# Hi-PACE/hipace

Hardware: AMD Instinct MI355X
Metric: transverse slices/s at 1024^2 x 4ppc (explicit solver) (higher is better)
Workload: dtype f64

## Files before the change

hipace_amd/_lib.py:

```python
import ctypes as C
import os
import subprocess


def hip_already_started():
    import sys
    if _LIB is not None:
        return True
    t = sys.modules.get("torch")
    try:
        return bool(t is not None and t.cuda.is_initialized())
    except Exception:
        return False


_LIB = None
_HWQ_PRESET = "GPU_MAX_HW_QUEUES" in os.environ
_HIP_STARTED_AT_IMPORT = hip_already_started()
_HERE = os.path.dirname(os.path.abspath(__file__))
CSRC = os.path.join(_HERE, "csrc")
SO = os.environ.get("HPS_LIB") or os.path.join(CSRC, "libhpslice.so")


class Slab(C.Structure):
    _fields_ = [("p", C.c_void_p), ("nx", C.c_int), ("ny", C.c_int), ("ng", C.c_int), ("ncomp", C.c_int),
                ("jstride", C.c_long), ("nstride", C.c_long)]


PL_REAL = ["x", "y", "w", "ux", "uy", "psi", "x_prev", "y_prev", "ux_half", "uy_half", "psi_half"]


class Plasma(C.Structure):
    _fields_ = [(k, C.c_void_p) for k in PL_REAL] + [("idcpu", C.c_void_p), ("ion_lev", C.c_void_p), ("n", C.c_long)]


class BeamSlice(C.Structure):
    _fields_ = [(k, C.c_void_p) for k in ("x", "y", "z", "ux", "uy", "uz", "w")] + [("nsub", C.c_void_p), ("n", C.c_long)]


class Geom(C.Structure):
    _fields_ = [(k, C.c_double) for k in ("dx", "dy", "dz", "xoff", "yoff", "c", "ep0", "mu0", "q_e", "m_e")] + \
               [("plo", C.c_double * 2), ("phi", C.c_double * 2), ("bc", C.c_int), ("normalized", C.c_int)]


class Deck(C.Structure):
    _fields_ = [("nx", C.c_int), ("ny", C.c_int), ("nz", C.c_int),
                ("lo", C.c_double * 3), ("hi", C.c_double * 3),
                ("order", C.c_int), ("deriv_type", C.c_int),
                ("plasma_ppc", C.c_int * 2), ("plasma_density", C.c_double), ("plasma_radius", C.c_double),
                ("plasma_charge", C.c_double), ("plasma_mass", C.c_double), ("max_qsa", C.c_double),
                ("n_subcycles", C.c_int),
                ("beam_profile", C.c_int), ("beam_zmin", C.c_double), ("beam_zmax", C.c_double),
                ("beam_radius", C.c_double), ("beam_density", C.c_double),
                ("beam_umean", C.c_double * 3), ("beam_pos_mean", C.c_double * 3),
                ("beam_pos_std", C.c_double * 3), ("beam_ppc", C.c_int * 3), ("beam_charge", C.c_double),
                ("bc", C.c_int), ("mg_tol_rel", C.c_double), ("mg_tol_abs", C.c_double),
                ("deposit_rho", C.c_int), ("n_steps", C.c_int),
                ("dt", C.c_double), ("beam_n_subcycles", C.c_int), ("beam_mass", C.c_double), ("ext_E_slope", C.c_double * 2),
                ("bxby_solver", C.c_int), ("predcorr_tol", C.c_double), ("predcorr_max_iter", C.c_int),
                ("predcorr_mix", C.c_double), ("field_bc", C.c_int),
                ("laser_on", C.c_int), ("laser_a0", C.c_double), ("laser_w0", C.c_double), ("laser_L0", C.c_double),
                ("laser_lambda0", C.c_double), ("laser_pos", C.c_double * 3),
                ("laser_zfoc", C.c_double), ("laser_solver", C.c_int), ("laser_use_phase", C.c_int), ("si_units", C.c_int),
                ("grid_current_on", C.c_int), ("grid_current_peak", C.c_double), ("grid_current_mean", C.c_double * 3),
                ("grid_current_std", C.c_double * 3), ("laser_mg_tol_rel", C.c_double), ("laser_mg_tol_abs", C.c_double),
                ("beam_radiation_reaction", C.c_int), ("background_density_SI", C.c_double), ("beam_no_z_push", C.c_int),
                ("plasma_no_neutralize", C.c_int), ("ion_on", C.c_int), ("ion_ppc", C.c_int * 2), ("ion_density", C.c_double),
                ("ion_mass", C.c_double), ("ion_charge", C.c_double), ("ion_init_level", C.c_int), ("ion_Z", C.c_int),
                ("ion_energies", C.c_double * 56), ("ion_seed", C.c_ulonglong),
                ("beam_spin_tracking", C.c_int), ("beam_initial_spin", C.c_double * 3), ("beam_spin_anom", C.c_double),
                ("dt_adaptive", C.c_int), ("nt_per_betatron", C.c_double), ("dt_max", C.c_double),
                ("adaptive_threshold_uz", C.c_double), ("adaptive_phase_tolerance", C.c_double),
                ("adaptive_no_predict_step", C.c_int), ("adaptive_no_phase_control", C.c_int), ("adaptive_phase_substeps", C.c_int),
                ("adaptive_density", C.c_double), ("max_time", C.c_double), ("beam_uz_std", C.c_double),
                ("ext_Ez_slope", C.c_double),
                ("beam_do_salame", C.c_int), ("salame_n_iter", C.c_int), ("salame_relative_tolerance", C.c_double),
                ("salame_no_advance", C.c_int), ("salame_Ez_target_slope", C.c_double)]


COMPS = ["N_jx_beam", "N_jy_beam", "chi", "Sy", "Sx", "ExmBy", "EypBx", "Ez", "Bx", "By", "Bz",
         "Psi", "jx_beam", "jy_beam", "jz_beam", "jx", "jy", "rhomjz", "P_jx_beam", "P_jy_beam",
         "Ion_rhomjz", "rho"]
CIDX = {n: i for i, n in enumerate(COMPS)}
COMPS_PC = ["N_jx", "N_jy", "ExmBy", "EypBx", "Ez", "Bx", "By", "Bz", "Psi", "jx", "jy", "jz", "rhomjz",
            "P_Bx", "P_By", "P_jx", "P_jy", "Ion_rhomjz", "It_Bx", "It_By", "PIt_Bx", "PIt_By", "rho"]
CIDX_PC = {n: i for i, n in enumerate(COMPS_PC)}
COMPS_SALAME = ["Ez_target", "Ez_no_salame", "Ez", "jx", "jy", "jz_beam", "Bx", "By", "Sy", "Sx", "Sy_back", "Sx_back"]
ID_VALID = 1 << 63

_SIGS = {
    "hps_last_error": (C.c_char_p, []),
    "hps_version": (C.c_char_p, []),
    "hps_deposit_current": (C.c_int, [Slab, Plasma, Geom, C.c_void_p, C.c_double, C.c_double, C.c_int, C.c_double,
                                      C.c_int, C.c_void_p, C.c_void_p]),
    "hps_explicit_deposit": (C.c_int, [Slab, Plasma, Geom, C.c_void_p, C.c_void_p, C.c_double, C.c_double, C.c_int,
                                       C.c_int, C.c_int, C.c_void_p]),
    "hps_advance_plasma": (C.c_int, [Slab, Plasma, Geom, C.c_void_p, C.c_double, C.c_double, C.c_int, C.c_int,
                                     C.c_int, C.c_int, C.c_void_p]),
    "hps_tiling_create": (C.c_int, [C.c_int, C.c_int, C.c_int, C.c_long, C.POINTER(C.c_void_p)]),
    "hps_reorder_particles": (C.c_int, [C.c_void_p, Plasma, Plasma, Geom, C.c_void_p]),
    "hps_tiling_info": (C.c_int, [C.c_void_p, C.POINTER(C.c_int), C.POINTER(C.c_void_p), C.POINTER(C.c_void_p)]),
    "hps_tiling_destroy": (C.c_int, [C.c_void_p]),
    "hps_deposit_current_tiled": (C.c_int, [Slab, Plasma, Geom, C.c_void_p, C.c_double, C.c_double, C.c_int, C.c_double,
                                            C.c_int, C.c_void_p, C.c_void_p, C.c_void_p, C.c_void_p]),
    "hps_explicit_deposit_tiled": (C.c_int, [Slab, Plasma, Geom, C.c_void_p, C.c_void_p, C.c_double, C.c_double, C.c_int,
                                             C.c_int, C.c_int, C.c_void_p, C.c_void_p, C.c_void_p]),
    "hps_advance_plasma_tiled": (C.c_int, [Slab, Plasma, Geom, C.c_void_p, C.c_double, C.c_double, C.c_int, C.c_int,
                                           C.c_int, C.c_int, C.c_void_p, C.c_void_p, C.c_void_p]),
    "hps_deposit_current_tiled_laser": (C.c_int, [Slab, Plasma, Geom, C.c_void_p, C.c_int, C.c_double, C.c_double, C.c_int,
                                                  C.c_double, C.c_int, C.c_void_p, C.c_void_p, C.c_void_p, C.c_void_p]),
    "hps_explicit_deposit_tiled_laser": (C.c_int, [Slab, Plasma, Geom, C.c_void_p, C.c_int, C.c_void_p, C.c_double, C.c_double,
                                                   C.c_int, C.c_int, C.c_int, C.c_void_p, C.c_void_p, C.c_void_p]),
    "hps_advance_plasma_tiled_laser": (C.c_int, [Slab, Plasma, Geom, C.c_void_p, C.c_int, C.c_double, C.c_double, C.c_int,
                                                 C.c_int, C.c_int, C.c_int, C.c_void_p, C.c_void_p, C.c_void_p]),
    "hps_tiling_set_validity": (C.c_int, [C.c_void_p, C.c_int, C.c_int]),
    "hps_particles_record": (C.c_int, [C.c_int]),
    "hps_particles_recorded": (C.c_int, [C.c_char_p, C.c_long, C.POINTER(C.c_long)]),
    "hps_poisson_create": (C.c_int, [C.c_int, C.c_int, C.c_double, C.c_double, C.POINTER(C.c_void_p)]),
    "hps_poisson_solve": (C.c_int, [C.c_void_p, C.c_void_p, Slab, C.c_int, C.c_void_p]),
    "hps_poisson_solve_batch": (C.c_int, [C.c_void_p, C.c_int, C.c_void_p, Slab, C.c_void_p, C.c_void_p]),
    "hps_poisson_info": (C.c_int, [C.c_void_p, C.POINTER(C.c_int), C.POINTER(C.c_int), C.POINTER(C.c_int)]),
    "hps_poisson_destroy": (C.c_int, [C.c_void_p]),
    "hps_mg_create": (C.c_int, [C.c_int, C.c_int, C.c_double, C.c_double, C.POINTER(C.c_void_p)]),
    "hps_mg_solve1": (C.c_int, [C.c_void_p, Slab, C.c_int, C.c_int, C.c_int, C.c_double, C.c_double, C.c_int,
                                C.POINTER(C.c_int), C.POINTER(C.c_double), C.c_void_p]),
    "hps_mg_solve1_fabs": (C.c_int, [C.c_void_p, Slab, Slab, Slab, C.c_double, C.c_double, C.c_int,
                                     C.POINTER(C.c_int), C.POINTER(C.c_double), C.c_void_p]),
    "hps_mg_info": (C.c_int, [C.c_void_p, C.POINTER(C.c_int), C.POINTER(C.c_int), C.POINTER(C.c_int), C.POINTER(C.c_int),
                              C.POINTER(C.c_long), C.POINTER(C.c_int), C.POINTER(C.c_int), C.POINTER(C.c_int), C.POINTER(C.c_int)]),
    "hps_mg_destroy": (C.c_int, [C.c_void_p]),
    "hps_mg2_create": (C.c_int, [C.c_int, C.c_int, C.c_double, C.c_double, C.POINTER(C.c_void_p)]),
    "hps_mg2_solve2": (C.c_int, [C.c_void_p, C.c_void_p, C.c_void_p, C.c_void_p, C.c_void_p, C.c_double, C.c_double, C.c_int,
                                 C.POINTER(C.c_int), C.POINTER(C.c_double), C.c_void_p]),
    "hps_mg2_info": (C.c_int, [C.c_void_p, C.POINTER(C.c_int), C.POINTER(C.c_int), C.POINTER(C.c_int), C.POINTER(C.c_int)]),
    "hps_mg2_destroy": (C.c_int, [C.c_void_p]),
    "hps_engine_laser_vcycles": (C.c_int, [C.c_void_p, C.POINTER(C.c_long)]),
    "hps_engine_create": (C.c_int, [C.POINTER(Deck), C.c_int, C.POINTER(C.c_void_p)]),
    "hps_engine_destroy": (C.c_int, [C.c_void_p]),
    "hps_engine_begin_step": (C.c_int, [C.c_void_p]),
    "hps_engine_solve_slice": (C.c_int, [C.c_void_p, C.c_int]),
    "hps_engine_solve_slice_begin": (C.c_int, [C.c_void_p, C.c_int]),
    "hps_engine_solve_slice_finish": (C.c_int, [C.c_void_p, C.c_int]),
    "hps_engine_slice_ready": (C.c_int, [C.c_void_p]),
    "hps_engine_run_step": (C.c_int, [C.c_void_p]),
    "hps_engine_sync": (C.c_int, [C.c_void_p]),
    "hps_engine_info": (C.c_int, [C.c_void_p, C.POINTER(C.c_int), C.POINTER(C.c_int), C.POINTER(C.c_long)]),
    "hps_engine_slab": (Slab, [C.c_void_p]),
    "hps_engine_plasma": (Plasma, [C.c_void_p]),
    "hps_engine_stream": (C.c_void_p, [C.c_void_p]),
    "hps_engine_ions": (Plasma, [C.c_void_p]),
    "hps_engine_ion_stats": (C.c_int, [C.c_void_p, C.POINTER(C.c_long), C.POINTER(C.c_long)]),
    "hps_engine_checksums": (C.c_int, [C.c_void_p, C.c_void_p]),
    "hps_beam_sort_by_box": (C.c_int, [C.c_void_p, C.c_long, C.c_double, C.c_double, C.c_int, C.c_void_p, C.c_void_p,
                                       C.c_void_p, C.c_void_p]),
    "hps_engine_stats": (C.c_int, [C.c_void_p, C.POINTER(C.c_long), C.POINTER(C.c_long)]),
    "hps_engine_set_insitu_plasma": (C.c_int, [C.c_void_p, C.c_double]),
    "hps_engine_set_insitu_beam": (C.c_int, [C.c_void_p, C.c_double]),
    "hps_engine_insitu_beam": (C.c_int, [C.c_void_p, C.c_void_p]),
    "hps_engine_insitu_plasma": (C.c_int, [C.c_void_p, C.c_void_p]),
    "hps_engine_set_insitu_fields": (C.c_int, [C.c_void_p, C.c_int]),
    "hps_engine_insitu_fields": (C.c_int, [C.c_void_p, C.c_void_p]),
    "hps_engine_set_field_diagnostic": (C.c_int, [C.c_void_p, C.c_int, C.c_void_p, C.c_void_p]),
    "hps_engine_field_diagnostic": (C.c_int, [C.c_void_p, C.c_void_p]),
    "hps_engine_set_field_diagnostic_box": (C.c_int, [C.c_void_p, C.c_int, C.c_void_p, C.c_void_p, C.c_int, C.c_void_p, C.c_void_p]),
    "hps_engine_field_diagnostic_geometry": (C.c_int, [C.c_void_p, C.c_void_p, C.c_void_p, C.c_void_p]),
    "hps_engine_record_event": (C.c_int, [C.c_void_p, C.c_int, C.POINTER(C.c_void_p)]),
    "hps_engine_wait_event": (C.c_int, [C.c_void_p, C.c_void_p]),
    "hps_stream_pool_shared_pairs": (C.c_int, [C.c_int]),
    "hps_engine_copy_async": (C.c_int, [C.c_void_p, C.c_void_p, C.c_void_p, C.c_long]),
    "hps_engine_set_profiling_stride": (C.c_int, [C.c_void_p, C.c_int]),
    "hps_engine_set_laser_import": (C.c_int, [C.c_void_p, C.c_int, C.c_int]),
    "hps_engine_set_step": (C.c_int, [C.c_void_p, C.c_int]),
    "hps_engine_set_time": (C.c_int, [C.c_void_p, C.c_double, C.c_double]),
    "hps_engine_beam_moments": (C.c_int, [C.c_void_p, C.c_void_p]),
    "hps_adaptive_create": (C.c_int, [C.c_void_p, C.POINTER(C.c_void_p)]),
    "hps_adaptive_set_density_profile": (C.c_int, [C.c_void_p, C.c_int, C.c_void_p, C.c_void_p, C.c_int, C.c_void_p, C.c_void_p]),
    "hps_adaptive_initial_dt": (C.c_int, [C.c_void_p, C.c_double, C.c_double, C.c_int, C.POINTER(C.c_double)]),
    "hps_adaptive_before_step": (C.c_int, [C.c_void_p, C.c_double, C.POINTER(C.c_double)]),
    "hps_adaptive_next_time": (C.c_int, [C.c_void_p, C.POINTER(C.c_double)]),
    "hps_adaptive_after_step": (C.c_int, [C.c_void_p, C.c_void_p, C.c_double, C.c_int, C.POINTER(C.c_double)]),
    "hps_adaptive_destroy": (C.c_int, [C.c_void_p]),
    "hps_engine_export_laser_slice": (C.c_int, [C.c_void_p, C.c_int, C.c_void_p]),
    "hps_engine_import_laser_slice": (C.c_int, [C.c_void_p, C.c_int, C.c_void_p]),
    "hps_engine_import_laser_from": (C.c_int, [C.c_void_p, C.c_int, C.c_void_p]),
    "hps_engine_laser_envelope": (C.c_int, [C.c_void_p, C.c_void_p]),
    "hps_engine_laser_info": (C.c_int, [C.c_void_p, C.POINTER(C.c_int), C.POINTER(C.c_double)]),
    "hps_deposit_current_laser": (C.c_int, [Slab, Plasma, Geom, C.c_void_p, C.c_int, C.c_double, C.c_double, C.c_int, C.c_double,
                                            C.c_int, C.c_void_p, C.c_void_p]),
    "hps_explicit_deposit_laser": (C.c_int, [Slab, Plasma, Geom, C.c_void_p, C.c_int, C.c_void_p, C.c_double, C.c_double, C.c_int,
                                             C.c_int, C.c_int, C.c_void_p]),
    "hps_advance_plasma_laser": (C.c_int, [Slab, Plasma, Geom, C.c_void_p, C.c_int, C.c_double, C.c_double, C.c_int, C.c_int,
                                           C.c_int, C.c_int, C.c_void_p]),
    "hps_engine_pc_stats": (C.c_int, [C.c_void_p, C.POINTER(C.c_long), C.POINTER(C.c_double)]),
    "hps_engine_pc_zero_b_slices": (C.c_int, [C.c_void_p, C.POINTER(C.c_long)]),
    "hps_engine_set_diagnostics": (C.c_int, [C.c_void_p, C.c_int]),
    "hps_engine_set_tiling": (C.c_int, [C.c_void_p, C.c_int, C.c_int]),
    "hps_engine_fallbacks": (C.c_int, [C.c_void_p, C.POINTER(C.c_long)]),
    "hps_engine_set_fusion": (C.c_int, [C.c_void_p, C.c_int]),
    "hps_engine_set_density_profile": (C.c_int, [C.c_void_p, C.c_int, C.c_void_p, C.c_void_p, C.c_int, C.c_void_p, C.c_void_p]),
    "hps_engine_sorts": (C.c_int, [C.c_void_p, C.POINTER(C.c_long)]),
    "hps_engine_assume_initial_beam_support": (C.c_int, [C.c_void_p]),
    "hps_engine_beam_state": (C.c_int, [C.c_void_p, C.c_void_p, C.c_void_p]),
    "hps_engine_beam_capacity": (C.c_int, [C.c_void_p, C.POINTER(C.c_long)]),
    "hps_engine_set_beam_capacity": (C.c_int, [C.c_void_p, C.c_long]),
    "hps_engine_beam_message_rows": (C.c_int, [C.c_void_p, C.POINTER(C.c_int)]),
    "hps_engine_beam_spin": (C.c_int, [C.c_void_p, C.c_void_p]),
    "hps_engine_set_beam_import": (C.c_int, [C.c_void_p, C.c_int]),
    "hps_engine_export_beam_slice": (C.c_int, [C.c_void_p, C.c_int, C.c_void_p]),
    "hps_engine_import_beam_slice": (C.c_int, [C.c_void_p, C.c_int, C.c_void_p]),
    "hps_engine_set_profiling": (C.c_int, [C.c_void_p, C.c_int]),
    "hps_engine_phase_times": (C.c_int, [C.c_void_p, C.c_void_p, C.c_void_p]),
    "hps_engine_beam_info": (C.c_int, [C.c_void_p, C.POINTER(C.c_long), C.c_void_p]),
    "hps_engine_set_beam_particles": (C.c_int, [C.c_void_p, C.c_long, C.c_void_p, C.POINTER(C.c_long)]),
    "hps_engine_set_beam_storage": (C.c_int, [C.c_void_p, C.c_void_p]),
    "hps_engine_initial_beam": (C.c_int, [C.c_void_p, C.c_void_p]),
    "hps_ring_unique_id": (C.c_int, [C.c_char_p]),
    "hps_ring_init": (C.c_int, [C.c_int, C.c_int, C.c_int, C.c_char_p, C.c_char_p, C.POINTER(C.c_void_p)]),
    "hps_ring_send_slice": (C.c_int, [C.c_void_p, C.c_void_p, C.c_long, C.c_void_p, C.c_int, C.POINTER(C.c_void_p)]),
    "hps_ring_recv_slice": (C.c_int, [C.c_void_p, C.c_void_p, C.c_long, C.c_void_p, C.c_int, C.POINTER(C.c_void_p)]),
    "hps_ring_sendrecv_self": (C.c_int, [C.c_void_p, C.c_void_p, C.c_void_p, C.c_long, C.c_void_p, C.c_int, C.POINTER(C.c_void_p)]),
    "hps_ring_stream_wait": (C.c_int, [C.c_void_p, C.c_int, C.c_void_p]),
    "hps_ring_sync_sends": (C.c_int, [C.c_void_p]),
    "hps_ring_sync": (C.c_int, [C.c_void_p]),
    "hps_ring_sync_timeout": (C.c_int, [C.c_void_p, C.c_double]),
    "hps_ring_stats": (C.c_int, [C.c_void_p, C.POINTER(C.c_long), C.POINTER(C.c_long), C.POINTER(C.c_longlong), C.POINTER(C.c_longlong)]),
    "hps_engine_tiling": (C.c_int, [C.c_void_p, C.POINTER(C.c_void_p)]),
    "hps_ring_info": (C.c_int, [C.c_void_p] + [C.POINTER(C.c_int)] * 5),
    "hps_ring_destroy": (C.c_int, [C.c_void_p]),
    "hps_ring_edge_kind": (C.c_int, [C.c_void_p]),
    "hps_ring_can_send": (C.c_int, [C.c_void_p]),
    "hps_ring_recv_landed": (C.c_int, [C.c_void_p, C.c_void_p]),
    "hps_ring_engine_wait": (C.c_int, [C.c_void_p, C.c_void_p, C.c_void_p]),
    "hps_engine_salame_stats": (C.c_int, [C.c_void_p, C.c_void_p]),
    "hps_salame_only_advance": (C.c_int, [Slab, Plasma, Geom, C.c_int, C.c_int, C.c_double, C.c_double, C.c_int, C.c_int, C.c_void_p]),
    "hps_salame_jxjy_from_bxby": (C.c_int, [Slab, Geom, C.c_int, C.c_int, C.c_int, C.c_int, C.c_int, C.c_void_p]),
    "hps_salame_sxsy_from_jz": (C.c_int, [Slab, Geom, C.c_int, C.c_int, C.c_int, C.c_void_p]),
    "hps_salame_get_w": (C.c_int, [Slab, C.c_int, C.c_int, C.c_int, C.c_int, C.c_void_p, C.c_void_p, C.c_void_p]),
    "hps_salame_scale_beam_slice": (C.c_int, [C.c_void_p, C.c_long, C.c_double, C.c_void_p]),
    "hps_collide_plasma": (C.c_int, [Plasma, C.c_void_p, Plasma, C.c_void_p, Geom, C.c_int, C.c_int, C.c_double, C.c_double, C.c_int,
                                     C.c_double, C.c_double, C.c_int, C.c_double, C.c_double, C.c_ulonglong, C.c_int, C.c_int, C.c_int,
                                     C.POINTER(C.c_long), C.POINTER(C.c_long), C.c_void_p]),
    "hps_engine_add_collision": (C.c_int, [C.c_void_p, C.c_int, C.c_int, C.c_double, C.c_ulonglong]),
    "hps_engine_collision_stats": (C.c_int, [C.c_void_p, C.POINTER(C.c_long), C.POINTER(C.c_long)]),
    "hps_collide_beam_plasma": (C.c_int, [BeamSlice, Plasma, Geom, C.c_int, C.c_int, C.c_double, C.c_double, C.c_double, C.c_double,
                                          C.c_int, C.c_double, C.c_double, C.c_ulonglong, C.c_int, C.c_int, C.c_int, C.c_double,
                                          C.POINTER(C.c_long), C.POINTER(C.c_long), C.c_void_p]),
    "hps_engine_add_beam_collision": (C.c_int, [C.c_void_p, C.c_int, C.c_double, C.c_ulonglong]),
    "hps_memcpy_d2h": (C.c_int, [C.c_void_p, C.c_void_p, C.c_long]),
    "hps_memcpy_h2d": (C.c_int, [C.c_void_p, C.c_void_p, C.c_long]),
    "hps_device_count": (C.c_int, [C.POINTER(C.c_int)]),
}


def build(force=False):
    args = ["make", "-C", CSRC, "-j8"]
    if force:
        args.append("-B")
    subprocess.check_call(args + ["libhpslice.so"], stdout=subprocess.DEVNULL)
    return SO


def lib():
    global _LIB
    if _LIB is None:
        if not os.path.exists(SO):
            raise RuntimeError(
                f"{SO} is missing: the HIP extension was not built (run __graft_entry__.build()); "
                "hipace_amd has no CPU fallback")
        L = C.CDLL(SO)
        for name, (res, args) in _SIGS.items():
            fn = getattr(L, name)
            fn.restype = res
            fn.argtypes = args
        _LIB = L
    return _LIB


class HpsError(RuntimeError):
    pass


def check(status):
    if status != 0:
        raise HpsError(f"hpslice status {status}: {lib().hps_last_error().decode()}")


def fill_struct(st, d):
    for name, typ in st._fields_:
        if name not in d:
            continue
        v = d[name]
        if hasattr(typ, "_length_"):
            setattr(st, name, typ(*v))
        else:
            setattr(st, name, v)
    return st
```

hipace_amd/api.py:

```python
import ctypes as C

import numpy as np
import torch

from . import _lib
from ._lib import CIDX, COMPS, ID_VALID, PL_REAL, check


def _stream():
    return C.c_void_p(torch.cuda.current_stream().cuda_stream)


def _iarr(vals):
    return (C.c_int * len(vals))(*[int(v) for v in vals])


class Geometry:

    def __init__(self, nx, ny, lo, hi, dz, bc=1, normalized=True, consts=(1., 1., 1., 1., 1.), ng=None):
        self.nx, self.ny = nx, ny
        g = _lib.Geom()
        g.dx = (hi[0] - lo[0]) / nx
        g.dy = (hi[1] - lo[1]) / ny
        g.dz = dz
        g.xoff = 0.5 * (lo[0] + hi[0] - g.dx * (nx - 1))
        g.yoff = 0.5 * (lo[1] + hi[1] - g.dy * (ny - 1))
        g.c, g.ep0, g.mu0, g.q_e, g.m_e = consts
        g.plo = (C.c_double * 2)(lo[0], lo[1])
        g.phi = (C.c_double * 2)(hi[0], hi[1])
        g.bc = bc
        g.normalized = int(normalized)
        self.c = g


class Fields:

    def __init__(self, nx, ny, ng, ncomp, device="cuda", data=None):
        self.nx, self.ny, self.ng, self.ncomp = nx, ny, ng, ncomp
        shape = (ncomp, ny + 2 * ng, nx + 2 * ng)
        if data is None:
            self.t = torch.zeros(shape, dtype=torch.float64, device=device)
        else:
            self.t = torch.as_tensor(np.ascontiguousarray(data), dtype=torch.float64).reshape(shape).to(device).contiguous()

    def struct(self):
        s = _lib.Slab()
        s.p = self.t.data_ptr()
        s.nx, s.ny, s.ng, s.ncomp = self.nx, self.ny, self.ng, self.ncomp
        s.jstride = self.nx + 2 * self.ng
        s.nstride = s.jstride * (self.ny + 2 * self.ng)
        return s

    def numpy(self):
        return self.t.cpu().numpy()


class PlasmaSheet:

    def __init__(self, real, valid=None, ion_lev=None, device="cuda", key=None):
        real = np.ascontiguousarray(real, dtype=np.float64)
        assert real.shape[0] == 11
        self.n = real.shape[1]
        self.real = torch.as_tensor(real).to(device).contiguous()
        if valid is None:
            valid = np.ones(self.n, dtype=np.int32)
        idcpu = np.where(np.asarray(valid) != 0, np.uint64(ID_VALID | (1 << 24)), np.uint64(1 << 24)).astype(np.uint64)
        if key is not None:
            ids = (np.asarray(key, dtype=np.uint64) + np.uint64(1)) << np.uint64(24)
            idcpu = (idcpu & np.uint64(ID_VALID)) | ids
        self.idcpu = torch.as_tensor(idcpu.view(np.int64)).to(device).contiguous()
        if ion_lev is None:
            ion_lev = np.zeros(self.n, dtype=np.int32)
        self.ion_lev = torch.as_tensor(np.asarray(ion_lev, dtype=np.int32)).to(device).contiguous()

    def struct(self):
        p = _lib.Plasma()
        base = self.real.data_ptr()
        for k, name in enumerate(PL_REAL):
            setattr(p, name, base + 8 * k * self.n)
        p.idcpu = self.idcpu.data_ptr()
        p.ion_lev = self.ion_lev.data_ptr()
        p.n = self.n
        return p

    def numpy(self):
        idc = self.idcpu.cpu().numpy().view(np.uint64)
        return self.real.cpu().numpy(), ((idc >> np.uint64(63)) & np.uint64(1)).astype(np.int32)


class BoxSorter:

    def sortParticlesByBox(self, z, plo_z, dz, num_boxes):
        z = z.contiguous()
        n = z.numel()
        counts = torch.zeros(num_boxes + 1, dtype=torch.int64, device=z.device)
        offsets = torch.zeros(num_boxes + 1, dtype=torch.int64, device=z.device)
        perm = torch.zeros(max(n, 1), dtype=torch.int64, device=z.device)
        check(_lib.lib().hps_beam_sort_by_box(C.c_void_p(z.data_ptr() if n else 0), n, float(plo_z), float(dz), num_boxes,
                                              C.c_void_p(counts.data_ptr()), C.c_void_p(offsets.data_ptr()),
                                              C.c_void_p(perm.data_ptr()), _stream()))
        torch.cuda.synchronize()
        self.boxCounts = counts.cpu().numpy().astype(np.uint64)
        self.boxOffsets = offsets.cpu().numpy().astype(np.uint64)
        self.boxPermutations = perm[:n].cpu().numpy().astype(np.uint64)
        return self


class Tiling:

    def __init__(self, nx, ny, tile_size, max_particles):
        self._h = C.c_void_p()
        check(_lib.lib().hps_tiling_create(nx, ny, tile_size, max_particles, C.byref(self._h)))
        self.fallback = torch.zeros(1, dtype=torch.int32, device="cuda")

    def reorder(self, plasma, geom):
        out = PlasmaSheet.__new__(PlasmaSheet)
        out.n = plasma.n
        out.real = torch.empty_like(plasma.real)
        out.idcpu = torch.empty_like(plasma.idcpu)
        out.ion_lev = torch.empty_like(plasma.ion_lev)
        check(_lib.lib().hps_reorder_particles(self._h, plasma.struct(), out.struct(), geom.c, _stream()))
        return out

    def set_validity(self, by_weight=False, by_psi_half=False):
        check(_lib.lib().hps_tiling_set_validity(self._h, int(by_weight), int(by_psi_half)))

    def info(self):
        nt, off, perm = C.c_int(), C.c_void_p(), C.c_void_p()
        check(_lib.lib().hps_tiling_info(self._h, C.byref(nt), C.byref(off), C.byref(perm)))
        return nt.value, off.value, perm.value

    def offsets_and_perm(self, n):
        torch.cuda.synchronize()
        nt, off, perm = self.info()
        o = np.empty(nt + 2, dtype=np.int32)
        p = np.empty(n, dtype=np.uint32)
        check(_lib.lib().hps_memcpy_d2h(o.ctypes.data_as(C.c_void_p), C.c_void_p(off), o.nbytes))
        if n:
            check(_lib.lib().hps_memcpy_d2h(p.ctypes.data_as(C.c_void_p), C.c_void_p(perm), p.nbytes))
        return o, p

    def __del__(self):
        if getattr(self, "_h", None) and _lib is not None:
            _lib.lib().hps_tiling_destroy(self._h)
            self._h = None


def DepositCurrent(plasma, fields, geom, charge, mass, depos_order, jx=-1, jy=-1, jz=-1, rho=-1, chi=-1,
                   rhomjz=-1, max_qsa_weighting_factor=35.0, can_ionize=False, n_qsa=None, tiling=None, aabs=-1):
    comp = _iarr([jx, jy, jz, rho, chi, rhomjz])
    nq = C.c_void_p(n_qsa.data_ptr()) if n_qsa is not None else None
    if tiling is None:
        check(_lib.lib().hps_deposit_current_laser(fields.struct(), plasma.struct(), geom.c, comp, aabs, charge, mass,
                                                   depos_order, max_qsa_weighting_factor, int(can_ionize), nq, _stream()))
    else:
        check(_lib.lib().hps_deposit_current_tiled_laser(fields.struct(), plasma.struct(), geom.c, comp, aabs, charge, mass,
                                                         depos_order, max_qsa_weighting_factor, int(can_ionize), nq,
                                                         tiling._h, C.c_void_p(tiling.fallback.data_ptr()), _stream()))


def ExplicitDeposition(plasma, fields, geom, charge, mass, depos_order, Bz, Ez, ExmBy, EypBx, Sy, Sx,
                       derivative_type=2, can_ionize=False, tiling=None, aabs=-1):
    if tiling is None:
        check(_lib.lib().hps_explicit_deposit_laser(fields.struct(), plasma.struct(), geom.c, _iarr([Bz, Ez, ExmBy, EypBx]),
                                                    aabs, _iarr([Sy, Sx]), charge, mass, depos_order, derivative_type,
                                                    int(can_ionize), _stream()))
    else:
        check(_lib.lib().hps_explicit_deposit_tiled_laser(fields.struct(), plasma.struct(), geom.c,
                                                          _iarr([Bz, Ez, ExmBy, EypBx]), aabs, _iarr([Sy, Sx]), charge, mass,
                                                          depos_order, derivative_type, int(can_ionize), tiling._h,
                                                          C.c_void_p(tiling.fallback.data_ptr()), _stream()))


def AdvancePlasmaParticles(plasma, fields, geom, charge, mass, depos_order, Psi, Ez, Bx, By, Bz,
                           temp_slice=False, n_subcycles=1, can_ionize=False, tiling=None, aabs=-1):
    if tiling is None:
        check(_lib.lib().hps_advance_plasma_laser(fields.struct(), plasma.struct(), geom.c, _iarr([Psi, Ez, Bx, By, Bz]),
                                                  aabs, charge, mass, depos_order, int(temp_slice), n_subcycles,
                                                  int(can_ionize), _stream()))
    else:
        check(_lib.lib().hps_advance_plasma_tiled_laser(fields.struct(), plasma.struct(), geom.c,
                                                        _iarr([Psi, Ez, Bx, By, Bz]), aabs, charge, mass, depos_order,
                                                        int(temp_slice), n_subcycles, int(can_ionize), tiling._h,
                                                        C.c_void_p(tiling.fallback.data_ptr()), _stream()))


def CoulombCollision(plasma_a, plasma_b, geom, charge_a, mass_a, charge_b=None, mass_b=None, can_ionize_a=False,
                     can_ionize_b=False, coulomb_log=-1.0, background_density_SI=0.0, seed=0, collision=0, step=0, islice=0,
                     tiling_a=None, tiling_b=None):
    if plasma_b is plasma_a or charge_b is None:
        charge_b, mass_b, can_ionize_b = charge_a, mass_a, can_ionize_a
    pairs, over = C.c_long(), C.c_long()
    check(_lib.lib().hps_collide_plasma(plasma_a.struct(), tiling_a._h if tiling_a is not None else None,
                                        plasma_b.struct(), tiling_b._h if tiling_b is not None else None, geom.c, geom.nx, geom.ny,
                                        charge_a, mass_a, int(can_ionize_a), charge_b, mass_b, int(can_ionize_b), coulomb_log,
                                        background_density_SI, seed, collision, step, islice, C.byref(pairs), C.byref(over),
                                        _stream()))
    return pairs.value, over.value


class BeamSlice:

    def __init__(self, soa, nsub=None, device="cuda"):
        soa = np.ascontiguousarray(soa, dtype=np.float64)
        assert soa.ndim == 2 and soa.shape[0] == 7
        self.n = soa.shape[1]
        self.soa = torch.as_tensor(soa).to(device).contiguous()
        self.nsub = None if nsub is None else torch.as_tensor(np.ascontiguousarray(nsub, dtype=np.int32)).to(device).contiguous()
        assert self.nsub is None or self.nsub.numel() == self.n

    def struct(self):
        b = _lib.BeamSlice()
        base = self.soa.data_ptr()
        for k, name in enumerate(("x", "y", "z", "ux", "uy", "uz", "w")):
            setattr(b, name, base + 8 * k * self.n)
        b.nsub = self.nsub.data_ptr() if self.nsub is not None else None
        b.n = self.n
        return b

    def numpy(self):
        return self.soa.cpu().numpy()


def BeamPlasmaCollision(beam, plasma, geom, charge_beam, mass_beam, charge_plasma, mass_plasma, dt, can_ionize_plasma=False,
                        coulomb_log=-1.0, background_density_SI=0.0, seed=0, collision=0, step=0, islice=0):
    pairs, over = C.c_long(), C.c_long()
    check(_lib.lib().hps_collide_beam_plasma(beam.struct(), plasma.struct(), geom.c, geom.nx, geom.ny, charge_beam, mass_beam,
                                             charge_plasma, mass_plasma, int(can_ionize_plasma), coulomb_log, background_density_SI,
                                             seed, collision, step, islice, dt, C.byref(pairs), C.byref(over), _stream()))
    return pairs.value, over.value


def record_particle_dispatch(on=True):
    check(_lib.lib().hps_particles_record(int(on)))


def recorded_particle_dispatch():
    n = C.c_long()
    check(_lib.lib().hps_particles_recorded(None, 0, C.byref(n)))
    buf = C.create_string_buffer(n.value + 1)
    check(_lib.lib().hps_particles_recorded(buf, n.value + 1, C.byref(n)))
    return set(buf.value.decode().split())


class FFTPoissonSolver:

    def __init__(self, nx, ny, dx, dy, device="cuda"):
        self.nx, self.ny = nx, ny
        self._h = C.c_void_p()
        check(_lib.lib().hps_poisson_create(nx, ny, dx, dy, C.byref(self._h)))
        self.staging = torch.zeros((ny, nx), dtype=torch.float64, device=device)

    def StagingArea(self):
        return self.staging

    BACKENDS = ("own-sym", "own-pow2", "dense", "rocfft")

    def info(self):
        b, n, m = C.c_int(), C.c_int(), C.c_int()
        check(_lib.lib().hps_poisson_info(self._h, C.byref(b), C.byref(n), C.byref(m)))
        return self.BACKENDS[b.value], n.value, m.value

    def SolvePoissonEquation(self, lhs_fields, comp):
        check(_lib.lib().hps_poisson_solve(self._h, C.c_void_p(self.staging.data_ptr()), lhs_fields.struct(), comp,
                                           _stream()))

    def __del__(self):
        if getattr(self, "_h", None) and _lib is not None:
            _lib.lib().hps_poisson_destroy(self._h)
            self._h = None


class MultiGrid2:

    def __init__(self, nx, ny, dx, dy):
        self._h = C.c_void_p()
        check(_lib.lib().hps_mg2_create(nx, ny, dx, dy, C.byref(self._h)))

    def solve2(self, sol2, rhs2, acoef_real, acoef_imag, tol_rel=1e-4, tol_abs=0.0, nummaxiter=200):
        it = C.c_int()
        rn = C.c_double()
        for t in (sol2, rhs2, acoef_real, acoef_imag):
            assert t.is_cuda and t.is_contiguous() and t.dtype == torch.float64
        check(_lib.lib().hps_mg2_solve2(self._h, sol2.data_ptr(), rhs2.data_ptr(), acoef_real.data_ptr(), acoef_imag.data_ptr(),
                                        tol_rel, tol_abs, nummaxiter, C.byref(it), C.byref(rn), _stream()))
        return it.value, rn.value

    BOTTOMS = ("lower-v", "single-block", "per-sweep")
    TILES = ("single-block", "32x16", "64x32")

    def info(self):
        nl, top, b, t = C.c_int(), C.c_int(), C.c_int(), (C.c_int * 31)()
        check(_lib.lib().hps_mg2_info(self._h, C.byref(nl), C.byref(top), C.byref(b), t))
        return {"nlev": nl.value, "low_top": top.value, "bottom": self.BOTTOMS[b.value],
                "tiles": tuple(self.TILES[v] for v in t if v >= 0)}

    def __del__(self):
        if getattr(self, "_h", None) and _lib is not None:
            _lib.lib().hps_mg2_destroy(self._h)
            self._h = None


class MultiGrid:

    def __init__(self, nx, ny, dx, dy):
        self._h = C.c_void_p()
        check(_lib.lib().hps_mg_create(nx, ny, dx, dy, C.byref(self._h)))

    LOWV = ("v3", "v-cc", "v-nodal", "bottom")
    TILES = ("TileSmall", "TileBig", "TileSmall-pull", "TileMid-pull")

    def info(self):
        cc, nl, lb, kind, npyr, nres, pull1 = (C.c_int() for _ in range(7))
        lds, t = C.c_long(), (C.c_int * 31)()
        check(_lib.lib().hps_mg_info(self._h, C.byref(cc), C.byref(nl), C.byref(lb), C.byref(kind), C.byref(lds), t,
                                     C.byref(pull1), C.byref(npyr), C.byref(nres)))
        return {"cc": bool(cc.value), "nlev": nl.value, "lowv_begin": lb.value, "lowv": self.LOWV[kind.value],
                "lowv_lds": lds.value, "tiles": tuple(self.TILES[v] for v in t if v >= 0), "nodal_pull1": bool(pull1.value),
                "pyramid": npyr.value, "restricts": nres.value}

    def solve1(self, fields, sol_comp, rhs_comp, acoef_comp, tol_rel=1e-4, tol_abs=2.2250738585072014e-308,
               nummaxiter=200):
        it = C.c_int()
        rn = C.c_double()
        check(_lib.lib().hps_mg_solve1(self._h, fields.struct(), sol_comp, rhs_comp, acoef_comp, tol_rel, tol_abs,
                                       nummaxiter, C.byref(it), C.byref(rn), _stream()))
        return it.value, rn.value

    def solve1_fabs(self, sol, rhs, acoef, tol_rel=1e-4, tol_abs=2.2250738585072014e-308, nummaxiter=200):
        it = C.c_int()
        rn = C.c_double()
        check(_lib.lib().hps_mg_solve1_fabs(self._h, sol.struct(), rhs.struct(), acoef.struct(), tol_rel, tol_abs, nummaxiter,
                                            C.byref(it), C.byref(rn), _stream()))
        return it.value, rn.value

    def __del__(self):
        if getattr(self, "_h", None) and _lib is not None:
            _lib.lib().hps_mg_destroy(self._h)
            self._h = None


class AdaptiveTimeStep:

    def __init__(self, deck, density_profile=None):
        self.deck = dict(deck)
        self._dk = _lib.fill_struct(_lib.Deck(), deck)
        self._h = C.c_void_p()
        check(_lib.lib().hps_adaptive_create(C.byref(self._dk), C.byref(self._h)))
        if density_profile is not None:
            self.set_density_profile(*density_profile)

    @classmethod
    def for_engine(cls, engine):
        return cls(engine.deck, getattr(engine, "density_profile", None))

    def __del__(self):
        if getattr(self, "_h", None) and _lib is not None:
            _lib.lib().hps_adaptive_destroy(self._h)
            self._h = None

    def set_density_profile(self, r=(), fr=(), ct=(), ft=()):
        a = [np.ascontiguousarray(v, dtype=np.float64) for v in (r, fr, ct, ft)]
        assert len(a[0]) == len(a[1]) and len(a[2]) == len(a[3])
        p = [x.ctypes.data_as(C.c_void_p) if len(x) else None for x in a]
        check(_lib.lib().hps_adaptive_set_density_profile(self._h, len(a[0]), p[0], p[1], len(a[2]), p[2], p[3]))

    def initial_dt(self, uz_mean=None, uz_std=None, nstages=1):
        um = self.deck["beam_umean"][2] if uz_mean is None else uz_mean
        us = self.deck.get("beam_uz_std", 0.0) if uz_std is None else uz_std
        dt = C.c_double()
        check(_lib.lib().hps_adaptive_initial_dt(self._h, float(um), float(us), int(nstages), C.byref(dt)))
        return dt.value

    def CalculateFromDensity(self, t):
        dt = C.c_double()
        check(_lib.lib().hps_adaptive_before_step(self._h, float(t), C.byref(dt)))
        return dt.value

    def next_time(self):
        t = C.c_double()
        check(_lib.lib().hps_adaptive_next_time(self._h, C.byref(t)))
        return t.value

    def CalculateFromMinUz(self, moments, t, nstages=1):
        m = np.ascontiguousarray(moments, dtype=np.float64)
        assert m.shape == (4,)
        dt = C.c_double()
        check(_lib.lib().hps_adaptive_after_step(self._h, m.ctypes.data_as(C.c_void_p), float(t), int(nstages), C.byref(dt)))
        return dt.value


class SliceEngine:

    def __init__(self, deck, device=0, tile_size=None, sort_period=None):
        self.deck = dict(deck)
        self.step_times = []
        self._dk = _lib.fill_struct(_lib.Deck(), deck)
        self._h = C.c_void_p()
        check(_lib.lib().hps_engine_create(C.byref(self._dk), device, C.byref(self._h)))
        if tile_size is not None:
            check(_lib.lib().hps_engine_set_tiling(self._h, tile_size, sort_period or 128))
        for a, b, coulomb_log, seed in deck.get("collisions", ()):
            if a == "beam":
                self.add_beam_collision(b, coulomb_log, seed)
            else:
                self.add_collision(a, b, coulomb_log, seed)
        nc, ng, npart = C.c_int(), C.c_int(), C.c_long()
        check(_lib.lib().hps_engine_info(self._h, C.byref(nc), C.byref(ng), C.byref(npart)))
        self.ncomp, self.ng, self.nparticles = nc.value, ng.value, npart.value

    def __del__(self):
        if getattr(self, "_h", None) and _lib is not None:
            _lib.lib().hps_engine_destroy(self._h)
            self._h = None

    def begin_step(self):
        check(_lib.lib().hps_engine_begin_step(self._h))

    def solve_slice(self, islice):
        check(_lib.lib().hps_engine_solve_slice(self._h, islice))

    def solve_slice_begin(self, islice):
        check(_lib.lib().hps_engine_solve_slice_begin(self._h, islice))

    def solve_slice_finish(self, islice):
        check(_lib.lib().hps_engine_solve_slice_finish(self._h, islice))

    def slice_ready(self):
        return bool(_lib.lib().hps_engine_slice_ready(self._h))

    def run_step(self):
        check(_lib.lib().hps_engine_run_step(self._h))

    def sync(self):
        check(_lib.lib().hps_engine_sync(self._h))

    def set_tiling(self, tile_size=16, sort_period=128):
        check(_lib.lib().hps_engine_set_tiling(self._h, tile_size, sort_period))

    def add_collision(self, species_a=0, species_b=0, coulomb_log=-1.0, seed=0):
        check(_lib.lib().hps_engine_add_collision(self._h, species_a, species_b, coulomb_log, seed))

    def add_beam_collision(self, plasma_species=0, coulomb_log=-1.0, seed=0):
        check(_lib.lib().hps_engine_add_beam_collision(self._h, plasma_species, coulomb_log, seed))

    def collision_stats(self):
        a, b = C.c_long(), C.c_long()
        check(_lib.lib().hps_engine_collision_stats(self._h, C.byref(a), C.byref(b)))
        return dict(pairs_collided=a.value, overfull_cells=b.value)

    @property
    def moving(self):
        return float(self.deck.get("dt", 0.0)) != 0.0 or self.adaptive

    @property
    def adaptive(self):
        return bool(self.deck.get("dt_adaptive", 0))

    def set_time(self, t, dt):
        check(_lib.lib().hps_engine_set_time(self._h, float(t), float(dt)))

    def beam_moments(self):
        out = np.zeros(4, dtype=np.float64)
        check(_lib.lib().hps_engine_beam_moments(self._h, out.ctypes.data_as(C.c_void_p)))
        return out

    def run_adaptive(self, n_steps=None, controller=None, on_step_end=None):
        assert self.adaptive, "run_adaptive needs a deck with dt_adaptive"
        n = self.deck["n_steps"] if n_steps is None else int(n_steps)
        ats = controller or AdaptiveTimeStep.for_engine(self)
        ats.initial_dt(nstages=1)
        t, log = 0.0, []
        for step in range(n):
            if t == float("inf"):
                break
            dt = ats.CalculateFromDensity(t)
            log.append((step, t, dt))
            self.set_time(t, dt)
            self.run_step()
            ats.CalculateFromMinUz(self.beam_moments(), t, 1)
            if on_step_end is not None:
                on_step_end(step, t, dt)
            t = ats.next_time()
        return log

    def beam_capacity(self):
        n = C.c_long()
        check(_lib.lib().hps_engine_beam_capacity(self._h, C.byref(n)))
        return n.value

    def set_beam_capacity(self, cap):
        check(_lib.lib().hps_engine_set_beam_capacity(self._h, int(cap)))

    def beam_message_doubles(self):
        r = C.c_int()
        check(_lib.lib().hps_engine_beam_message_rows(self._h, C.byref(r)))
        return 1 + r.value * self.beam_capacity()

    def beam_spin(self):
        nbeam, _ = self.beam_layout()
        out = np.zeros((3, max(nbeam, 1)), dtype=np.float64)
        check(_lib.lib().hps_engine_beam_spin(self._h, out.ctypes.data_as(C.c_void_p) if nbeam else None))
        return out[:, :nbeam]

    def set_beam_import(self, on):
        check(_lib.lib().hps_engine_set_beam_import(self._h, int(on)))

    def export_beam_slice(self, islice, msg):
        check(_lib.lib().hps_engine_export_beam_slice(self._h, islice, C.c_void_p(msg.data_ptr())))

    def import_beam_slice(self, islice, msg):
        check(_lib.lib().hps_engine_import_beam_slice(self._h, islice, C.c_void_p(msg.data_ptr())))

    def beam_state(self):
        nbeam, _ = self.beam_layout()
        nz = self.deck["nz"]
        bnd = np.zeros(nz + 1, dtype=np.int64)
        soa = np.zeros((7, max(nbeam, 1)), dtype=np.float64)
        check(_lib.lib().hps_engine_beam_state(self._h, bnd.ctypes.data_as(C.c_void_p), soa.ctypes.data_as(C.c_void_p) if nbeam else None))
        return bnd, soa[:, :nbeam].reshape(7, nbeam) if nbeam else soa[:, :0]

    def set_density_profile(self, r=(), fr=(), ct=(), ft=()):
        self.density_profile = (r, fr, ct, ft)
        a = [np.ascontiguousarray(v, dtype=np.float64) for v in (r, fr, ct, ft)]
        assert len(a[0]) == len(a[1]) and len(a[2]) == len(a[3])
        p = [x.ctypes.data_as(C.c_void_p) if len(x) else None for x in a]
        check(_lib.lib().hps_engine_set_density_profile(self._h, len(a[0]), p[0], p[1], len(a[2]), p[2], p[3]))

    def set_fusion(self, on=True):
        check(_lib.lib().hps_engine_set_fusion(self._h, int(on)))

    def fallbacks(self):
        n = C.c_long()
        check(_lib.lib().hps_engine_fallbacks(self._h, C.byref(n)))
        return n.value

    def sorts(self):
        n = C.c_long()
        check(_lib.lib().hps_engine_sorts(self._h, C.byref(n)))
        return n.value

    def set_diagnostics(self, on=True):
        check(_lib.lib().hps_engine_set_diagnostics(self._h, int(on)))

    def set_profiling(self, on=True, stride=1, light=False):
        check(_lib.lib().hps_engine_set_profiling_stride(self._h, int(stride)))
        check(_lib.lib().hps_engine_set_profiling(self._h, (2 if light else 1) if on else 0))

    def beam_layout(self):
        nb = C.c_long()
        off = (C.c_long * (self.deck["nz"] + 1))()
        check(_lib.lib().hps_engine_beam_info(self._h, C.byref(nb), off))
        return nb.value, np.array(off[:], dtype=np.int64)

    def set_beam_particles(self, soa, allow_outside=False):
        soa = np.ascontiguousarray(soa, dtype=np.float64)
        assert soa.ndim == 2 and soa.shape[0] == 7
        out = C.c_long(0)
        check(_lib.lib().hps_engine_set_beam_particles(self._h, soa.shape[1], soa.ctypes.data_as(C.c_void_p),
                                                       C.byref(out) if allow_outside else None))
        return out.value

    def set_beam_storage(self, tensor, injected_beam_support=False):
        check(_lib.lib().hps_engine_set_beam_storage(self._h, C.c_void_p(tensor.data_ptr()) if tensor is not None else None))
        if tensor is not None and injected_beam_support:
            check(_lib.lib().hps_engine_assume_initial_beam_support(self._h))

    def initial_beam_into(self, tensor):
        check(_lib.lib().hps_engine_initial_beam(self._h, C.c_void_p(tensor.data_ptr())))

    def set_field_diagnostic(self, names, coarsening=(1, 1, 1), diag_type="xyz", patch_lo=None, patch_hi=None):
        idx = _lib.CIDX_PC if self.deck.get("bxby_solver", 0) else _lib.CIDX
        cn = self.comp_names()
        comps = (C.c_int * len(names))(*[idx[n] if n in idx else cn.index(n) for n in names])
        co = (C.c_int * 3)(*coarsening)
        sd = {"xyz": -1, "yz": 0, "xz": 1, "xy": 2}[diag_type]
        plo = (C.c_double * 3)(*patch_lo) if patch_lo is not None else None
        phi = (C.c_double * 3)(*patch_hi) if patch_hi is not None else None
        check(_lib.lib().hps_engine_set_field_diagnostic_box(self._h, len(names), comps, co, sd, plo, phi))
        self._fd = (list(names), tuple(coarsening))

    def field_diagnostic_geometry(self):
        n, lo, hi = (C.c_int * 3)(), (C.c_double * 3)(), (C.c_double * 3)()
        check(_lib.lib().hps_engine_field_diagnostic_geometry(self._h, n, lo, hi))
        return tuple(n), tuple(lo), tuple(hi)

    def field_diagnostic(self):
        names, _ = self._fd
        n, _, _ = self.field_diagnostic_geometry()
        out = np.empty((len(names), n[2], n[1], n[0]))
        check(_lib.lib().hps_engine_field_diagnostic(self._h, out.ctypes.data_as(C.c_void_p)))
        return {k: out[i] for i, k in enumerate(names)}

    INSITU_FIELDS = ["[Ex^2]", "[Ey^2]", "[Ez^2]", "[Bx^2]", "[By^2]", "[Bz^2]", "[ExmBy^2]", "[EypBx^2]", "[jz_beam]",
                     "[Ez*jz_beam]"]

    INSITU_PLASMA = ["sum(w)", "[x]", "[x^2]", "[y]", "[y^2]", "[ux]", "[ux^2]", "[uy]", "[uy^2]", "[uz]", "[uz^2]", "[ga]",
                     "[ga^2]", "[(ga-1)*(1-vz)]", "Np"]

    INSITU_BEAM = ["sum(w)", "[x]", "[x^2]", "[y]", "[y^2]", "[z]", "[z^2]", "[ux]", "[ux^2]", "[uy]", "[uy^2]", "[uz]", "[uz^2]",
                   "[x*ux]", "[y*uy]", "[z*uz]", "[x*uy]", "[y*ux]", "[ux/uz]", "[uy/uz]", "[ga]", "[ga^2]", "Np"]

    def laser_vcycles(self):
        n = C.c_long()
        check(_lib.lib().hps_engine_laser_vcycles(self._h, C.byref(n)))
        return n.value

    def set_insitu_beam(self, radius=float("inf")):
        check(_lib.lib().hps_engine_set_insitu_beam(self._h, min(float(radius), 1.0e300)))

    def insitu_beam(self):
        out = np.empty((23, self.deck["nz"]))
        check(_lib.lib().hps_engine_insitu_beam(self._h, out.ctypes.data_as(C.c_void_p)))
        return {n: out[i] for i, n in enumerate(self.INSITU_BEAM)}

    def set_insitu_plasma(self, radius=float("inf")):
        check(_lib.lib().hps_engine_set_insitu_plasma(self._h, min(float(radius), 1.0e300)))

    def insitu_plasma(self):
        out = np.empty((15, self.deck["nz"]))
        check(_lib.lib().hps_engine_insitu_plasma(self._h, out.ctypes.data_as(C.c_void_p)))
        return {n: out[i] for i, n in enumerate(self.INSITU_PLASMA)}
# ... 142 lines not shown
```

hipace_amd/csrc/multigrid.hip:

```cpp
#include "common.h"
#include <type_traits>
#include "mg_gate.h"
#include "slab_ops.h"

#include <vector>
#include <algorithm>
#include <cmath>
#include <cstring>

namespace hps {

struct FView {
    double* p; long js, ns; int oi, oj;
    __device__ __forceinline__ double& operator() (int i, int j, int n) const {
        const unsigned o = (unsigned)((i + oi) + (j + oj)*(int)js + n*(int)ns)*8u;
        return *reinterpret_cast<double*>(reinterpret_cast<char*>(p) + o);
    }
};

struct LevBox { int lox, loy, hix, hiy;
                int vlx, vly, vhx, vhy; };

enum { SRC_ZERO = 0, SRC_DIRECT = 1, SRC_PROLONG = 2 };

#define HPS_KEEP(x) asm volatile("" :: "v"(x))

#ifdef HPS_STAMPS
__device__ long long* g_mg_dbg = nullptr;
#define MG_STAMP(i) do { if (g_mg_dbg && blockIdx.x == 0 && threadIdx.x == 0) g_mg_dbg[i] = __builtin_amdgcn_s_memtime(); } while (0)
#else
#define MG_STAMP(i) do { } while (0)
#endif

template <int TX_, int TY_, int NT_>
struct TileShape {
    static constexpr int TX = TX_, TY = TY_, NT = NT_;
    static constexpr int AX = TX + 2, AY = TY + 2;
    static constexpr int PR = TX/2;
    static constexpr int GPAIRS = TX*TY/2/NT;
    static_assert(TX*TY/2 % NT == 0 && NT % 64 == 0 && (PR == 16 || PR == 32), "tile shape");
};
using TileBig = TileShape<64, 32, 512>;
using TileMid = TileShape<32, 32, 256>;
using TileHuge = TileShape<64, 48, 512>;
using TileHugeNodal = TileShape<64, 32, 512>;
template <bool CC> struct HugeTileOf { using type = TileHuge; };
template <> struct HugeTileOf<false> { using type = TileHugeNodal; };
using TileSmall = TileShape<32, 16, 256>;

template <bool CC>
__device__ __forceinline__ double diag_c0 (int i, int j, const LevBox& b, double acf, double facx, double facy)
{
    double c0 = -(acf + 2.0*(facx + facy));
    if (CC && (i == b.lox || i == b.hix)) c0 -= 2.0*facx;
    if (CC && (j == b.loy || j == b.hiy)) c0 -= 2.0*facy;
    return c0;
}

template <bool CC, bool INTERIOR = false, class P>
__device__ __forceinline__ double offdiag (P c, int sy, int i, int j, const LevBox& b, double facx, double facy)
{
    const double w = c[-1], e = c[1], s = c[-sy], n = c[sy];
    double lx = facx*(w + e), ly = facy*(s + n);
    if (CC && !INTERIOR) {
        const double fx43 = facx*(4./3.), fy43 = facy*(4./3.);
        lx = (i == b.lox) ? fx43*e : ((i == b.hix) ? fx43*w : lx);
        ly = (j == b.loy) ? fy43*n : ((j == b.hiy) ? fy43*s : ly);
    }
    return lx + ly;
}

template <class P>
__device__ __forceinline__ double offdiag_m (P c, int sy, double fxm, double fym)
{
    return fxm*(c[-1] + c[1]) + fym*(c[-sy] + c[sy]);
}
template <bool CC>
__device__ __forceinline__ double wall_mult (int i, int lo, int hi, double fac)
{
    return (CC && (i == lo || i == hi)) ? fac*(4./3.) : fac;
}

template <bool INTERIOR = false>
__device__ __forceinline__ double residual_v (double p0, double w, double e, double s, double n, int i, int j, const LevBox& b,
                                              double rhs, double acf, double facx, double facy);

template <bool INTERIOR = false, class P>
__device__ __forceinline__ double residual_at (P c, int sy, int i, int j, const LevBox& b,
                                               double rhs, double acf, double facx, double facy)
{
    return residual_v<INTERIOR>(c[0], c[-1], c[1], c[-sy], c[sy], i, j, b, rhs, acf, facx, facy);
}

template <bool INTERIOR>
__device__ __forceinline__ double residual_v (double p0, double w, double e, double s, double n, int i, int j, const LevBox& b,
                                              double rhs, double acf, double facx, double facy)
{
    double lap = -2.0*(facx + facy)*p0;
    double tx = facx*(w + e), ty = facy*(s + n);
    if (!INTERIOR) {
        tx = (i == b.lox) ? facx*((4./3.)*e - 2.0*p0) : ((i == b.hix) ? facx*((4./3.)*w - 2.0*p0) : tx);
        ty = (j == b.loy) ? facy*((4./3.)*n - 2.0*p0) : ((j == b.hiy) ? facy*((4./3.)*s - 2.0*p0) : ty);
    }
    lap += tx;
    lap += ty;
    return rhs + acf*p0 - lap;
}

template <bool CC>
__device__ __forceinline__ double prolong_at (const FView& crse, int i, int j, int n)
{
    const int ic = i >> 1, jc = j >> 1;
    if (CC) return crse(ic, jc, n);
    const bool io = (i & 1), jo = (j & 1);
    if (io && jo)  return (crse(ic, jc, n) + crse(ic+1, jc, n) + crse(ic, jc+1, n) + crse(ic+1, jc+1, n))*0.25;
    if (io)        return (crse(ic, jc, n) + crse(ic+1, jc, n))*0.5;
    if (jo)        return (crse(ic, jc, n) + crse(ic, jc+1, n))*0.5;
    return crse(ic, jc, n);
}

constexpr int MG_MAX_VCYCLES = 1024;
template <int NT>
__device__ __forceinline__ void block_max_to (unsigned long long* slot, double v, double* s_red)
{
    for (int o = 32; o > 0; o >>= 1) v = fmax(v, __shfl_xor(v, o));
    if ((threadIdx.x & 63) == 0) s_red[threadIdx.x >> 6] = v;
    __syncthreads();
    if (threadIdx.x == 0) {
        double m = 0.0;
        for (int w = 0; w < NT/64; ++w) m = fmax(m, s_red[w]);
        if (m > 0.0) atomicMax(slot + (blockIdx.x & (MG_NSUB - 1)), (unsigned long long)__double_as_longlong(m));
    }
    __syncthreads();
}

#define MG_ROWPK(m) const int jj = BR ? (tid / PR)*GPAIRS + (m) : (tid + MG_NT*(m)) / PR, pk = BR ? (tid & (PR - 1)) : (tid + MG_NT*(m)) - jj*PR
template <bool CC> __device__ __forceinline__ double restrict_at (const FView& fine, int i, int j, int n);
template <class TS, bool CC, int SRC, bool DO_RES, bool FUSE_R, bool INTERIOR, int NSW, bool GATE_IN = (NSW == 4), bool RPULL = false>
__device__ __forceinline__ void smooth_tile (double (&s_phi)[2][TS::AY*TS::AX], double* s_red, double* s_crs, const LevBox& b, const FView& phi_out,
                                             const FView& phi_out2, const FView& rhs, const FView& acf, const FView& phi_in, const FView& crse,
                                             const FView& res_out, const FView& cres_out, double facx, double facy,
                                             int gi0, int gj0, unsigned long long* resnorm, unsigned long long* rhsnorm, const StopRule& sr)
{
    constexpr int E = DO_RES ? NSW : NSW - 1;
    constexpr int GT_X = TS::TX, GT_Y = TS::TY, GA_X = TS::AX, GA_Y = TS::AY, MG_NT = TS::NT, GPAIRS = TS::GPAIRS, PR = TS::PR;
    constexpr int AXH = GA_X/2, CH = GA_Y*AXH;
    constexpr bool BR = GPAIRS <= 2 || INTERIOR;
    const int tid = threadIdx.x;
    const int cpar = (gi0 + gj0) & 1;
    MG_STAMP(0);
    double r0[GPAIRS][2], r1[GPAIRS][2], ac[GPAIRS][2], ci[GPAIRS][2];
    bool in[GPAIRS][2];
    int hx[GPAIRS];
    double fxm[GPAIRS][2], fym[GPAIRS];
    double rmax = 0.0;
#pragma unroll
    for (int m = 0; m < GPAIRS; ++m) {
        MG_ROWPK(m);
        const int j = gj0 + jj;
        hx[m] = (gi0 + 2*pk + j) & 1;
        fym[m] = INTERIOR ? facy : wall_mult<CC>(j, b.loy, b.hiy, facy);
#pragma unroll
        for (int p = 0; p < 2; ++p) {
            const int i = gi0 + 2*pk + (hx[m] ^ p);
            fxm[m][p] = INTERIOR ? facx : wall_mult<CC>(i, b.lox, b.hix, facx);
            const int ic = INTERIOR ? i : min(max(i, b.vlx), b.vhx), jc = INTERIOR ? j : min(max(j, b.vly), b.vhy);
            const bool ok = INTERIOR || (ic == i && jc == j);
            in[m][p] = ok;
            double a0, a1;
            if constexpr (RPULL) { a0 = restrict_at<CC>(crse, ic, jc, 0); a1 = restrict_at<CC>(crse, ic, jc, 1); }
            else { a0 = rhs(ic, jc, 0); a1 = rhs(ic, jc, 1); }
            const double a2 = acf(ic, jc, 0);
            r0[m][p] = ok ? a0 : 0.0;
            r1[m][p] = ok ? a1 : 0.0;
            ac[m][p] = ok ? a2 : 0.0;
            ci[m][p] = 1.0/diag_c0<CC>(i, j, b, ac[m][p], facx, facy);
            if (rhsnorm) rmax = fmax(rmax, fmax(fabs(r0[m][p]), fabs(r1[m][p])));
        }
    }
    MG_STAMP(1);
    {
        constexpr int NF = (GA_X*GA_Y + MG_NT - 1)/MG_NT;
        double v0[NF], v1[NF];
        constexpr bool PLDS = !CC && SRC == SRC_PROLONG;
        constexpr int CXN = GA_X/2 + 2, CYN = GA_Y/2 + 2;
        const int cx0 = (INTERIOR ? gi0 - 1 : min(max(gi0 - 1, b.vlx), b.vhx)) >> 1, cy0 = (INTERIOR ? gj0 - 1 : min(max(gj0 - 1, b.vly), b.vhy)) >> 1;
        if constexpr (PLDS) {
            const int cxl = b.vlx >> 1, cxh = (b.vhx >> 1) + 1, cyl = b.vly >> 1, cyh = (b.vhy >> 1) + 1;
            constexpr int NC = (CXN*CYN + MG_NT - 1)/MG_NT;
            double c0[NC], c1[NC];
#pragma unroll
            for (int m = 0; m < NC; ++m) {
                const int q = min(tid + MG_NT*m, CXN*CYN - 1);
                const int ly = q / CXN, lx = q - ly*CXN;
                const int X = min(max(cx0 + lx, cxl), cxh), Y = min(max(cy0 + ly, cyl), cyh);
                c0[m] = crse(X, Y, 0); c1[m] = crse(X, Y, 1);
            }
#pragma unroll
            for (int m = 0; m < NC; ++m) {
                const int q = tid + MG_NT*m;
                if (q < CXN*CYN) { s_crs[q] = c0[m]; s_crs[CXN*CYN + q] = c1[m]; }
            }
        }
#pragma unroll
        for (int m = 0; m < NF; ++m) {
            const int s = min(tid + MG_NT*m, GA_X*GA_Y - 1);
            const int lj = s / GA_X, li = s - lj*GA_X;
            const int i = gi0 - 1 + li, j = gj0 - 1 + lj;
            v0[m] = 0.0; v1[m] = 0.0;
            if (SRC != SRC_ZERO) {
                const int ic = INTERIOR ? i : min(max(i, b.vlx), b.vhx), jc = INTERIOR ? j : min(max(j, b.vly), b.vhy);
                double a0 = phi_in(ic, jc, 0), a1 = phi_in(ic, jc, 1);
                if (SRC == SRC_PROLONG && !PLDS) { a0 += prolong_at<CC>(crse, ic, jc, 0); a1 += prolong_at<CC>(crse, ic, jc, 1); }
                const bool inside = INTERIOR || (ic == i && jc == j);
                v0[m] = inside ? a0 : 0.0; v1[m] = inside ? a1 : 0.0;
            }
        }
        if constexpr (PLDS) {
            __syncthreads();
#pragma unroll
            for (int m = 0; m < NF; ++m) {
                const int s = min(tid + MG_NT*m, GA_X*GA_Y - 1);
                const int lj = s / GA_X, li = s - lj*GA_X;
                const int i = gi0 - 1 + li, j = gj0 - 1 + lj;
                const int ic = INTERIOR ? i : min(max(i, b.vlx), b.vhx), jc = INTERIOR ? j : min(max(j, b.vly), b.vhy);
                const bool inside = INTERIOR || (ic == i && jc == j);
                const int o = ((jc >> 1) - cy0)*CXN + (ic >> 1) - cx0;
                const bool io = (ic & 1), jo = (jc & 1);
                double p0, p1;
                const double* q0 = s_crs + o; const double* q1 = s_crs + CXN*CYN + o;
                if (io && jo)  { p0 = (q0[0] + q0[1] + q0[CXN] + q0[CXN + 1])*0.25; p1 = (q1[0] + q1[1] + q1[CXN] + q1[CXN + 1])*0.25; }
                else if (io)   { p0 = (q0[0] + q0[1])*0.5; p1 = (q1[0] + q1[1])*0.5; }
                else if (jo)   { p0 = (q0[0] + q0[CXN])*0.5; p1 = (q1[0] + q1[CXN])*0.5; }
                else           { p0 = q0[0]; p1 = q1[0]; }
                if (inside) { v0[m] += p0; v1[m] += p1; }
            }
        }
        {
            if (GATE_IN) {
                const bool active = vcycle_active(sr);
#pragma unroll
                for (int m = 0; m < GPAIRS; ++m) { HPS_KEEP(r0[m][0]); HPS_KEEP(r0[m][1]); HPS_KEEP(r1[m][0]); HPS_KEEP(r1[m][1]); HPS_KEEP(ac[m][0]); HPS_KEEP(ac[m][1]); }
#pragma unroll
                for (int m = 0; m < NF; ++m) { HPS_KEEP(v0[m]); HPS_KEEP(v1[m]); }
                if (!active) return;
            }
        }
#pragma unroll
        for (int m = 0; m < NF; ++m) {
            const int s = tid + MG_NT*m;
            if (s < GA_X*GA_Y) {
                const int lj = s / GA_X, li = s - lj*GA_X;
                const int o = ((cpar + li + lj) & 1)*CH + lj*AXH + (li >> 1);
                s_phi[0][o] = v0[m]; s_phi[1][o] = v1[m];
            }
        }
    }
    __syncthreads();
    MG_STAMP(2);

    double l0[GPAIRS][2], l1[GPAIRS][2];
    if constexpr (BR) {
#pragma unroll
        for (int m = 0; m < GPAIRS; ++m) {
            MG_ROWPK(m);
            const int row = (jj + 1)*AXH + pk;
#pragma unroll
            for (int p = 0; p < 2; ++p) { const int h = hx[m] ^ p; l0[m][p] = s_phi[0][p*CH + row + h]; l1[m][p] = s_phi[1][p*CH + row + h]; }
        }
#pragma unroll
        for (int icolor = 0; icolor < NSW; ++icolor) {
            const int p = icolor & 1;
#pragma unroll
            for (int m = 0; m < GPAIRS; ++m) {
                MG_ROWPK(m);
                const int h = hx[m] ^ p;
                const int row = (jj + 1)*AXH + pk;
                const double* nb0 = &s_phi[0][(1 - p)*CH + row];
                const double* nb1 = &s_phi[1][(1 - p)*CH + row];
                const double we0 = nb0[h] + l0[m][1 - p], we1 = nb1[h] + l1[m][1 - p];
                const double s0 = (m > 0) ? l0[m > 0 ? m - 1 : 0][1 - p] : nb0[h - AXH], s1 = (m > 0) ? l1[m > 0 ? m - 1 : 0][1 - p] : nb1[h - AXH];
                const double t0 = (m + 1 < GPAIRS) ? l0[m + 1 < GPAIRS ? m + 1 : m][1 - p] : nb0[h + AXH], t1 = (m + 1 < GPAIRS) ? l1[m + 1 < GPAIRS ? m + 1 : m][1 - p] : nb1[h + AXH];
                const double n0 = (r0[m][p] - (fxm[m][p]*we0 + fym[m]*(s0 + t0)))*ci[m][p];
                const double n1 = (r1[m][p] - (fxm[m][p]*we1 + fym[m]*(s1 + t1)))*ci[m][p];
                if (INTERIOR || in[m][p]) { s_phi[0][p*CH + row + h] = n0; s_phi[1][p*CH + row + h] = n1; l0[m][p] = n0; l1[m][p] = n1; }
            }
            __syncthreads();
        }
    } else {
#pragma unroll
        for (int icolor = 0; icolor < NSW; ++icolor) {
            constexpr int dummy = 0; (void)dummy;
            const int p = icolor & 1;
#pragma unroll
            for (int m = 0; m < GPAIRS; ++m) {
                MG_ROWPK(m);
                const int h = hx[m] ^ p;
                const int row = (jj + 1)*AXH + pk;
                const double* nb0 = &s_phi[0][(1 - p)*CH + row];
                const double* nb1 = &s_phi[1][(1 - p)*CH + row];
                const double n0 = (r0[m][p] - (fxm[m][p]*(nb0[0] + nb0[1]) + fym[m]*(nb0[h - AXH] + nb0[h + AXH])))*ci[m][p];
                const double n1 = (r1[m][p] - (fxm[m][p]*(nb1[0] + nb1[1]) + fym[m]*(nb1[h - AXH] + nb1[h + AXH])))*ci[m][p];
                if (INTERIOR || in[m][p]) { s_phi[0][p*CH + row + h] = n0; s_phi[1][p*CH + row + h] = n1; }
            }
            __syncthreads();
        }
    }
    MG_STAMP(3);

    double resmax = 0.0;
    if constexpr (BR) {
        double la0[GPAIRS], ra0[GPAIRS], la1[GPAIRS], ra1[GPAIRS];
        bool finr[GPAIRS];
#pragma unroll
        for (int m = 0; m < GPAIRS; ++m) {
            MG_ROWPK(m);
            const int j = gj0 + jj;
            const bool rowok = (jj >= E && jj < GT_Y - E);
            double q0[2], q1[2];
            bool fin[2];
#pragma unroll
            for (int p = 0; p < 2; ++p) {
                const int h = hx[m] ^ p;
                const int ii = 2*pk + h;
                fin[p] = rowok && ii >= E && ii < GT_X - E && in[m][p];
                const int i = gi0 + ii;
                const int row = (jj + 1)*AXH + pk;
                const double f0 = l0[m][p], f1 = l1[m][p];
                q0[p] = 0.0; q1[p] = 0.0;
                if (DO_RES) {
                    const double* nb0 = &s_phi[0][(1 - p)*CH + row];
                    const double* nb1 = &s_phi[1][(1 - p)*CH + row];
                    const double o0 = nb0[h], o1 = nb1[h];
                    const double w0 = h ? l0[m][1 - p] : o0, e0 = h ? o0 : l0[m][1 - p];
                    const double w1 = h ? l1[m][1 - p] : o1, e1 = h ? o1 : l1[m][1 - p];
                    const double s0 = (m > 0) ? l0[m > 0 ? m - 1 : 0][1 - p] : nb0[h - AXH], s1 = (m > 0) ? l1[m > 0 ? m - 1 : 0][1 - p] : nb1[h - AXH];
                    const double n0 = (m + 1 < GPAIRS) ? l0[m + 1 < GPAIRS ? m + 1 : m][1 - p] : nb0[h + AXH], n1 = (m + 1 < GPAIRS) ? l1[m + 1 < GPAIRS ? m + 1 : m][1 - p] : nb1[h + AXH];
                    const double t0 = residual_v<INTERIOR>(f0, w0, e0, s0, n0, i, j, b, r0[m][p], ac[m][p], facx, facy);
                    const double t1 = residual_v<INTERIOR>(f1, w1, e1, s1, n1, i, j, b, r1[m][p], ac[m][p], facx, facy);
                    q0[p] = fin[p] ? t0 : 0.0; q1[p] = fin[p] ? t1 : 0.0;
                    resmax = fmax(resmax, fmax(fabs(q0[p]), fabs(q1[p])));
                }
                if (fin[p]) {
                    if constexpr (RPULL) { rhs(i, j, 0) = r0[m][p]; rhs(i, j, 1) = r1[m][p]; }
                    if (DO_RES && !FUSE_R) { res_out(i, j, 0) = q0[p]; res_out(i, j, 1) = q1[p]; }
                    phi_out(i, j, 0) = f0;
                    phi_out(i, j, 1) = f1;
                    if (phi_out2.p) { phi_out2(i, j, 0) = f0; phi_out2(i, j, 1) = f1; }
                }
            }
            const bool sw = (hx[m] != 0);
            la0[m] = sw ? q0[1] : q0[0]; ra0[m] = sw ? q0[0] : q0[1];
            la1[m] = sw ? q1[1] : q1[0]; ra1[m] = sw ? q1[0] : q1[1];
            finr[m] = fin[0];
        }
        if (FUSE_R) {
            const double c0 = __shfl_down(la0[0], PR), d0 = __shfl_down(ra0[0], PR);
            const double c1 = __shfl_down(la1[0], PR), d1 = __shfl_down(ra1[0], PR);
#pragma unroll
            for (int m = 0; m < GPAIRS; ++m) {
                MG_ROWPK(m);
                if (finr[m] && ((jj & 1) == 0)) {
                    const bool own = (m + 1 < GPAIRS);
                    const int mu = own ? m + 1 : m;
                    const double ua0 = own ? la0[mu] : c0, ub0 = own ? ra0[mu] : d0, ua1 = own ? la1[mu] : c1, ub1 = own ? ra1[mu] : d1;
                    const int ic = (gi0 + 2*pk) >> 1, jc = (gj0 + jj) >> 1;
                    cres_out(ic, jc, 0) = 0.25*(la0[m] + ra0[m] + ua0 + ub0);
                    cres_out(ic, jc, 1) = 0.25*(la1[m] + ra1[m] + ua1 + ub1);
                }
            }
        }
    } else {
#pragma unroll
        for (int m = 0; m < GPAIRS; ++m) {
            MG_ROWPK(m);
            const int j = gj0 + jj;
            const bool rowok = (jj >= E && jj < GT_Y - E);
            double q0[2], q1[2];
            bool fin[2];
#pragma unroll
            for (int p = 0; p < 2; ++p) {
                const int h = hx[m] ^ p;
                const int ii = 2*pk + h;
                fin[p] = rowok && ii >= E && ii < GT_X - E && in[m][p];
                const int i = gi0 + ii;
                const int row = (jj + 1)*AXH + pk;
                const double f0 = s_phi[0][p*CH + row + h], f1 = s_phi[1][p*CH + row + h];
                q0[p] = 0.0; q1[p] = 0.0;
                if (DO_RES) {
                    const double* nb0 = &s_phi[0][(1 - p)*CH + row];
                    const double* nb1 = &s_phi[1][(1 - p)*CH + row];
                    const double t0 = residual_v<INTERIOR>(f0, nb0[0], nb0[1], nb0[h - AXH], nb0[h + AXH], i, j, b, r0[m][p], ac[m][p], facx, facy);
                    const double t1 = residual_v<INTERIOR>(f1, nb1[0], nb1[1], nb1[h - AXH], nb1[h + AXH], i, j, b, r1[m][p], ac[m][p], facx, facy);
                    q0[p] = fin[p] ? t0 : 0.0; q1[p] = fin[p] ? t1 : 0.0;
                    resmax = fmax(resmax, fmax(fabs(q0[p]), fabs(q1[p])));
                }
                if (fin[p]) {
                    if constexpr (RPULL) { rhs(i, j, 0) = r0[m][p]; rhs(i, j, 1) = r1[m][p]; }
                    if (DO_RES && !FUSE_R) { res_out(i, j, 0) = q0[p]; res_out(i, j, 1) = q1[p]; }
                    phi_out(i, j, 0) = f0;
                    phi_out(i, j, 1) = f1;
                    if (phi_out2.p) { phi_out2(i, j, 0) = f0; phi_out2(i, j, 1) = f1; }
                }
            }
            if (FUSE_R) {
                const bool sw = (hx[m] != 0);
                const double la0 = sw ? q0[1] : q0[0], ra0 = sw ? q0[0] : q0[1];
                const double la1 = sw ? q1[1] : q1[0], ra1 = sw ? q1[0] : q1[1];
                const double c0 = __shfl_down(la0, PR), d0 = __shfl_down(ra0, PR);
                const double c1 = __shfl_down(la1, PR), d1 = __shfl_down(ra1, PR);
                if (fin[0] && ((tid & PR) == 0)) {
                    const int ic = (gi0 + 2*pk) >> 1, jc = j >> 1;
                    cres_out(ic, jc, 0) = 0.25*(la0 + ra0 + c0 + d0);
                    cres_out(ic, jc, 1) = 0.25*(la1 + ra1 + c1 + d1);
                }
            }
        }
    }
    MG_STAMP(4);
    if (DO_RES && resnorm) block_max_to<MG_NT>(resnorm, resmax, s_red);
    if (rhsnorm) block_max_to<MG_NT>(rhsnorm, rmax, s_red);
    MG_STAMP(5);
}

template <class TS, bool CC, int SRC, bool DO_RES, bool FUSE_R, int NSW = 4, bool RPULL = false>
__global__ __launch_bounds__(TS::NT, (RPULL && TS::GPAIRS > 1) ? 2 : 4)
void k_smooth (LevBox b, FView phi_out, FView phi_out2, FView rhs, FView acf, FView phi_in, FView crse, FView res_out,
               FView cres_out, double facx, double facy, int ntx, unsigned long long* resnorm,
               unsigned long long* rhsnorm, StopRule sr)
{
    static_assert(!FUSE_R || (CC && DO_RES), "fused restriction is cell-centred only");
    if (NSW != 4 && !vcycle_active(sr)) return;
    constexpr int GT_X = TS::TX, GT_Y = TS::TY;
    __shared__ double s_phi[2][TS::AY*TS::AX];
    __shared__ double s_red[TS::NT/64];
    constexpr bool PLDS = !CC && SRC == SRC_PROLONG;
    __shared__ double s_crs[PLDS ? 2*(TS::AX/2 + 2)*(TS::AY/2 + 2) : 1];
    constexpr int E = DO_RES ? NSW : NSW - 1;
    constexpr int FX = GT_X - 2*E, FY = GT_Y - 2*E;
    const int nb = gridDim.x, q8 = nb >> 3, r8 = nb & 7, xcd = blockIdx.x & 7;
    const int tile = xcd*q8 + min(xcd, r8) + (blockIdx.x >> 3);
    const int bx = tile % ntx, by = tile / ntx;
    const int gi0 = b.vlx + bx*FX - E;
    const int gj0 = b.vly + by*FY - E;
    const bool interior = (gi0 - 1 >= b.vlx) && (gi0 + GT_X <= b.vhx) && (gj0 - 1 >= b.vly) && (gj0 + GT_Y <= b.vhy)
                       && (gi0 > b.lox) && (gi0 + GT_X - 1 < b.hix) && (gj0 > b.loy) && (gj0 + GT_Y - 1 < b.hiy);
    constexpr bool GATE_IN = (NSW == 4);
    if (interior) smooth_tile<TS, CC, SRC, DO_RES, FUSE_R, true, NSW, GATE_IN, RPULL>(s_phi, s_red, s_crs, b, phi_out, phi_out2, rhs, acf, phi_in, crse, res_out, cres_out,
                                                             facx, facy, gi0, gj0, resnorm, rhsnorm, sr);
    else          smooth_tile<TS, CC, SRC, DO_RES, FUSE_R, false, NSW, GATE_IN, RPULL>(s_phi, s_red, s_crs, b, phi_out, phi_out2, rhs, acf, phi_in, crse, res_out, cres_out,
                                                              facx, facy, gi0, gj0, resnorm, rhsnorm, sr);
}

template <bool CC>
__device__ __forceinline__ double restrict_at (const FView& fine, int i, int j, int n)
{
    if (CC) return 0.25*(fine(2*i, 2*j, n) + fine(2*i+1, 2*j, n) + fine(2*i, 2*j+1, n) + fine(2*i+1, 2*j+1, n));
    return (1./16.)*(fine(2*i-1, 2*j-1, n) + 2.*fine(2*i, 2*j-1, n) + fine(2*i+1, 2*j-1, n)
                   + 2.*fine(2*i-1, 2*j, n) + 4.*fine(2*i, 2*j, n) + 2.*fine(2*i+1, 2*j, n)
                   + fine(2*i-1, 2*j+1, n) + 2.*fine(2*i, 2*j+1, n) + fine(2*i+1, 2*j+1, n));
}

template <bool CC>
__global__ __launch_bounds__(256)
void k_restrict (LevBox cb, FView crse, FView fine, int ncomp, StopRule sr)
{
    if (!vcycle_active(sr)) return;
    const int i = cb.vlx + blockIdx.x*blockDim.x + threadIdx.x;
    const int j = cb.vly + blockIdx.y;
    if (i > cb.vhx || j > cb.vhy) return;
    for (int n = 0; n < ncomp; ++n) crse(i, j, n) = restrict_at<CC>(fine, i, j, n);
}

typedef __attribute__((address_space(3))) double lds_double;

struct LowLev { LevBox b; int nxb; int cells; int off; };

struct LView {
    lds_double* p; int nxb; int lox, loy;
    __device__ __forceinline__ lds_double& operator() (int i, int j) const { return p[(i - lox) + (j - loy)*nxb]; }
};
__device__ __forceinline__ LView lplane (lds_double* base, const LowLev& l, int plane)
{
    return LView{base + l.off + plane*l.cells, l.nxb, l.b.lox, l.b.loy};
}

template <bool CC>
__device__ __forceinline__ double lrestrict (const LView& f, int i, int j)
{
    if (CC) return 0.25*(f(2*i, 2*j) + f(2*i+1, 2*j) + f(2*i, 2*j+1) + f(2*i+1, 2*j+1));
    return (1./16.)*(f(2*i-1, 2*j-1) + 2.*f(2*i, 2*j-1) + f(2*i+1, 2*j-1)
                   + 2.*f(2*i-1, 2*j) + 4.*f(2*i, 2*j) + 2.*f(2*i+1, 2*j)
                   + f(2*i-1, 2*j+1) + 2.*f(2*i, 2*j+1) + f(2*i+1, 2*j+1));
}

template <bool CC>
__device__ __forceinline__ double lprolong (const LView& c, int i, int j)
{
    const int ic = i >> 1, jc = j >> 1;
    if (CC) return c(ic, jc);
    const bool io = (i & 1), jo = (j & 1);
    if (io && jo)  return (c(ic, jc) + c(ic+1, jc) + c(ic, jc+1) + c(ic+1, jc+1))*0.25;
    if (io)        return (c(ic, jc) + c(ic+1, jc))*0.5;
    if (jo)        return (c(ic, jc) + c(ic, jc+1))*0.5;
    return c(ic, jc);
}

#define HPS_LOW_FOR_VALID(l, i, j)                                                          \
    for (int j = (l).b.vly + (int)(threadIdx.x >> 5); j <= (l).b.vhy; j += (int)(blockDim.x >> 5))   \
        for (int i = (l).b.vlx + (int)(threadIdx.x & 31); i <= (l).b.vhx; i += 32)

__device__ __forceinline__ double low_fac (double f0, int l) { for (int k = 0; k < l; ++k) f0 *= 0.25; return f0; }

template <bool CC>
__device__ void low_sweeps (lds_double* base, const LowLev& l, double facx, double facy, int nsweeps, int n0 = 0, int n1 = 2)
{
    const int ti = (int)(threadIdx.x & 15), tj = (int)(threadIdx.x >> 4);
    const int si = 16, sj = (int)(blockDim.x >> 4);
    const LView cinv = lplane(base, l, 7);
    if (!CC && l.b.vhy - l.b.vly < sj && l.b.vhx - l.b.vlx < 2*si) {
        const int j = l.b.vly + tj;
        const bool rowok = j <= l.b.vhy;
        const int jc = rowok ? j : l.b.vly;
        int off[2]; bool ok[2]; double ci[2], r0[2], r1[2];
        const bool two = (n1 - n0) == 2;
        lds_double* ph0 = base + l.off + (3 + n0)*l.cells;
        lds_double* ph1 = base + l.off + (2 + n1)*l.cells;
#pragma unroll
        for (int par = 0; par < 2; ++par) {
            const int i = l.b.vlx + ((l.b.vlx + jc + par) & 1) + 2*ti;
            ok[par] = rowok && i <= l.b.vhx;
            const int ic = ok[par] ? i : l.b.vlx;
            off[par] = (ic - l.b.lox) + (jc - l.b.loy)*l.nxb;
            ci[par] = cinv(ic, jc);
            r0[par] = base[l.off + (1 + n0)*l.cells + off[par]];
            r1[par] = base[l.off + n1*l.cells + off[par]];
        }
        const int sy = l.nxb;
        for (int is = 0; is < nsweeps; ++is) {
            const int par = is & 1;
            const int o = par ? off[1] : off[0];
            const bool k = par ? ok[1] : ok[0];
            const double c = par ? ci[1] : ci[0], ra = par ? r0[1] : r0[0], rb = par ? r1[1] : r1[0];
            if (k) {
                {   const lds_double* q = ph0 + o;
                    const double w = q[-1], e = q[1], so = q[-sy], no = q[sy];
                    ph0[o] = (ra - (facx*(w + e) + facy*(so + no)))*c; }
                if (two) {
                    const lds_double* q = ph1 + o;
                    const double w = q[-1], e = q[1], so = q[-sy], no = q[sy];
                    ph1[o] = (rb - (facx*(w + e) + facy*(so + no)))*c; }
            }
            __syncthreads();
        }
        return;
    }
    for (int is = 0; is < nsweeps; ++is) {
        for (int j = l.b.vly + tj; j <= l.b.vhy; j += sj) {
            for (int i = l.b.vlx + ((l.b.vlx + j + is) & 1) + 2*ti; i <= l.b.vhx; i += 2*si) {
                const double ci = cinv(i, j);
                for (int n = n0; n < n1; ++n) {
                    const LView rhs = lplane(base, l, 1 + n), phi = lplane(base, l, 3 + n);
                    phi(i, j) = (rhs(i, j) - offdiag<CC, false>((const lds_double*)&phi(i, j), l.nxb, i, j, l.b, facx, facy))*ci;
                }
            }
        }
        __syncthreads();
    }
}

template <bool CC>
__device__ void low_hier_level (lds_double* base, const LowLev& f, const LowLev& c)
{
    const LView fine = lplane(base, f, 0), crse = lplane(base, c, 0);
    HPS_LOW_FOR_VALID(c, i, j) crse(i, j) = lrestrict<CC>(fine, i, j);
    __syncthreads();
}
template <bool CC>
__device__ void low_cinv_level (lds_double* base, const LowLev& l, double fx, double fy)
{
    const LView acf = lplane(base, l, 0), cinv = lplane(base, l, 7);
    HPS_LOW_FOR_VALID(l, i, j) cinv(i, j) = 1.0/diag_c0<CC>(i, j, l.b, acf(i, j), fx, fy);
}

template <bool CC>
__device__ void low_down_level (lds_double* base, const LowLev& l, const LowLev& c, double facx, double facy, int n0, int n1)
{
    low_sweeps<CC>(base, l, facx, facy, 4, n0, n1);
    {
        const LView acf = lplane(base, l, 0);
        HPS_LOW_FOR_VALID(l, i, j) {
            const double a = acf(i, j);
            for (int n = n0; n < n1; ++n) {
                const LView rhs = lplane(base, l, 1 + n), phi = lplane(base, l, 3 + n), rc = lplane(base, l, 5 + n);
                rc(i, j) = residual_at<false>((const lds_double*)&phi(i, j), l.nxb, i, j, l.b, rhs(i, j), a, facx, facy);
            }
        }
        __syncthreads();
    }
    {
        HPS_LOW_FOR_VALID(c, i, j) {
            for (int n = n0; n < n1; ++n) lplane(base, c, 1 + n)(i, j) = lrestrict<CC>(lplane(base, l, 5 + n), i, j);
        }
        __syncthreads();
    }
}
template <bool CC>
__device__ void low_up_level (lds_double* base, const LowLev& l, const LowLev& c, double facx, double facy, int n0, int n1)
{
    HPS_LOW_FOR_VALID(l, i, j) {
        for (int n = n0; n < n1; ++n) {
            const LView fine = lplane(base, l, 3 + n);
            fine(i, j) = fine(i, j) + lprolong<CC>(lplane(base, c, 3 + n), i, j);
        }
    }
    __syncthreads();
    low_sweeps<CC>(base, l, facx, facy, 4, n0, n1);
}

template <bool CC, int P0>
__device__ __forceinline__ void low_bottom_regs_p (lds_double* base, const LowLev& l, double facx, double facy, int nsweeps, int n0, int n1)
{
    const int nvx = l.b.vhx - l.b.vlx + 1, nvy = l.b.vhy - l.b.vly + 1;
    for (int n = n0 + (int)threadIdx.x; n < n1; n += (int)blockDim.x) {
        const LView rhs = lplane(base, l, 1 + n), phi = lplane(base, l, 3 + n), cinv = lplane(base, l, 7);
        double p[5][5], r[3][3], c[3][3];
        bool ok[3][3];
#pragma unroll
        for (int a = 0; a < 5; ++a)
#pragma unroll
            for (int b = 0; b < 5; ++b) p[a][b] = 0.0;
#pragma unroll
        for (int a = 0; a < 3; ++a)
#pragma unroll
            for (int b = 0; b < 3; ++b) {
                ok[a][b] = a < nvy && b < nvx;
                r[a][b] = ok[a][b] ? rhs(l.b.vlx + b, l.b.vly + a) : 0.0;
                c[a][b] = ok[a][b] ? cinv(l.b.vlx + b, l.b.vly + a) : 0.0;
            }
        auto half = [&] (auto colc) {
            constexpr int col = decltype(colc)::value;
#pragma unroll
            for (int a = 0; a < 3; ++a)
#pragma unroll
                for (int b = 0; b < 3; ++b) {
                    if (((a + b + P0 + col) & 1) != 0) continue;
                    const int i = l.b.vlx + b, j = l.b.vly + a;
                    const double w = p[a + 1][b], e = p[a + 1][b + 2], so = p[a][b + 1], no = p[a + 2][b + 1];
                    double lx = facx*(w + e), ly = facy*(so + no);
                    if (CC) {
                        const double fx43 = facx*(4./3.), fy43 = facy*(4./3.);
                        lx = (i == l.b.lox) ? fx43*e : ((i == l.b.hix) ? fx43*w : lx);
                        ly = (j == l.b.loy) ? fy43*no : ((j == l.b.hiy) ? fy43*so : ly);
                    }
                    const double v = (r[a][b] - (lx + ly))*c[a][b];
                    p[a + 1][b + 1] = ok[a][b] ? v : p[a + 1][b + 1];
                }
        };
        int is = 0;
        for (; is + 1 < nsweeps; is += 2) { half(std::integral_constant<int, 0>{}); half(std::integral_constant<int, 1>{}); }
        if (is < nsweeps) half(std::integral_constant<int, 0>{});
#pragma unroll
        for (int a = 0; a < 3; ++a)
#pragma unroll
            for (int b = 0; b < 3; ++b)
                if (ok[a][b]) phi(l.b.vlx + b, l.b.vly + a) = p[a + 1][b + 1];
    }
}
template <bool CC>
__device__ void low_bottom_lane (lds_double* base, const LowLev& l, double facx, double facy, int nsweeps, int n0, int n1)
{
    if (((l.b.vlx + l.b.vly) & 1) == 0) low_bottom_regs_p<CC, 0>(base, l, facx, facy, nsweeps, n0, n1);
    else low_bottom_regs_p<CC, 1>(base, l, facx, facy, nsweeps, n0, n1);
    __syncthreads();
}

template <bool CC>
__global__ __launch_bounds__(1024)
void k_lower_v (const LowLev* __restrict__ lv, int nl, const double* __restrict__ acf_g, const double* __restrict__ res_g,
                double* __restrict__ cor_g, double facx0, double facy0, int nsweeps_bottom, StopRule sr, FView fine_res = FView{})
{
    if (!vcycle_active(sr)) return;
    extern __shared__ __attribute__((aligned(16))) double lds_raw[];
    lds_double* base = (lds_double*)lds_raw;
    const int n0 = gridDim.x == 2 ? (int)blockIdx.x : 0, n1 = gridDim.x == 2 ? n0 + 1 : 2;
    MG_STAMP(8);
    {
        const LowLev last = lv[nl - 1];
        const int total = last.off + 8*last.cells;
        for (int s = threadIdx.x; s < total; s += blockDim.x) base[s] = 0.0;
        __syncthreads();
    }
    {
        const LowLev l = lv[0];
        if (fine_res.p) {
            for (int s = threadIdx.x; s < l.cells; s += blockDim.x) base[l.off + s] = acf_g[s];
            HPS_LOW_FOR_VALID(l, i, j) {
                for (int n = n0; n < n1; ++n) lplane(base, l, 1 + n)(i, j) = restrict_at<CC>(fine_res, i, j, n);
            }
        } else
        for (int s = threadIdx.x; s < l.cells; s += blockDim.x) {
            base[l.off + s] = acf_g[s];
            base[l.off + l.cells + s] = res_g[s];
            base[l.off + 2*l.cells + s] = res_g[l.cells + s];
        }
        __syncthreads();
    }
    for (int il = 1; il < nl; ++il) { const LowLev f = lv[il - 1], c = lv[il]; low_hier_level<CC>(base, f, c); }
    MG_STAMP(9);
    for (int il = 0; il < nl; ++il) { const LowLev l = lv[il]; low_cinv_level<CC>(base, l, low_fac(facx0, il), low_fac(facy0, il)); }
    __syncthreads();
    MG_STAMP(10);
    for (int il = 0; il < nl - 1; ++il) { const LowLev l = lv[il], c = lv[il + 1]; low_down_level<CC>(base, l, c, low_fac(facx0, il), low_fac(facy0, il), n0, n1); }
    MG_STAMP(11);
    {
        const LowLev l = lv[nl - 1];
        if (l.b.vhx - l.b.vlx < 3 && l.b.vhy - l.b.vly < 3)
            low_bottom_lane<CC>(base, l, low_fac(facx0, nl - 1), low_fac(facy0, nl - 1), nsweeps_bottom, n0, n1);
        else
        low_sweeps<CC>(base, l, low_fac(facx0, nl - 1), low_fac(facy0, nl - 1), nsweeps_bottom, n0, n1);
    }
    MG_STAMP(12);
    for (int il = nl - 2; il >= 0; --il) { const LowLev l = lv[il], c = lv[il + 1]; low_up_level<CC>(base, l, c, low_fac(facx0, il), low_fac(facy0, il), n0, n1); }
    MG_STAMP(13);
    {
        const LowLev l = lv[0];
        for (int s = n0*l.cells + threadIdx.x; s < n1*l.cells; s += blockDim.x) cor_g[s] = base[l.off + 3*l.cells + s];
    }
    MG_STAMP(14);
}

constexpr int LOW2_MAXLEV = 8;
struct Low2 { int nl; int total; int nx[LOW2_MAXLEV], ny[LOW2_MAXLEV], off[LOW2_MAXLEV];
              int coff[LOW2_MAXLEV], cbase, ctot; };

__device__ __forceinline__ LevBox cc_box (int nx, int ny) { return LevBox{0, 0, nx - 1, ny - 1, 0, 0, nx - 1, ny - 1}; }

template <bool WAVE>
__device__ __forceinline__ void lvl_sync ()
{
    if (WAVE) asm volatile("" ::: "memory");
    else __syncthreads();
}

struct Blk {
    lds_double* c0;
    int pitch;
    bool act;
    bool ok[4];
    double fxm[2], fym[2];
    double v0[4];
    double r0[4], ci[4];
};
// ... 234 lines not shown
#pragma unroll
        for (int m = 0; m < NIMG; ++m) if (t + 1024*m < ctot) base[d.cbase + t + 1024*m] = img[m];
        for (int q = t + 1024*NIMG; q < ctot; q += 1024) base[d.cbase + q] = coef_g[q];
    }
    __syncthreads();
    if (derive) {
        if (nl > 1 && A.act) {
            const int p1 = d.nx[1] + 2;
            base[d.coff[1] + ((jA >> 1) + 1)*p1 + (iA >> 1) + 1] = 0.25*(aA[0] + aA[1] + aA[2] + aA[3]);
        }
        __syncthreads();
        for (int l = 1; l < nl; ++l) {
            const double fx = lvl_fac(facx0, l), fy = lvl_fac(facy0, l);
            const int nx = d.nx[l], ny = d.ny[l];
            Blk B; int i, j;
            blk_geometry(B, base + d.coff[l], nx, ny, t, fx, fy, i, j);
            const int ps = B.pitch*(ny + 2);
            lds_double* acf = B.c0;
            const int ok[4] = {0, 1, B.pitch, B.pitch + 1};
            if (B.act) {
                double a[4];
#pragma unroll
                for (int k = 0; k < 4; ++k) a[k] = B.ok[k] ? acf[ok[k]] : 0.0;
                if (l + 1 < nl) {
                    const int pn = d.nx[l+1] + 2;
                    base[d.coff[l+1] + ((j >> 1) + 1)*pn + (i >> 1) + 1] = 0.25*(a[0] + a[1] + a[2] + a[3]);
                }
#pragma unroll
                for (int k = 0; k < 4; ++k)
                    if (B.ok[k]) acf[ps + ok[k]] = 1.0/diag_c0<true>(i + (k & 1), j + (k >> 1), cc_box(nx, ny), a[k], fx, fy);
            }
            __syncthreads();
        }
        if (blockIdx.x == 0) for (int q = t; q < ctot; q += 1024) coef_g[q] = base[d.cbase + q];
    }
    MG_STAMP(9);
    const bool bottomA = (nl == 1);
    blk_down_sweeps<false>(A, bottomA ? nsweeps_bottom : 4);
    if (!bottomA) {
        double q0[4];
        blk_residual(A, iA, jA, bA, aA, facx0, facy0, q0);
        if (A.act) {
            const int p1 = d.nx[1] + 2, ps1 = p1*(d.ny[1] + 2);
            base[d.off[1] + ps1 + ((jA >> 1) + 1)*p1 + (iA >> 1) + 1] = 0.25*(q0[0] + q0[1] + q0[2] + q0[3]);
        }
        __syncthreads();
    }
    MG_STAMP(10);
    if (!bottomA) {
        int lw = 1;
        for (; lw < nl; ++lw) {
            const int nbx = (d.nx[lw] + 1) >> 1, nby = (d.ny[lw] + 1) >> 1;
            int lg = 0; while ((1 << lg) < nbx) ++lg;
            if ((nby << lg) <= 64) break;
        }
        for (int l = 1; l < lw; ++l)
            low_down_s<false>(base, d, l, t, lvl_fac(facx0, l), lvl_fac(facy0, l), (l == nl - 1) ? nsweeps_bottom : 4, l == nl - 1);
        MG_STAMP(11);
        if (lw < nl) {
            if (t < 64) {
                for (int l = lw; l < nl; ++l) {
                    MG_STAMP(16 + l);
                    const bool tiny = (d.nx[l] <= 8 && d.ny[l] <= 8 && l < nl - 1);
                    if (tiny) tiny_down_s(base, d, l, t, lvl_fac(facx0, l), lvl_fac(facy0, l));
                    else low_down_s<true>(base, d, l, t, lvl_fac(facx0, l), lvl_fac(facy0, l), (l == nl - 1) ? nsweeps_bottom : 4, l == nl - 1);
                }
                for (int l = nl - 2; l >= lw; --l) {
                    MG_STAMP(32 + l);
                    if (d.nx[l] <= 8 && d.ny[l] <= 8) tiny_up_s(base, d, l, t, lvl_fac(facx0, l), lvl_fac(facy0, l));
                    else low_up_s<true>(base, d, l, t, lvl_fac(facx0, l), lvl_fac(facy0, l));
                }
            }
            __syncthreads();
        }
        MG_STAMP(12);
        for (int l = min(lw - 1, nl - 2); l >= 1; --l)
            low_up_s<false>(base, d, l, t, lvl_fac(facx0, l), lvl_fac(facy0, l));
        const int p1 = d.nx[1] + 2;
        const lds_double* kc = base + d.off[1] + ((jA >> 1) + 1)*p1 + (iA >> 1) + 1;
        const double k0 = A.act ? kc[0] : 0.0;
        const int ok[4] = {0, 1, A.pitch, A.pitch + 1};
#pragma unroll
        for (int k = 0; k < 4; ++k) {
            const int o = A.ok[k] ? ok[k] : 0;
            const double c0 = A.c0[o];
            A.v0[k] = A.ok[k] ? c0 + k0 : 0.0;
            if (A.ok[k]) A.c0[o] = A.v0[k];
            A.r0[k] = rA[k];
        }
        __syncthreads();
        blk_sweep<0, false>(A); blk_sweep<1, false>(A); blk_sweep<0, false>(A); blk_sweep<1, false>(A);
    }
    MG_STAMP(13);
#pragma unroll
    for (int k = 0; k < 4; ++k) {
        const int g = min(iA + (k & 1), nxA - 1) + min(jA + (k >> 1), nyA - 1)*nxA;
        if (A.ok[k]) cor_g[g] = A.v0[k];
    }
    MG_STAMP(14);
}

struct PyrOut { double* p[5]; int nx[5], ny[5];
                double* cinv; int cinv_l; double cfx, cfy; };

__device__ __forceinline__ void acf_pyramid_block (const FView& acf0, int nx0, int ny0, const PyrOut& out, int nlev_out, unsigned long long* zero, int nzero,
                                                   int bx, int by)
{
    if (bx == 0 && by == 0) for (int q = threadIdx.x; q < nzero; q += 256) zero[q] = 0ULL;
    __shared__ double s_a[2][16*16];
    const int t = threadIdx.x;
    const int bi = bx*32, bj = by*32;
    int li = t & 15, lj = t >> 4;
    double v = 0.0;
    {
        const int i = bi + 2*li, j = bj + 2*lj;
        if (i + 1 < nx0 && j + 1 < ny0) v = 0.25*(acf0(i, j, 0) + acf0(i+1, j, 0) + acf0(i, j+1, 0) + acf0(i+1, j+1, 0));
        const int ic = (bi >> 1) + li, jc = (bj >> 1) + lj;
        if (ic < out.nx[0] && jc < out.ny[0]) {
            out.p[0][ic + (long)jc*out.nx[0]] = v;
            if (out.cinv && out.cinv_l == 0) out.cinv[ic + (long)jc*out.nx[0]] = 1.0/diag_c0<true>(ic, jc, cc_box(out.nx[0], out.ny[0]), v, out.cfx, out.cfy);
        }
        s_a[0][t] = v;
    }
    int n = 16, cur = 0;
    for (int l = 1; l < nlev_out; ++l) {
        __syncthreads();
        n >>= 1;
        if (t < n*n) {
            li = t % n; lj = t / n;
            const double* f = s_a[cur];
            const int w = 2*n;
            v = 0.25*(f[2*li + 2*lj*w] + f[2*li + 1 + 2*lj*w] + f[2*li + (2*lj + 1)*w] + f[2*li + 1 + (2*lj + 1)*w]);
            const int ic = (bi >> (l + 1)) + li, jc = (bj >> (l + 1)) + lj;
            if (ic < out.nx[l] && jc < out.ny[l]) {
                out.p[l][ic + (long)jc*out.nx[l]] = v;
                if (out.cinv && out.cinv_l == l) out.cinv[ic + (long)jc*out.nx[l]] = 1.0/diag_c0<true>(ic, jc, cc_box(out.nx[l], out.ny[l]), v, out.cfx, out.cfy);
            }
            s_a[cur ^ 1][t] = v;
        }
        cur ^= 1;
    }
}

__global__ __launch_bounds__(256)
void k_acf_pyramid (FView acf0, int nx0, int ny0, PyrOut out, int nlev_out, unsigned long long* zero, int nzero)
{
    acf_pyramid_block(acf0, nx0, ny0, out, nlev_out, zero, nzero, (int)blockIdx.x, (int)blockIdx.y);
}

__global__ __launch_bounds__(256)
void k_hierarchy_gradpsi (FView acf0, int nx0, int ny0, PyrOut out, int nlev_out, unsigned long long* zero, int nzero, int gx, int gy,
                          SlabView f, GradPsiSxSy ga, int nbx)
{
    const int b = (int)blockIdx.x;
    if (b < gx*gy) { acf_pyramid_block(acf0, nx0, ny0, out, nlev_out, zero, nzero, b % gx, b / gx); return; }
    const int q = b - gx*gy;
    const int row = q / nbx, bxs = q - row*nbx;
    gradpsi_sxsy_cell(f, ga, bxs*256 + (int)threadIdx.x - f.ng, row - f.ng);
}

constexpr int NPYR_MAX = 5, NPYR_NB = 2;
struct NodalPyr { FView lev[NPYR_MAX]; int vhx[NPYR_MAX + 1], vhy[NPYR_MAX + 1]; int np; };

template <int NP>
__global__ __launch_bounds__(256)
void k_nodal_acf_pyramid (FView f0, NodalPyr o, unsigned long long* zero, int nzero)
{
    extern __shared__ double npyr_lds[];
    constexpr int np = NP;
    const int tid = threadIdx.x;
    if (blockIdx.x == 0 && blockIdx.y == 0) for (int w = tid; w < nzero; w += 256) zero[w] = 0ULL;
    const int T0x = blockIdx.x*NPYR_NB, T0y = blockIdx.y*NPYR_NB;
    int w = NPYR_NB*(1 << np) + (1 << np) - 1;
    int lox = T0x*(1 << np) - ((1 << np) - 1), loy = T0y*(1 << np) - ((1 << np) - 1);
    double* cur = npyr_lds;
    for (int e0 = tid; e0 < w*w; e0 += 8*256) {
        double v[8];
#pragma unroll
        for (int u = 0; u < 8; ++u) {
            const int e = min(e0 + 256*u, w*w - 1);
            const int lj = e / w, li = e - lj*w;
            const int i = lox + li, j = loy + lj;
            const bool in = (i >= 1 && i <= o.vhx[0] && j >= 1 && j <= o.vhy[0]);
            const double x = f0(min(max(i, 1), o.vhx[0]), min(max(j, 1), o.vhy[0]), 0);
            v[u] = in ? x : 0.0;
        }
#pragma unroll
        for (int u = 0; u < 8; ++u) { const int e = e0 + 256*u; if (e < w*w) cur[e] = v[u]; }
    }
    __syncthreads();
#pragma unroll
    for (int l = 1; l <= np; ++l) {
        const int s = np - l;
        const int wl = NPYR_NB*(1 << s) + (1 << s) - 1;
        const int lxl = T0x*(1 << s) - ((1 << s) - 1), lyl = T0y*(1 << s) - ((1 << s) - 1);
        const int ox = T0x*(1 << s), oy = T0y*(1 << s);
        double* nxt = cur + w*w;
        const FView& out = o.lev[l - 1];
        for (int e = tid; e < wl*wl; e += 256) {
            const int lj = e / wl, li = e - lj*wl;
            const int i = lxl + li, j = lyl + lj;
            double v = 0.0;
            if (i >= 1 && i <= o.vhx[l] && j >= 1 && j <= o.vhy[l]) {
                const double* f = cur + (2*lj)*w + 2*li;
                v = (1./16.)*(f[0] + 2.*f[1] + f[2]
                            + 2.*f[w] + 4.*f[w + 1] + 2.*f[w + 2]
                            + f[2*w] + 2.*f[2*w + 1] + f[2*w + 2]);
                if (i >= ox && j >= oy) out(i, j, 0) = v;
            }
            if (l < np) nxt[e] = v;
        }
        __syncthreads();
        cur = nxt; w = wl;
    }
}
static size_t nodal_pyramid_lds (int np)
{
    size_t n = 0;
    for (int l = 0; l < np; ++l) { const int s = np - l; const size_t w = (size_t)NPYR_NB*(1 << s) + (1 << s) - 1; n += w*w; }
    return n*sizeof(double);
}

__global__ void k_level_cinv (const double* __restrict__ acf, double* __restrict__ cinv, int nx, int ny, double fx, double fy)
{
    const int i = blockIdx.x*blockDim.x + threadIdx.x, j = blockIdx.y;
    if (i < nx && j < ny) cinv[i + (long)j*nx] = 1.0/diag_c0<true>(i, j, cc_box(nx, ny), acf[i + (long)j*nx], fx, fy);
}

__global__ void k_copy2 (LevBox b, FView dst, FView src)
{
    const int i = b.vlx + blockIdx.x*blockDim.x + threadIdx.x;
    const int j = b.vly + blockIdx.y;
    if (i > b.vhx || j > b.vhy) return;
    dst(i, j, 0) = src(i, j, 0); dst(i, j, 1) = src(i, j, 1);
}

template <bool CC>
__global__ __launch_bounds__(256)
void k_bottom_sweep (LevBox b, FView cor, FView rhs, FView acf, double facx, double facy, int is, StopRule sr)
{
    if (!vcycle_active(sr)) return;
    const int i = b.vlx + blockIdx.x*blockDim.x + threadIdx.x;
    const int j = b.vly + blockIdx.y;
    if (i > b.vhx || j > b.vhy) return;
    if (is < 0) { cor(i, j, 0) = 0.0; cor(i, j, 1) = 0.0; return; }
    if ((i + j + is) & 1) return;
    const double ci = 1.0/diag_c0<CC>(i, j, b, acf(i, j, 0), facx, facy);
    for (int n = 0; n < 2; ++n) {
        const double w = (i > b.lox) ? cor(i-1, j, n) : 0.0, e = (i < b.hix) ? cor(i+1, j, n) : 0.0;
        const double s = (j > b.loy) ? cor(i, j-1, n) : 0.0, no = (j < b.hiy) ? cor(i, j+1, n) : 0.0;
        double lx = facx*(w + e), ly = facy*(s + no);
        if (CC) {
            lx = (i == b.lox) ? facx*(4./3.)*e : ((i == b.hix) ? facx*(4./3.)*w : lx);
            ly = (j == b.loy) ? facy*(4./3.)*no : ((j == b.hiy) ? facy*(4./3.)*s : ly);
        }
        cor(i, j, n) = (rhs(i, j, n) - (lx + ly))*ci;
    }
}

struct MGLevelDev { LevBox b; long cells; double *acf, *res, *cor, *rescor; };

constexpr long LOWV_MAX_CELLS = 34*34;
constexpr long SMALL_TILE_CELLS = 300L*300L;

constexpr int MG_GO_WORD = 8;
struct SolveRun { int enq, nspec, nzeroed, max_iters; double tol_rel, tol_abs; bool cc; };

struct Multigrid {
    bool cc; int nx, ny; double dx, dy;
    bool hierarchy_ready = false;
    bool nodal_pull1 = false;
    std::vector<MGLevelDev> L;
    int lowv_begin = 1;
    LowLev* d_low = nullptr; size_t low_lds = 0;
    bool bottom = false;
    unsigned long long *d_buf = nullptr, *h_buf = nullptr;
    unsigned long long* h_buf_dev = nullptr;
    long dbg_trips = 0, dbg_solves = 0, dbg_hist[8] = {0,0,0,0,0,0,0,0};
    unsigned long long* h_seq = nullptr; unsigned long long* h_seq_dev = nullptr; unsigned long long seq = 0;
    unsigned long long* d_norms = nullptr;
    unsigned long long* h_norms = nullptr;
    int last_iters = 1;
    SolveRun run{};
    bool defer_post = false; bool deferred_valid = false; MgPost deferred{};
    bool use_low3 = false; Low2 low3{}; Low2* d_low3 = nullptr; size_t low3_lds = 0;
    double* cinvA = nullptr;
    double* coef_img = nullptr;
    double* tmp0 = nullptr;
    bool cor_in_tmp = false;
    FView sol, rhs, acf0;

    ~Multigrid () {
        for (auto& l : L) { (void)hipFree(l.acf); (void)hipFree(l.res); (void)hipFree(l.cor); (void)hipFree(l.rescor); }
        if (getenv("HPS_MG_DEBUG")) fprintf(stderr, "mg: solves %ld trips %ld hist %ld %ld %ld %ld %ld %ld\n", dbg_solves, dbg_trips, dbg_hist[0], dbg_hist[1], dbg_hist[2], dbg_hist[3], dbg_hist[4], dbg_hist[5]);
        (void)hipFree(d_buf); (void)hipFree(d_low); (void)hipFree(tmp0); (void)hipFree(d_low3); (void)hipFree(cinvA); (void)hipFree(coef_img);
        if (h_buf) (void)hipHostFree(h_buf);
    }
    FView lv (int il, double* p) const {
        const MGLevelDev& l = L[il];
        const long nxb = l.b.hix - l.b.lox + 1;
        return FView{p, nxb, l.cells, -l.b.lox, -l.b.loy};
    }
    int nlev () const { return (int)L.size(); }
    bool pulls (int il) const {
        return !cc && ((il >= 2 && ((il < lowv_begin && L[il].cells <= SMALL_TILE_CELLS) ||
                                    (il == lowv_begin && !use_low3 && !bottom))) ||
                       (il == 1 && nodal_pull1));
    }
};

static size_t device_max_lds ()
{
    static const size_t lim = [] {
        int dev = 0, a = 0, b = 0;
        if (hipGetDevice(&dev) != hipSuccess) return (size_t)0;
        if (hipDeviceGetAttribute(&a, hipDeviceAttributeMaxSharedMemoryPerBlock, dev) != hipSuccess) a = 0;
        if (hipDeviceGetAttribute(&b, hipDeviceAttributeSharedMemPerBlockOptin, dev) != hipSuccess) b = 0;
        return (size_t)std::max(a, b);
    }();
    return lim;
}

int mg_create (int nx, int ny, double dx, double dy, Multigrid** out)
{
    if (nx % 2 != ny % 2) { set_error("hps_mg_create: nx and ny must have the same parity"); return HPS_ERR_ARG; }
    HPS_REQUIRE((long)(nx + 16)*(ny + 16) < (1L << 27), "hps_mg_create: the kernels address a two-component plane pair by 32-bit byte offsets (at most 2^27 cells per plane)");
    Multigrid* M = new Multigrid;
    M->cc = (nx % 2 == 0); M->nx = nx; M->ny = ny; M->dx = dx; M->dy = dy;
    int hx = M->cc ? nx - 1 : nx + 1, hy = M->cc ? ny - 1 : ny + 1;
    for (int il = 0; il < 31; ++il) {
        MGLevelDev l{};
        l.b.lox = 0; l.b.loy = 0; l.b.hix = hx; l.b.hiy = hy;
        if (M->cc) { l.b.vlx = 0; l.b.vly = 0; l.b.vhx = hx; l.b.vhy = hy; }
        else       { l.b.vlx = 1; l.b.vly = 1; l.b.vhx = hx - 1; l.b.vhy = hy - 1; }
        l.cells = (long)(hx + 1)*(hy + 1);
        HPS_HIP_CHECK(hipMalloc(&l.acf, l.cells*sizeof(double)));
        HPS_HIP_CHECK(hipMalloc(&l.res, 2*l.cells*sizeof(double)));
        HPS_HIP_CHECK(hipMalloc(&l.cor, 2*l.cells*sizeof(double)));
        HPS_HIP_CHECK(hipMalloc(&l.rescor, 2*l.cells*sizeof(double)));
        HPS_HIP_CHECK(hipMemset(l.acf, 0, l.cells*sizeof(double)));
        HPS_HIP_CHECK(hipMemset(l.res, 0, 2*l.cells*sizeof(double)));
        HPS_HIP_CHECK(hipMemset(l.cor, 0, 2*l.cells*sizeof(double)));
        HPS_HIP_CHECK(hipMemset(l.rescor, 0, 2*l.cells*sizeof(double)));
        M->L.push_back(l);
        bool ok;
        const int nxl = hx + 1, nyl = hy + 1;
        if (M->cc) { ok = nxl >= 4 && nyl >= 4 && nxl % 2 == 0 && nyl % 2 == 0; if (ok) { hx = nxl/2 - 1; hy = nyl/2 - 1; } }
        else       { ok = nxl >= 8 && nyl >= 8 && hx % 2 == 0 && hy % 2 == 0;   if (ok) { hx /= 2; hy /= 2; } }
        if (!ok) break;
    }
    if (M->nlev() < 2) { delete M; set_error("hps_mg_create: grid too small to coarsen"); return HPS_ERR_ARG; }
    if (!M->cc)
        HPS_HIP_CHECK(hipFuncSetAttribute((const void*)k_nodal_acf_pyramid<5>, hipFuncAttributeMaxDynamicSharedMemorySize, (int)nodal_pyramid_lds(NPYR_MAX)));
    const int nl = M->nlev();
    M->lowv_begin = nl - 1;
    for (int il = nl - 1; il >= 1; --il) if (M->L[il].cells <= LOWV_MAX_CELLS) M->lowv_begin = il;
    if (M->cc) {
        for (int il = 1; il < nl; ++il) {
            const LevBox& b = M->L[il].b;
            const bool fits = (b.hix + 1 <= 64) && (b.hiy + 1 <= 64) && (nl - il <= LOW2_MAXLEV)
                           && (il + 1 >= nl || (M->L[il+1].b.hix + 1 <= 32 && M->L[il+1].b.hiy + 1 <= 32));
            if (!fits) continue;
            M->use_low3 = true; M->lowv_begin = il;
            Low2& e = M->low3;
            e.nl = nl - il;
            int off3 = 0;
            for (int k = 0; k < e.nl; ++k) {
                const LevBox& bk = M->L[il + k].b;
                e.nx[k] = bk.hix + 1; e.ny[k] = bk.hiy + 1; e.off[k] = off3;
                off3 += (k == 0 ? 1 : 2)*(e.nx[k] + 2)*(e.ny[k] + 2);
            }
            e.cbase = off3; e.coff[0] = off3;
            for (int k = 1; k < e.nl; ++k) { e.coff[k] = off3; off3 += 2*(e.nx[k] + 2)*(e.ny[k] + 2); }
            e.ctot = std::max(off3 - e.cbase, 1);
            e.total = off3;
            HPS_HIP_CHECK(hipMalloc(&M->coef_img, (size_t)e.ctot*sizeof(double)));
            HPS_HIP_CHECK(hipMemset(M->coef_img, 0, (size_t)e.ctot*sizeof(double)));
            M->low3_lds = (size_t)off3*sizeof(double);
            if (M->low3_lds > 64*1024)
                HPS_HIP_CHECK(hipFuncSetAttribute((const void*)k_lower_v3, hipFuncAttributeMaxDynamicSharedMemorySize, (int)M->low3_lds));
            HPS_HIP_CHECK(hipMalloc(&M->d_low3, sizeof(Low2)));
            HPS_HIP_CHECK(hipMemcpy(M->d_low3, &e, sizeof(Low2), hipMemcpyHostToDevice));
            HPS_HIP_CHECK(hipMalloc(&M->cinvA, (size_t)e.nx[0]*e.ny[0]*sizeof(double)));
            break;
        }
    }
    if (!M->use_low3) {
        long cells = 0;
        for (int il = M->lowv_begin; il < nl; ++il) cells += M->L[il].cells;
        M->low_lds = (size_t)(8*cells)*sizeof(double);
        hipFuncAttributes fa{};
        HPS_HIP_CHECK(hipFuncGetAttributes(&fa, M->cc ? (const void*)k_lower_v<true> : (const void*)k_lower_v<false>));
        if (M->low_lds + fa.sharedSizeBytes > device_max_lds()) { M->bottom = true; M->lowv_begin = nl - 1; M->low_lds = 0; }
    }
    M->nodal_pull1 = !M->cc && M->lowv_begin > 1;
    if (!M->use_low3 && !M->bottom) {
        std::vector<LowLev> low;
        int off = 0;
        for (int il = M->lowv_begin; il < nl; ++il) {
            const MGLevelDev& l = M->L[il];
            low.push_back(LowLev{l.b, l.b.hix - l.b.lox + 1, (int)l.cells, off});
            off += 8*(int)l.cells;
        }
        if (M->low_lds > 64*1024) {
            HPS_HIP_CHECK(hipFuncSetAttribute((const void*)k_lower_v<true>, hipFuncAttributeMaxDynamicSharedMemorySize, (int)M->low_lds));
            HPS_HIP_CHECK(hipFuncSetAttribute((const void*)k_lower_v<false>, hipFuncAttributeMaxDynamicSharedMemorySize, (int)M->low_lds));
        }
        HPS_HIP_CHECK(hipMalloc(&M->d_low, low.size()*sizeof(LowLev)));
        HPS_HIP_CHECK(hipMemcpy(M->d_low, low.data(), low.size()*sizeof(LowLev), hipMemcpyHostToDevice));
    }
    HPS_HIP_CHECK(hipMalloc(&M->d_buf, (3 + MG_MAX_VCYCLES)*MG_NSUB*sizeof(unsigned long long)));
    HPS_HIP_CHECK(hipHostMalloc(&M->h_buf, ((3 + MG_MAX_VCYCLES)*MG_NSUB + 8)*sizeof(unsigned long long), hipHostMallocMapped));
    HPS_HIP_CHECK(hipHostGetDevicePointer((void**)&M->h_buf_dev, M->h_buf, 0));
    M->h_seq = M->h_buf + (3 + MG_MAX_VCYCLES)*MG_NSUB; M->h_seq_dev = M->h_buf_dev + (3 + MG_MAX_VCYCLES)*MG_NSUB;
    *M->h_seq = 0ULL;
    HPS_HIP_CHECK(hipMemset(M->d_buf, 0, (3 + MG_MAX_VCYCLES)*MG_NSUB*sizeof(unsigned long long)));
    memset(M->h_buf, 0, (3 + MG_MAX_VCYCLES)*MG_NSUB*sizeof(unsigned long long));
    M->d_norms = M->d_buf + MG_NSUB; M->h_norms = M->h_buf + MG_NSUB;
    HPS_HIP_CHECK(hipMalloc(&M->tmp0, 2*M->L[0].cells*sizeof(double)));
    HPS_HIP_CHECK(hipMemset(M->tmp0, 0, 2*M->L[0].cells*sizeof(double)));
    *out = M;
    return HPS_OK;
}

template <class TS, bool CC, int SRC, bool DO_RES, int NSW = 4, bool RPULL = false>
static void launch_smooth_ts (Multigrid* M, int il, FView phi_out, FView phi_out2, FView rhs, FView acf, FView phi_in, FView crse,
                              FView res_out, FView cres_out, unsigned long long* resnorm, unsigned long long* rhsnorm,
                              const StopRule& sr, hipStream_t st)
{
    const LevBox& b = M->L[il].b;
    constexpr int E = DO_RES ? NSW : NSW - 1;
    constexpr int FX = TS::TX - 2*E, FY = TS::TY - 2*E;
    const int ntx = ceil_div(b.vhx - b.vlx + 1, FX), nty = ceil_div(b.vhy - b.vly + 1, FY);
    const double fac = (double)(1 << il);
    const double ldx = M->dx*fac, ldy = M->dy*fac;
    const double facx = 1.0/(ldx*ldx), facy = 1.0/(ldy*ldy);
    constexpr bool FUSE = CC && DO_RES;
    hipLaunchKernelGGL((k_smooth<TS, CC, SRC, DO_RES, FUSE, NSW, RPULL>), dim3(ntx*nty), dim3(TS::NT), 0, st, b, phi_out, phi_out2, rhs, acf,
                       phi_in, crse, res_out, cres_out, facx, facy, ntx, resnorm, rhsnorm, sr);
}

template <bool CC, int SRC, bool DO_RES>
static void launch_smooth (Multigrid* M, int il, FView phi_out, FView phi_out2, FView rhs, FView acf, FView phi_in, FView crse,
                           FView res_out, FView cres_out, unsigned long long* resnorm, unsigned long long* rhsnorm,
                           const StopRule& sr, hipStream_t st)
{
    if (M->L[il].cells <= SMALL_TILE_CELLS)
        launch_smooth_ts<TileSmall, CC, SRC, DO_RES>(M, il, phi_out, phi_out2, rhs, acf, phi_in, crse, res_out, cres_out, resnorm, rhsnorm, sr, st);
    else
        launch_smooth_ts<TileBig, CC, SRC, DO_RES>(M, il, phi_out, phi_out2, rhs, acf, phi_in, crse, res_out, cres_out, resnorm, rhsnorm, sr, st);
}

template <bool CC>
static void restrict_residual_if_nodal (Multigrid* M, int il, const StopRule& sr, hipStream_t st)
{
    if (CC) return;
    const LevBox& cb = M->L[il+1].b;
    hipLaunchKernelGGL(k_restrict<CC>, dim3(ceil_div(cb.vhx - cb.vlx + 1, 64), cb.vhy - cb.vly + 1), dim3(64), 0, st,
                       cb, M->lv(il+1, M->L[il+1].res), M->lv(il, M->L[il].rescor), 2, sr);
}

template <bool CC>
static void vcycle (Multigrid* M, int k, double tol_rel, double tol_abs, hipStream_t st)
{
    const int nl = M->nlev();
    const int lb = M->lowv_begin;
    const FView none{};
    const StopRule sr{M->d_norms, k, tol_rel, tol_abs};
    for (int il = 1; il < lb; ++il) {
        if (!M->pulls(il))
            launch_smooth<CC, SRC_ZERO, true>(M, il, M->lv(il, M->L[il].cor), none, M->lv(il, M->L[il].res), M->lv(il, M->L[il].acf), none,
                                              none, M->lv(il, M->L[il].rescor), M->lv(il+1, M->L[il+1].res), nullptr, nullptr, sr, st);
        else if constexpr (!CC) {
            if (M->L[il].cells > SMALL_TILE_CELLS)
                launch_smooth_ts<TileMid, CC, SRC_ZERO, true, 4, true>(M, il, M->lv(il, M->L[il].cor), none, M->lv(il, M->L[il].res), M->lv(il, M->L[il].acf), none,
                                                                       M->lv(il-1, M->L[il-1].rescor), M->lv(il, M->L[il].rescor), M->lv(il+1, M->L[il+1].res), nullptr, nullptr, sr, st);
            else
                launch_smooth_ts<TileSmall, CC, SRC_ZERO, true, 4, true>(M, il, M->lv(il, M->L[il].cor), none, M->lv(il, M->L[il].res), M->lv(il, M->L[il].acf), none,
                                                                         M->lv(il-1, M->L[il-1].rescor), M->lv(il, M->L[il].rescor), M->lv(il+1, M->L[il+1].res), nullptr, nullptr, sr, st);
        }
        if (!M->pulls(il + 1)) restrict_residual_if_nodal<CC>(M, il, sr, st);
    }
    {
        const double fac = (double)(1 << lb);
        const double ldx = M->dx*fac, ldy = M->dy*fac;
        const LevBox& bb = M->L[nl-1].b;
        const int nsweeps = std::max(16, (std::max(bb.hix - bb.lox + 1, bb.hiy - bb.loy + 1) + 1)/2*2);
        if (M->bottom) {
            const FView cor = M->lv(lb, M->L[lb].cor), rhs = M->lv(lb, M->L[lb].res), acf = M->lv(lb, M->L[lb].acf);
            const dim3 grid(ceil_div(bb.vhx - bb.vlx + 1, 64), bb.vhy - bb.vly + 1);
            for (int is = -1; is < nsweeps; ++is)
                hipLaunchKernelGGL(k_bottom_sweep<CC>, grid, dim3(64), 0, st, bb, cor, rhs, acf, 1.0/(ldx*ldx), 1.0/(ldy*ldy), is, sr);
        } else if (M->use_low3)
            hipLaunchKernelGGL(k_lower_v3, dim3(2), dim3(1024), M->low3_lds, st, M->d_low3, M->L[lb].acf, M->cinvA, M->L[lb].res, M->L[lb].cor,
                               M->coef_img, M->low3.nx[0], M->low3.ny[0], M->low3.ctot, 1.0/(ldx*ldx), 1.0/(ldy*ldy), nsweeps, sr);
        else
            hipLaunchKernelGGL(k_lower_v<CC>, dim3(CC ? 1 : 2), dim3(1024), M->low_lds, st, M->d_low, nl - lb, M->L[lb].acf, M->L[lb].res,
                               M->L[lb].cor, 1.0/(ldx*ldx), 1.0/(ldy*ldy), nsweeps, sr, M->pulls(lb) ? M->lv(lb-1, M->L[lb-1].rescor) : FView{});
    }
    for (int il = lb - 1; il >= 1; --il) {
        double* crse = (il + 1 == lb) ? M->L[il+1].cor : M->L[il+1].rescor;
        launch_smooth<CC, SRC_PROLONG, false>(M, il, M->lv(il, M->L[il].rescor), none, M->lv(il, M->L[il].res), M->lv(il, M->L[il].acf),
                                              M->lv(il, M->L[il].cor), M->lv(il+1, crse), none, none, nullptr, nullptr, sr, st);
    }
    {
        double* crse = (1 == lb) ? M->L[1].cor : M->L[1].rescor;
        double* in = M->cor_in_tmp ? M->tmp0 : M->L[0].cor;
        double* out = M->cor_in_tmp ? M->L[0].cor : M->tmp0;
        launch_smooth_ts<typename HugeTileOf<CC>::type, CC, SRC_PROLONG, true, 8>(M, 0, M->lv(0, out), M->sol, M->rhs, M->acf0, M->lv(0, in), M->lv(1, crse),
                                                             M->lv(0, M->L[0].rescor), M->lv(1, M->L[1].res), M->d_norms + (2 + k)*MG_NSUB,
                                                             nullptr, sr, st);
        M->cor_in_tmp = !M->cor_in_tmp;
    }
    if (!M->nodal_pull1) restrict_residual_if_nodal<CC>(M, 0, sr, st);
}

__global__ __launch_bounds__(256)
void k_post_norms (const unsigned long long* __restrict__ src, volatile unsigned long long* dst, int nwords,
                   volatile unsigned long long* seq_slot, unsigned long long seq, int* go_word, StopRule after)
{
    {   const bool act = vcycle_active(after);
        if (threadIdx.x == 0) *go_word = act ? 0 : 1; }
    for (int w = threadIdx.x; w < nwords; w += blockDim.x) dst[w] = src[w];
    HPS_HOST_STORES_ACKNOWLEDGED();
    __syncthreads();
    if (threadIdx.x == 0) { *seq_slot = seq; }
}

template <bool CC>
static void enqueue_cycles (Multigrid* M, hipStream_t st)
{
    SolveRun& r = M->run;
    for (int v = 0; v < r.nspec && r.enq < r.max_iters; ++v, ++r.enq) {
        if (r.enq >= r.nzeroed) {
            const int more = std::min(r.max_iters - r.nzeroed, 64);
            (void)hipMemsetAsync(M->d_norms + (2 + r.nzeroed)*MG_NSUB, 0, more*MG_NSUB*sizeof(unsigned long long), st);
            r.nzeroed += more;
        }
        vcycle<CC>(M, r.enq, r.tol_rel, r.tol_abs, st);
    }
    ++M->seq; ++M->dbg_trips;
    if (M->defer_post) {
        M->defer_post = false; M->deferred_valid = true;
        M->deferred = MgPost{M->d_buf, (volatile unsigned long long*)M->h_buf_dev, (3 + r.enq)*MG_NSUB, (volatile unsigned long long*)M->h_seq_dev, M->seq,
                             StopRule{M->d_norms, r.enq, r.tol_rel, r.tol_abs}};
        return;
    }
    hipLaunchKernelGGL(k_post_norms, dim3(1), dim3(256), 0, st, M->d_buf, (volatile unsigned long long*)M->h_buf_dev,
                       (3 + r.enq)*MG_NSUB, (volatile unsigned long long*)M->h_seq_dev, M->seq,
                       reinterpret_cast<int*>(M->d_buf) + MG_GO_WORD, StopRule{M->d_norms, r.enq, r.tol_rel, r.tol_abs});
}

struct GuestPass { bool on = false; SlabView f{hps_slab{}}; GradPsiSxSy ga{}; };

template <bool CC>
static int solve1_hierarchy (Multigrid* M, int max_iters, hipStream_t st, const GuestPass* guest = nullptr)
{
    const int lb = M->lowv_begin;
    max_iters = std::min(max_iters, MG_MAX_VCYCLES);
    const StopRule always{nullptr, -1, 0.0, 0.0};
    int nspec = std::min(std::max(M->last_iters, 1), std::max(max_iters, 1));
    int nzeroed = std::min(max_iters, nspec + 8);
    const int nzero_words = (2 + nzeroed)*MG_NSUB;
    int first = 1;
    if (CC) {
        PyrOut po{};
        const int np = std::min(lb, 5);
        for (int il = 1; il <= np; ++il) { po.p[il-1] = M->L[il].acf; po.nx[il-1] = M->L[il].b.hix + 1; po.ny[il-1] = M->L[il].b.hiy + 1; }
        const double lfac = (double)(1 << lb), lfx = 1.0/(M->dx*lfac*M->dx*lfac), lfy = 1.0/(M->dy*lfac*M->dy*lfac);
        if (M->use_low3 && lb <= np) { po.cinv = M->cinvA; po.cinv_l = lb - 1; po.cfx = lfx; po.cfy = lfy; }
        if (guest) {
            const int gx = ceil_div(M->nx, 32), gy = ceil_div(M->ny, 32);
            const SlabView& f = guest->f;
            const int nbx = ceil_div(f.js, 256), rows = f.ny + 2*f.ng;
            hipLaunchKernelGGL(k_hierarchy_gradpsi, dim3(gx*gy + nbx*rows), dim3(256), 0, st, M->acf0, M->nx, M->ny, po, np, M->d_norms, nzero_words,
                               gx, gy, f, guest->ga, nbx);
        } else
        hipLaunchKernelGGL(k_acf_pyramid, dim3(ceil_div(M->nx, 32), ceil_div(M->ny, 32)), dim3(256), 0, st, M->acf0, M->nx, M->ny, po, np,
                           M->d_norms, nzero_words);
        first = np + 1;
    } else {
        NodalPyr o{};
        const int np = std::min(lb, NPYR_MAX);
        o.np = np;
        o.vhx[0] = M->L[0].b.vhx; o.vhy[0] = M->L[0].b.vhy;
        for (int il = 1; il <= np; ++il) { o.lev[il-1] = M->lv(il, M->L[il].acf); o.vhx[il] = M->L[il].b.vhx; o.vhy[il] = M->L[il].b.vhy; }
        const int tx = ceil_div(M->L[np].b.hix, NPYR_NB), ty = ceil_div(M->L[np].b.hiy, NPYR_NB);
        switch (np) {
            case 1: hipLaunchKernelGGL(k_nodal_acf_pyramid<1>, dim3(tx, ty), dim3(256), nodal_pyramid_lds(np), st, M->acf0, o, M->d_norms, nzero_words); break;
            case 2: hipLaunchKernelGGL(k_nodal_acf_pyramid<2>, dim3(tx, ty), dim3(256), nodal_pyramid_lds(np), st, M->acf0, o, M->d_norms, nzero_words); break;
            case 3: hipLaunchKernelGGL(k_nodal_acf_pyramid<3>, dim3(tx, ty), dim3(256), nodal_pyramid_lds(np), st, M->acf0, o, M->d_norms, nzero_words); break;
            case 4: hipLaunchKernelGGL(k_nodal_acf_pyramid<4>, dim3(tx, ty), dim3(256), nodal_pyramid_lds(np), st, M->acf0, o, M->d_norms, nzero_words); break;
            default: hipLaunchKernelGGL(k_nodal_acf_pyramid<5>, dim3(tx, ty), dim3(256), nodal_pyramid_lds(np), st, M->acf0, o, M->d_norms, nzero_words); break;
        }
        first = np + 1;
    }
    for (int il = first; il <= lb; ++il) {
        const LevBox& cb = M->L[il].b;
        FView fine = (il == 1) ? M->acf0 : M->lv(il-1, M->L[il-1].acf);
        hipLaunchKernelGGL(k_restrict<CC>, dim3(ceil_div(cb.vhx - cb.vlx + 1, 64), cb.vhy - cb.vly + 1), dim3(64), 0, st,
                           cb, M->lv(il, M->L[il].acf), fine, 1, always);
    }
    if (CC && M->use_low3 && lb > 5) {
        const double lfac = (double)(1 << lb);
        const int lnx = M->L[lb].b.hix + 1, lny = M->L[lb].b.hiy + 1;
        hipLaunchKernelGGL(k_level_cinv, dim3(ceil_div(lnx, 64), lny), dim3(64), 0, st, M->L[lb].acf, M->cinvA, lnx, lny,
                           1.0/(M->dx*lfac*M->dx*lfac), 1.0/(M->dy*lfac*M->dy*lfac));
    }
    HPS_HIP_CHECK(hipGetLastError());
    return HPS_OK;
}

template <bool CC>
static int solve1_begin (Multigrid* M, double tol_rel, double tol_abs, int max_iters, hipStream_t st)
{
    max_iters = std::min(max_iters, MG_MAX_VCYCLES);
    M->cor_in_tmp = false;
    const StopRule always{nullptr, -1, 0.0, 0.0};
    int nspec = std::min(std::max(M->last_iters, 1), std::max(max_iters, 1));
    int nzeroed = std::min(max_iters, nspec + 8);
    if (M->hierarchy_ready) M->hierarchy_ready = false;
    else if (int e = solve1_hierarchy<CC>(M, max_iters, st)) return e;
    launch_smooth<CC, SRC_DIRECT, true>(M, 0, M->lv(0, M->L[0].cor), FView{}, M->rhs, M->acf0, M->sol, FView{}, M->lv(0, M->L[0].rescor),
                                        M->lv(1, M->L[1].res), M->d_norms, M->d_norms + MG_NSUB, always, st);
    if (!M->nodal_pull1) restrict_residual_if_nodal<CC>(M, 0, always, st);
    M->run = SolveRun{0, nspec, nzeroed, max_iters, tol_rel, tol_abs, CC};
    enqueue_cycles<CC>(M, st);
    HPS_HIP_CHECK(hipGetLastError());
    return HPS_OK;
}

template <bool CC>
static int solve1_finish (Multigrid* M, int* iters_out, double* resnorm_out, int* extra, hipStream_t st)
{
    SolveRun& r = M->run;
    int status = HPS_OK;
    int iters = 0;
    double last_norm = 0.0;
    bool converged = false, diverged = false, first_trip = true;
    if (extra) *extra = 0;
    auto slot_value = [M] (int slot) {
        unsigned long long m = 0ULL;
        for (int q = 0; q < MG_NSUB; ++q) m = std::max(m, M->h_norms[slot*MG_NSUB + q]);
        double dd; memcpy(&dd, &m, 8); return dd;
    };
    while (true) {
        {   volatile unsigned long long* hs = M->h_seq;
            long spins = 0;
            while (*hs != M->seq) {
                if ((++spins & 0xfffff) == 0 && hipStreamQuery(st) != hipErrorNotReady) {
                    if (*hs == M->seq) break;
                    HPS_HIP_CHECK(hipStreamSynchronize(st));
                    if (*hs != M->seq) { set_error("hps_mg_solve1: the norm read-back never arrived"); return HPS_ERR_HIP; }
                }
            }
            __atomic_thread_fence(__ATOMIC_ACQUIRE); }
        const double res0 = slot_value(0), rhs0 = slot_value(1);
        const double max_norm = (rhs0 >= res0) ? rhs0 : res0;
        const double target = std::max(r.tol_abs, std::max(r.tol_rel, 1.e-16)*max_norm);
        last_norm = res0; iters = 0;
        converged = (res0 <= target); diverged = false;
        for (int k = 0; k < r.enq && !converged && !diverged; ++k) {
            last_norm = slot_value(2 + k); ++iters;
            if (last_norm <= target) converged = true;
            else if (!(last_norm <= 1.e20*max_norm)) diverged = true;
        }
        if (first_trip) {
            const double prev = (r.enq == 0) ? res0 : slot_value(2 + r.enq - 1);
            const bool gate_active = prev > target && prev <= 1.e20*max_norm;
            if (gate_active != !(converged || diverged)) { set_error("hps_mg_solve1: host and device stopping rules disagree"); return HPS_ERR_HIP; }
            if (extra) *extra = gate_active ? 1 : 0;
            first_trip = false;
        }
        if (converged || diverged) break;
        if (r.enq >= r.max_iters) { set_error("hps_mg_solve1: not converged after max_iters V-cycles"); status = HPS_ERR_MG_MAXITER; break; }
        r.nspec = 1;
        enqueue_cycles<CC>(M, st);
    }
    if (diverged) { set_error("hps_mg_solve1: diverging"); status = HPS_ERR_MG_DIVERGED; }
    M->last_iters = std::max(1, iters); ++M->dbg_solves; ++M->dbg_hist[std::min(iters, 7)];
    if (iters == 0) {
        const LevBox& b0 = M->L[0].b;
        hipLaunchKernelGGL(k_copy2, dim3(ceil_div(b0.vhx - b0.vlx + 1, 64), b0.vhy - b0.vly + 1), dim3(64), 0, st,
                           b0, M->sol, M->lv(0, M->L[0].cor));
    }
    HPS_HIP_CHECK(hipGetLastError());
    if (iters_out) *iters_out = iters;
    if (resnorm_out) *resnorm_out = last_norm;
    return status;
}

static void set_views (Multigrid* M, const hps_slab& s, int sol_comp, int rhs_comp, int acf_comp)
{
    const int sh = M->cc ? 0 : 1;
    const int o = s.ng - sh;
    M->sol  = FView{s.p + (long)sol_comp*s.nstride, s.jstride, s.nstride, o, o};
    M->rhs  = FView{s.p + (long)rhs_comp*s.nstride, s.jstride, s.nstride, o, o};
    M->acf0 = FView{s.p + (long)acf_comp*s.nstride, s.jstride, s.nstride, o, o};
}

int mg_solve1_begin (void* handle, hps_slab s, int sol_comp, int rhs_comp, int acf_comp, double tol_rel, double tol_abs,
                     int max_iters, hipStream_t st)
{
    Multigrid* M = static_cast<Multigrid*>(handle);
    HPS_REQUIRE(s.nstride < (1L << 27) && s.ng <= 8, "mg_solve1_begin: planes of at most 2^27 doubles and at most 8 guard cells (32-bit byte offsets in the kernels)");
    set_views(M, s, sol_comp, rhs_comp, acf_comp);
    return M->cc ? solve1_begin<true>(M, tol_rel, tol_abs, max_iters, st) : solve1_begin<false>(M, tol_rel, tol_abs, max_iters, st);
}
int mg_solve1_prepare (void* handle, hps_slab s, int sol_comp, int rhs_comp, int acf_comp, int max_iters, hipStream_t st)
{
    Multigrid* M = static_cast<Multigrid*>(handle);
    set_views(M, s, sol_comp, rhs_comp, acf_comp);
    if (int e = M->cc ? solve1_hierarchy<true>(M, max_iters, st) : solve1_hierarchy<false>(M, max_iters, st)) return e;
    M->hierarchy_ready = true;
    return HPS_OK;
}
int mg_solve1_prepare_with (void* handle, hps_slab s, int sol_comp, int rhs_comp, int acf_comp, int max_iters, SlabView f, GradPsiSxSy ga,
                            hipStream_t st, bool* done)
{
    Multigrid* M = static_cast<Multigrid*>(handle);
    *done = false;
    if (!M->cc) return HPS_OK;
    set_views(M, s, sol_comp, rhs_comp, acf_comp);
    GuestPass g; g.on = true; g.f = f; g.ga = ga;
    if (int e = solve1_hierarchy<true>(M, max_iters, st, &g)) return e;
    M->hierarchy_ready = true;
    *done = true;
    return HPS_OK;
}
void mg_solve1_forget_hierarchy (void* handle) { if (handle) static_cast<Multigrid*>(handle)->hierarchy_ready = false; }
void mg_defer_post (void* handle) { Multigrid* M = static_cast<Multigrid*>(handle); M->defer_post = true; M->deferred_valid = false; }
bool mg_take_deferred_post (void* handle, MgPost* out)
{
    Multigrid* M = static_cast<Multigrid*>(handle);
    M->defer_post = false;
    if (!M->deferred_valid) return false;
    M->deferred_valid = false; *out = M->deferred;
    return true;
}
const int* mg_gate_after_enqueued (void* handle)
{
    return reinterpret_cast<const int*>(static_cast<Multigrid*>(handle)->d_buf) + MG_GO_WORD;
}
bool mg_solve1_ready (void* handle)
{
    Multigrid* M = static_cast<Multigrid*>(handle);
    return *(volatile unsigned long long*)M->h_seq == M->seq;
}
int mg_solve1_finish (void* handle, int* iters_out, double* resnorm_out, int* extra, hipStream_t st)
{
    Multigrid* M = static_cast<Multigrid*>(handle);
    return M->cc ? solve1_finish<true>(M, iters_out, resnorm_out, extra, st) : solve1_finish<false>(M, iters_out, resnorm_out, extra, st);
}

int mg_solve1 (Multigrid* M, hps_slab s, int sol_comp, int rhs_comp, int acf_comp, double tol_rel, double tol_abs,
               int max_iters, int* iters_out, double* resnorm_out, hipStream_t st)
{
    if (int e = mg_solve1_begin(M, s, sol_comp, rhs_comp, acf_comp, tol_rel, tol_abs, max_iters, st)) return e;
    return mg_solve1_finish(M, iters_out, resnorm_out, nullptr, st);
}

}

using namespace hps;

extern "C" int hps_mg_create (int nx, int ny, double dx, double dy, void** handle)
{
    HPS_REQUIRE(nx >= 2 && ny >= 2 && handle, "hps_mg_create: bad size");
    Multigrid* M = nullptr;
    if (int e = mg_create(nx, ny, dx, dy, &M)) return e;
    *handle = M;
    return HPS_OK;
}

extern "C" int hps_mg_info (void* handle, int* cc, int* nlev, int* lowv_begin, int* lowv_kind, long* lowv_lds, int* tiles,
                            int* nodal_pull1, int* pyr_levels, int* pyr_restricts)
{
    HPS_REQUIRE(handle, "hps_mg_info: null handle");
    const Multigrid* M = static_cast<const Multigrid*>(handle);
    const int lb = M->lowv_begin;
    if (cc) *cc = M->cc;
    if (nlev) *nlev = M->nlev();
    if (lowv_begin) *lowv_begin = lb;
    if (lowv_kind) *lowv_kind = M->bottom ? HPS_MG_LOWV_BOTTOM : M->use_low3 ? HPS_MG_LOWV_V3 : M->cc ? HPS_MG_LOWV_CC : HPS_MG_LOWV_NODAL;
    if (lowv_lds) *lowv_lds = (long)(M->use_low3 ? M->low3_lds : M->low_lds);
    if (tiles) {
        for (int il = 0; il < HPS_MG_MAXLEV; ++il) {
            int t = -1;
            if (il < lb) {
                const bool small = M->L[il].cells <= SMALL_TILE_CELLS;
                t = M->pulls(il) ? (small ? HPS_MG_TILE_SMALL_PULL : HPS_MG_TILE_MID_PULL) : (small ? HPS_MG_TILE_SMALL : HPS_MG_TILE_BIG);
            }
            tiles[il] = t;
        }
    }
    if (nodal_pull1) *nodal_pull1 = M->nodal_pull1;
    if (pyr_levels) *pyr_levels = std::min(lb, M->cc ? 5 : NPYR_MAX);
    if (pyr_restricts) *pyr_restricts = lb - std::min(lb, M->cc ? 5 : NPYR_MAX);
    return HPS_OK;
}

extern "C" int hps_mg_solve1 (void* handle, hps_slab slab, int sol_comp, int rhs_comp, int acoef_comp, double tol_rel,
                              double tol_abs, int max_iters, int* iters_host, double* resnorm_host, hps_stream stream)
{
    HPS_REQUIRE(handle && slab.p, "hps_mg_solve1: null argument");
    Multigrid* M = static_cast<Multigrid*>(handle);
    HPS_REQUIRE(slab.nx == M->nx && slab.ny == M->ny, "hps_mg_solve1: slab size does not match the solver");
    HPS_REQUIRE(sol_comp >= 0 && sol_comp + 1 < slab.ncomp && rhs_comp >= 0 && rhs_comp + 1 < slab.ncomp &&
                acoef_comp >= 0 && acoef_comp < slab.ncomp, "hps_mg_solve1: bad component");
    HPS_REQUIRE(M->cc || slab.ng >= 1, "hps_mg_solve1: node-centred solve needs >= 1 guard cell");
    HPS_REQUIRE(slab.nstride < (1L << 27) && slab.ng <= 8, "hps_mg_solve1: planes of at most 2^27 doubles and at most 8 guard cells (32-bit byte offsets in the kernels)");
    return mg_solve1(M, slab, sol_comp, rhs_comp, acoef_comp, tol_rel, tol_abs, max_iters, iters_host, resnorm_host,
                     (hipStream_t)stream);
}

extern "C" int hps_mg_solve1_fabs (void* handle, hps_slab sol2, hps_slab rhs2, hps_slab acoef1, double tol_rel, double tol_abs,
                                   int max_iters, int* iters_host, double* resnorm_host, hps_stream stream)
{
    HPS_REQUIRE(handle && sol2.p && rhs2.p && acoef1.p, "hps_mg_solve1_fabs: null argument");
    Multigrid* M = static_cast<Multigrid*>(handle);
    for (const hps_slab* s : {&sol2, &rhs2, &acoef1}) {
        HPS_REQUIRE(s->nx == M->nx && s->ny == M->ny, "hps_mg_solve1_fabs: view size does not match the solver");
        HPS_REQUIRE(M->cc || s->ng >= 1, "hps_mg_solve1_fabs: node-centred solve needs >= 1 guard cell in every view");
    }
    HPS_REQUIRE(sol2.ncomp >= 2 && rhs2.ncomp >= 2 && acoef1.ncomp >= 1, "hps_mg_solve1_fabs: sol and rhs need two components, acoef one");
    const int sh = M->cc ? 0 : 1;
    HPS_REQUIRE(sol2.nstride < (1L << 27) && rhs2.nstride < (1L << 27) && acoef1.nstride < (1L << 27), "hps_mg_solve1_fabs: planes of at most 2^27 doubles (32-bit byte offsets in the kernels)");
    M->sol  = FView{sol2.p, sol2.jstride, sol2.nstride, sol2.ng - sh, sol2.ng - sh};
    M->rhs  = FView{rhs2.p, rhs2.jstride, rhs2.nstride, rhs2.ng - sh, rhs2.ng - sh};
    M->acf0 = FView{acoef1.p, acoef1.jstride, acoef1.nstride, acoef1.ng - sh, acoef1.ng - sh};
    hipStream_t st = (hipStream_t)stream;
    if (int e = M->cc ? solve1_begin<true>(M, tol_rel, tol_abs, max_iters, st) : solve1_begin<false>(M, tol_rel, tol_abs, max_iters, st)) return e;
    return mg_solve1_finish(M, iters_host, resnorm_host, nullptr, st);
}

void mg_rider (void* handle, int** dev_words, const int** host_words)
{
    Multigrid* M = static_cast<Multigrid*>(handle);
    *dev_words = reinterpret_cast<int*>(M->d_buf);
    *host_words = reinterpret_cast<const int*>(M->h_buf);
}

extern "C" int hps_mg_debug_stamps (long long* stamps16_host)
{
#ifndef HPS_STAMPS
    (void)stamps16_host; set_error("hps_mg_debug_stamps: the library was built without -DHPS_STAMPS (make stamps)"); return HPS_ERR_UNSUPPORTED;
#else
    static long long* d = nullptr;
    if (!d) {
        HPS_HIP_CHECK(hipMalloc(&d, 48*sizeof(long long)));
        HPS_HIP_CHECK(hipMemset(d, 0, 48*sizeof(long long)));
        HPS_HIP_CHECK(hipMemcpyToSymbol(HIP_SYMBOL(g_mg_dbg), &d, sizeof(d)));
        return HPS_OK;
    }
    HPS_HIP_CHECK(hipDeviceSynchronize());
    HPS_HIP_CHECK(hipMemcpy(stamps16_host, d, 48*sizeof(long long), hipMemcpyDeviceToHost));
    return HPS_OK;
#endif
}

extern "C" int hps_mg_destroy (void* handle)
{
    delete static_cast<Multigrid*>(handle);
    return HPS_OK;
}
```

include/hpslice.h:

```cpp
#ifndef HPSLICE_H_
#define HPSLICE_H_

#include <stdint.h>

#ifdef __cplusplus
extern "C" {
#endif

typedef void* hps_stream;

enum { HPS_OK = 0, HPS_ERR_ARG = 1, HPS_ERR_HIP = 2, HPS_ERR_FFT = 3, HPS_ERR_MG_DIVERGED = 4,
       HPS_ERR_MG_MAXITER = 5, HPS_ERR_COMM = 6, HPS_ERR_UNSUPPORTED = 7 };

enum { HPS_BC_REFLECTING = 0, HPS_BC_PERIODIC = 1, HPS_BC_ABSORBING = 2 };

typedef struct {
    double* p;
    int nx, ny, ng, ncomp;
    long jstride, nstride;
} hps_slab;

typedef struct {
    double *x, *y, *w, *ux, *uy, *psi, *x_prev, *y_prev, *ux_half, *uy_half, *psi_half;
    uint64_t* idcpu;
    int32_t* ion_lev;
    long n;
} hps_plasma;
#define HPS_ID_VALID (1ULL << 63)

typedef struct {
    double dx, dy, dz;
    double xoff, yoff;
    double c, ep0, mu0, q_e, m_e;
    double plo[2], phi[2];
    int bc;
    int normalized;
} hps_geom;

const char* hps_last_error (void);
const char* hps_version (void);


int hps_deposit_current (hps_slab slab, hps_plasma plasma, hps_geom geom, const int comp[6],
                         double charge, double mass, int depos_order, double max_qsa_weighting,
                         int can_ionize, int* n_qsa_violation, hps_stream stream);

int hps_explicit_deposit (hps_slab slab, hps_plasma plasma, hps_geom geom, const int cache[4],
                          const int depos[2], double charge, double mass, int depos_order,
                          int derivative_type, int can_ionize, hps_stream stream);

int hps_advance_plasma (hps_slab slab, hps_plasma plasma, hps_geom geom, const int comp[5],
                        double charge, double mass, int depos_order, int temp_slice,
                        int n_subcycles, int can_ionize, hps_stream stream);

int hps_deposit_current_laser (hps_slab slab, hps_plasma plasma, hps_geom geom, const int comp[6], int aabs_comp,
                               double charge, double mass, int depos_order, double max_qsa_weighting,
                               int can_ionize, int* n_qsa_violation, hps_stream stream);
int hps_explicit_deposit_laser (hps_slab slab, hps_plasma plasma, hps_geom geom, const int cache[4], int aabs_comp,
                                const int depos[2], double charge, double mass, int depos_order,
                                int derivative_type, int can_ionize, hps_stream stream);
int hps_advance_plasma_laser (hps_slab slab, hps_plasma plasma, hps_geom geom, const int comp[5], int aabs_comp,
                              double charge, double mass, int depos_order, int temp_slice,
                              int n_subcycles, int can_ionize, hps_stream stream);


int hps_tiling_create (int nx, int ny, int tile_size, long max_particles, void** handle);
int hps_reorder_particles (void* tiling, hps_plasma src, hps_plasma dst, hps_geom geom,
                           hps_stream stream);
int hps_tiling_info (void* tiling, int* ntiles, const int** offsets_dev, const unsigned int** perm_dev);
int hps_tiling_destroy (void* tiling);

int hps_beam_sort_by_box (const double* z_dev, long n, double plo_z, double dz, int num_boxes,
                          unsigned long long* counts_dev, unsigned long long* offsets_dev,
                          unsigned long long* perm_dev, hps_stream stream);

int hps_deposit_current_tiled (hps_slab slab, hps_plasma plasma, hps_geom geom, const int comp[6],
                               double charge, double mass, int depos_order, double max_qsa_weighting,
                               int can_ionize, int* n_qsa_violation, void* tiling, int* n_fallback,
                               hps_stream stream);
int hps_explicit_deposit_tiled (hps_slab slab, hps_plasma plasma, hps_geom geom, const int cache[4],
                                const int depos[2], double charge, double mass, int depos_order,
                                int derivative_type, int can_ionize, void* tiling, int* n_fallback,
                                hps_stream stream);
int hps_advance_plasma_tiled (hps_slab slab, hps_plasma plasma, hps_geom geom, const int comp[5],
                              double charge, double mass, int depos_order, int temp_slice,
                              int n_subcycles, int can_ionize, void* tiling, int* n_fallback,
                              hps_stream stream);
int hps_deposit_current_tiled_laser (hps_slab slab, hps_plasma plasma, hps_geom geom, const int comp[6], int aabs_comp,
                                     double charge, double mass, int depos_order, double max_qsa_weighting,
                                     int can_ionize, int* n_qsa_violation, void* tiling, int* n_fallback,
                                     hps_stream stream);
int hps_explicit_deposit_tiled_laser (hps_slab slab, hps_plasma plasma, hps_geom geom, const int cache[4], int aabs_comp,
                                      const int depos[2], double charge, double mass, int depos_order,
                                      int derivative_type, int can_ionize, void* tiling, int* n_fallback,
                                      hps_stream stream);
int hps_advance_plasma_tiled_laser (hps_slab slab, hps_plasma plasma, hps_geom geom, const int comp[5], int aabs_comp,
                                    double charge, double mass, int depos_order, int temp_slice,
                                    int n_subcycles, int can_ionize, void* tiling, int* n_fallback,
                                    hps_stream stream);
int hps_tiling_set_validity (void* tiling, int by_weight, int by_psi_half);

int hps_particles_record (int on);
int hps_particles_recorded (char* buf, long cap, long* len);


int hps_poisson_create (int nx, int ny, double dx, double dy, void** handle);
int hps_poisson_solve (void* handle, const double* staging, hps_slab dst, int dst_comp,
                       hps_stream stream);
int hps_poisson_solve_batch (void* handle, int nbatch, const double* staging, hps_slab dst,
                             const int* dst_comps, hps_stream stream);
enum { HPS_POISSON_OWN_SYM = 0, HPS_POISSON_OWN_POW2 = 1, HPS_POISSON_DENSE = 2, HPS_POISSON_ROCFFT = 3 };
int hps_poisson_info (void* handle, int* backend, int* x_len, int* tri_rows);
int hps_poisson_destroy (void* handle);

int hps_mg_create (int nx, int ny, double dx, double dy, void** handle);
int hps_mg_solve1 (void* handle, hps_slab slab, int sol_comp, int rhs_comp, int acoef_comp,
                   double tol_rel, double tol_abs, int max_iters, int* iters_host,
                   double* resnorm_host, hps_stream stream);
int hps_mg_solve1_fabs (void* handle, hps_slab sol2, hps_slab rhs2, hps_slab acoef1, double tol_rel, double tol_abs,
                        int max_iters, int* iters_host, double* resnorm_host, hps_stream stream);
enum { HPS_MG_LOWV_V3 = 0, HPS_MG_LOWV_CC = 1, HPS_MG_LOWV_NODAL = 2, HPS_MG_LOWV_BOTTOM = 3 };
enum { HPS_MG_TILE_SMALL = 0, HPS_MG_TILE_BIG = 1, HPS_MG_TILE_SMALL_PULL = 2, HPS_MG_TILE_MID_PULL = 3 };
enum { HPS_MG_MAXLEV = 31 };
int hps_mg_info (void* handle, int* cc, int* nlev, int* lowv_begin, int* lowv_kind, long* lowv_lds, int* tiles,
                 int* nodal_pull1, int* pyr_levels, int* pyr_restricts);
int hps_mg_destroy (void* handle);

int hps_mg2_create (int nx, int ny, double dx, double dy, void** handle);
int hps_mg2_solve2 (void* handle, double* sol2_dev, const double* rhs2_dev, const double* acoef_real_dev,
                    const double* acoef_imag_dev, double tol_rel, double tol_abs, int max_iters, int* iters_host,
                    double* resnorm_host, hps_stream stream);
enum { HPS_MG2_BOTTOM_LOWER_V = 0, HPS_MG2_BOTTOM_SINGLE_BLOCK = 1, HPS_MG2_BOTTOM_PER_SWEEP = 2 };
enum { HPS_MG2_TILE_SINGLE_BLOCK = 0, HPS_MG2_TILE_SMALL = 1, HPS_MG2_TILE_BIG = 2 };
int hps_mg2_info (void* handle, int* nlev, int* low_top, int* bottom, int* tiles);
int hps_mg2_destroy (void* handle);


#define HPS_MAX_ION_LEVELS 56
typedef struct {
    int nx, ny, nz; double lo[3], hi[3];
    int order; int deriv_type;
    int plasma_ppc[2]; double plasma_density; double plasma_radius;
    double plasma_charge, plasma_mass; double max_qsa; int n_subcycles;
    int beam_profile;
    double beam_zmin, beam_zmax, beam_radius, beam_density;
    double beam_umean[3], beam_pos_mean[3], beam_pos_std[3]; int beam_ppc[3]; double beam_charge;
    int bc; double mg_tol_rel, mg_tol_abs; int deposit_rho; int n_steps;
    double dt; int beam_n_subcycles; double beam_mass; double ext_E_slope[2];
    int bxby_solver; double predcorr_tol; int predcorr_max_iter; double predcorr_mix; int field_bc;
    int laser_on; double laser_a0, laser_w0, laser_L0, laser_lambda0, laser_pos[3];
    double laser_zfoc; int laser_solver; int laser_use_phase;
    int si_units;
    int grid_current_on; double grid_current_peak, grid_current_mean[3], grid_current_std[3];
    double laser_mg_tol_rel, laser_mg_tol_abs;
    int beam_radiation_reaction; double background_density_SI; int beam_no_z_push;
    int plasma_no_neutralize;
    int ion_on; int ion_ppc[2]; double ion_density, ion_mass, ion_charge; int ion_init_level, ion_Z;
    double ion_energies[HPS_MAX_ION_LEVELS]; unsigned long long ion_seed;
    int beam_spin_tracking; double beam_initial_spin[3]; double beam_spin_anom;
    int dt_adaptive; double nt_per_betatron, dt_max, adaptive_threshold_uz, adaptive_phase_tolerance;
    int adaptive_no_predict_step, adaptive_no_phase_control, adaptive_phase_substeps;
    double adaptive_density, max_time, beam_uz_std;
    double ext_Ez_slope;
    int beam_do_salame; int salame_n_iter; double salame_relative_tolerance; int salame_no_advance;
    double salame_Ez_target_slope;
} hps_deck;

enum { HPS_SAL_EZ_TARGET = 0, HPS_SAL_EZ_NO_SALAME, HPS_SAL_EZ, HPS_SAL_JX, HPS_SAL_JY, HPS_SAL_JZB, HPS_SAL_BX, HPS_SAL_BY,
       HPS_SAL_SY, HPS_SAL_SX, HPS_SAL_SY_BACK, HPS_SAL_SX_BACK, HPS_SAL_NCOMP };

enum { HPS_C_N_JXB = 0, HPS_C_N_JYB, HPS_C_CHI, HPS_C_SY, HPS_C_SX, HPS_C_EXMBY, HPS_C_EYPBX,
       HPS_C_EZ, HPS_C_BX, HPS_C_BY, HPS_C_BZ, HPS_C_PSI, HPS_C_JXB, HPS_C_JYB, HPS_C_JZB,
       HPS_C_JX, HPS_C_JY, HPS_C_RHOMJZ, HPS_C_P_JXB, HPS_C_P_JYB, HPS_C_ION_RHOMJZ, HPS_C_RHO,
       HPS_NCOMP_MAX };

enum { HPS_PC_N_JX = 0, HPS_PC_N_JY, HPS_PC_EXMBY, HPS_PC_EYPBX, HPS_PC_EZ, HPS_PC_BX, HPS_PC_BY, HPS_PC_BZ,
       HPS_PC_PSI, HPS_PC_JX, HPS_PC_JY, HPS_PC_JZ, HPS_PC_RHOMJZ, HPS_PC_P_BX, HPS_PC_P_BY, HPS_PC_P_JX,
       HPS_PC_P_JY, HPS_PC_ION_RHOMJZ, HPS_PC_IT_BX, HPS_PC_IT_BY, HPS_PC_PIT_BX, HPS_PC_PIT_BY, HPS_PC_RHO,
       HPS_PC_NCOMP_MAX };

int hps_engine_create (const hps_deck* deck, int device, void** handle);
int hps_engine_destroy (void* handle);
int hps_engine_begin_step (void* handle);
int hps_engine_set_step (void* handle, int step);
int hps_engine_set_time (void* handle, double t, double dt);
int hps_engine_beam_moments (void* handle, double* out4_host);
int hps_engine_solve_slice (void* handle, int islice);
int hps_engine_solve_slice_begin (void* handle, int islice);
int hps_engine_solve_slice_finish (void* handle, int islice);
int hps_engine_slice_ready (void* handle);
int hps_engine_run_step (void* handle);
int hps_engine_sync (void* handle);
int hps_engine_info (void* handle, int* ncomp, int* nguards, long* nparticles);
hps_slab hps_engine_slab (void* handle);
hps_plasma hps_engine_plasma (void* handle);
int hps_engine_tiling (void* handle, void** tiling);
hps_plasma hps_engine_ions (void* handle);
int hps_engine_ion_stats (void* handle, long* n_ionized_host, long* n_product_host);
hps_stream hps_engine_stream (void* handle);
int hps_engine_checksums (void* handle, double* out_host);
int hps_engine_stats (void* handle, long* total_vcycles, long* slices_done);
int hps_engine_pc_stats (void* handle, long* iterations, double* error_sum);
int hps_engine_pc_zero_b_slices (void* handle, long* slices);
int hps_engine_laser_info (void* handle, int* aabs_comp, double* envelope_abs_sum_host);
int hps_engine_laser_envelope (void* handle, double* out_host);
int hps_engine_set_laser_import (void* handle, int on, int step);
int hps_engine_export_laser_slice (void* handle, int islice, double* msg_dev);
int hps_engine_import_laser_slice (void* handle, int islice, const double* msg_dev);
int hps_engine_import_laser_from (void* handle, int islice, void* src_engine);
int hps_engine_set_diagnostics (void* handle, int on);
int hps_engine_set_field_diagnostic (void* handle, int ncomps, const int* comps, const int coarsening[3]);
int hps_engine_field_diagnostic (void* handle, double* out_host);
int hps_engine_set_field_diagnostic_box (void* handle, int ncomps, const int* comps, const int coarsening[3], int slice_dir,
                                         const double* patch_lo , const double* patch_hi );
int hps_engine_field_diagnostic_geometry (void* handle, int* n3, double* lo3, double* hi3);

int hps_engine_set_insitu_fields (void* handle, int on);
int hps_engine_insitu_fields (void* handle, double* out_host );

int hps_engine_set_insitu_plasma (void* handle, double radius);
int hps_engine_laser_vcycles (void* handle, long* vcycles);
int hps_engine_set_insitu_beam (void* handle, double radius);
int hps_engine_insitu_beam (void* handle, double* out_host );
int hps_engine_insitu_plasma (void* handle, double* out_host );

int hps_engine_set_tiling (void* handle, int tile_size, int sort_period);
int hps_engine_fallbacks (void* handle, long* n_fallback_host);
int hps_engine_set_density_profile (void* handle, int nr, const double* r_host, const double* fr_host, int nt,
                                    const double* ct_host, const double* ft_host);
int hps_engine_set_fusion (void* handle, int on);
int hps_engine_sorts (void* handle, long* n_sorts_host);
int hps_engine_set_profiling (void* handle, int on);
int hps_engine_set_profiling_stride (void* handle, int stride);
int hps_engine_phase_times (void* handle, double* ms_host, long* nslices_host);

int hps_engine_beam_info (void* handle, long* nbeam_host, long* offsets_host );
int hps_engine_set_beam_particles (void* handle, long n, const double* soa_host, long* n_outside);
int hps_engine_set_beam_storage (void* handle, double* storage_dev );
int hps_engine_initial_beam (void* handle, double* dst_dev);
int hps_engine_beam_state (void* handle, long* boundaries_host, double* soa_host);
int hps_engine_beam_capacity (void* handle, long* cap_host);
int hps_engine_set_beam_capacity (void* handle, long cap);
int hps_engine_beam_message_rows (void* handle, int* rows_host);
int hps_engine_beam_spin (void* handle, double* soa_host);
int hps_engine_set_beam_import (void* handle, int on);
int hps_engine_export_beam_slice (void* handle, int islice, double* msg_dev);
int hps_engine_import_beam_slice (void* handle, int islice, const double* msg_dev);
int hps_engine_assume_initial_beam_support (void* handle);

int hps_engine_record_event (void* handle, int slot, void** event_out);
int hps_stream_pool_shared_pairs (int device);
int hps_engine_wait_event (void* handle, void* event);
int hps_engine_copy_async (void* handle, void* dst_dev, const void* src_dev, long bytes);

int hps_engine_salame_stats (void* handle, double* out_host );
int hps_salame_only_advance (hps_slab slab, hps_plasma plasma, hps_geom geom, int bx_comp, int by_comp, double charge,
                             double mass, int depos_order, int can_ionize, hps_stream stream);
int hps_salame_jxjy_from_bxby (hps_slab slab, hps_geom geom, int bx_comp, int by_comp, int chi_comp, int jx_comp, int jy_comp,
                               hps_stream stream);
int hps_salame_sxsy_from_jz (hps_slab slab, hps_geom geom, int jz_comp, int sy_comp, int sx_comp, hps_stream stream);
int hps_salame_get_w (hps_slab slab, int ez_target_comp, int ez_no_salame_comp, int ez_comp, int jz_comp, double* scratch_dev,
                      double* out4_host, hps_stream stream);
int hps_salame_scale_beam_slice (double* w_dev, long n, double W, hps_stream stream);

int hps_adaptive_create (const hps_deck* deck, void** handle);
int hps_adaptive_set_density_profile (void* handle, int nr, const double* r_host, const double* fr_host, int nt,
                                      const double* ct_host, const double* ft_host);
int hps_adaptive_initial_dt (void* handle, double uz_mean, double uz_std, int nstages, double* dt_host);
int hps_adaptive_before_step (void* handle, double t, double* dt_host);
int hps_adaptive_next_time (void* handle, double* t_next_host);
int hps_adaptive_after_step (void* handle, const double* moments4_host, double t, int nstages, double* dt_host);
int hps_adaptive_destroy (void* handle);

#define HPS_RING_ID_BYTES 128
int hps_ring_unique_id (char* id_out );
int hps_ring_init (int rank, int world, int device, const char* id_edge_in, const char* id_edge_out, void** ring);
int hps_ring_send_slice (void* ring, const void* msg_dev, long bytes, void* after_event, int slot, void** done_event);
int hps_ring_recv_slice (void* ring, void* msg_dev, long bytes, void* after_event, int slot, void** done_event);
int hps_ring_sendrecv_self (void* ring, const void* src_dev, void* dst_dev, long bytes, void* after_event, int slot,
                            void** done_event);
int hps_ring_stream_wait (void* ring, int which, void* event);
int hps_ring_sync_sends (void* ring);
int hps_ring_sync (void* ring);
int hps_ring_sync_timeout (void* ring, double seconds);
int hps_ring_stats (void* ring, long* n_sent, long* n_received, long long* bytes_sent, long long* bytes_received);
int hps_ring_info (void* ring, int* world, int* comm_in_ranks, int* comm_out_ranks, int* my_rank_in, int* my_rank_out);
int hps_ring_destroy (void* ring);
int hps_ring_edge_kind (void* ring);
int hps_ring_can_send (void* ring);
int hps_ring_recv_landed (void* ring, void* done_event);
int hps_ring_engine_wait (void* ring, void* engine, void* done_event);

int hps_collide_plasma (hps_plasma a, void* tiling_a, hps_plasma b, void* tiling_b, hps_geom geom, int nx, int ny,
                        double charge_a, double mass_a, int can_ionize_a, double charge_b, double mass_b, int can_ionize_b,
                        double coulomb_log, double background_density_SI, unsigned long long seed, int collision,
                        int step, int islice, long* pairs_collided_host, long* overfull_cells_host, hps_stream stream);
#define HPS_MAX_COLLISIONS 8
int hps_engine_add_collision (void* handle, int species_a, int species_b, double coulomb_log, unsigned long long seed);
typedef struct {
    double *x, *y, *z, *ux, *uy, *uz, *w;
    int32_t* nsub;
    long n;
} hps_beam_slice;
int hps_collide_beam_plasma (hps_beam_slice beam, hps_plasma plasma, hps_geom geom, int nx, int ny, double charge_beam,
                             double mass_beam, double charge_plasma, double mass_plasma, int can_ionize_plasma,
                             double coulomb_log, double background_density_SI, unsigned long long seed, int collision,
                             int step, int islice, double dt, long* pairs_collided_host, long* overfull_cells_host,
                             hps_stream stream);
int hps_engine_add_beam_collision (void* handle, int plasma_species, double coulomb_log, unsigned long long seed);
int hps_engine_collision_stats (void* handle, long* pairs_collided, long* overfull_cells);

int hps_memcpy_d2h (void* dst_host, const void* src_dev, long bytes);
int hps_memcpy_h2d (void* dst_dev, const void* src_host, long bytes);
int hps_device_count (int* n_host);

#ifdef __cplusplus
}
#endif
#endif
```

Before: 1652.

## Split multigrid smoother components across a second grid dimension on small levels

Adds a SPLIT mode to the multigrid smoother kernel. On levels whose workgroup count is small relative to the CU count, the two solution components are handled by separate workgroups (grid.y = 2), each holding one component in LDS. The aim is to fill idle CUs on the coarser down-leg levels and to cut per-workgroup LDS and register use. The cost is duplicate loads of the shared coefficient and a second launch dimension. The mode can be disabled with an environment variable, and extra debug stamp filtering is added.

```diff
diff --git a/hipace_amd/_lib.py b/hipace_amd/_lib.py
--- a/hipace_amd/_lib.py
+++ b/hipace_amd/_lib.py
@@ -128,6 +128,7 @@
                                      C.POINTER(C.c_int), C.POINTER(C.c_double), C.c_void_p]),
     "hps_mg_info": (C.c_int, [C.c_void_p, C.POINTER(C.c_int), C.POINTER(C.c_int), C.POINTER(C.c_int), C.POINTER(C.c_int),
                               C.POINTER(C.c_long), C.POINTER(C.c_int), C.POINTER(C.c_int), C.POINTER(C.c_int), C.POINTER(C.c_int)]),
+    "hps_mg_split_info": (C.c_int, [C.c_void_p, C.POINTER(C.c_int), C.POINTER(C.c_int)]),
     "hps_mg_destroy": (C.c_int, [C.c_void_p]),
     "hps_mg2_create": (C.c_int, [C.c_int, C.c_int, C.c_double, C.c_double, C.POINTER(C.c_void_p)]),
     "hps_mg2_solve2": (C.c_int, [C.c_void_p, C.c_void_p, C.c_void_p, C.c_void_p, C.c_void_p, C.c_double, C.c_double, C.c_int,
diff --git a/hipace_amd/api.py b/hipace_amd/api.py
--- a/hipace_amd/api.py
+++ b/hipace_amd/api.py
@@ -318,6 +318,11 @@
         return {"cc": bool(cc.value), "nlev": nl.value, "lowv_begin": lb.value, "lowv": self.LOWV[kind.value],
                 "lowv_lds": lds.value, "tiles": tuple(self.TILES[v] for v in t if v >= 0), "nodal_pull1": bool(pull1.value),
                 "pyramid": npyr.value, "restricts": nres.value}
+
+    def split_levels(self):
+        t, ncu = (C.c_int * 31)(), C.c_int()
+        check(_lib.lib().hps_mg_split_info(self._h, t, C.byref(ncu)))
+        return tuple(bool(v) for v in t if v >= 0)
 
     def solve1(self, fields, sol_comp, rhs_comp, acoef_comp, tol_rel=1e-4, tol_abs=2.2250738585072014e-308,
                nummaxiter=200):
diff --git a/hipace_amd/csrc/multigrid.hip b/hipace_amd/csrc/multigrid.hip
--- a/hipace_amd/csrc/multigrid.hip
+++ b/hipace_amd/csrc/multigrid.hip
@@ -27,9 +27,12 @@
 
 #ifdef HPS_STAMPS
 __device__ long long* g_mg_dbg = nullptr;
-#define MG_STAMP(i) do { if (g_mg_dbg && blockIdx.x == 0 && threadIdx.x == 0) g_mg_dbg[i] = __builtin_amdgcn_s_memtime(); } while (0)
+#define MG_STAMP(i) do { if (g_mg_dbg && blockIdx.x == 0 && blockIdx.y == 0 && threadIdx.x == 0) g_mg_dbg[i] = __builtin_amdgcn_s_memtime(); } while (0)
+__device__ int g_mg_dbg_hix = -1, g_mg_dbg_res = -1;
+#define MG_STAMP_T(i) do { if ((g_mg_dbg_hix < 0 || b.hix == g_mg_dbg_hix) && (g_mg_dbg_res < 0 || (int)DO_RES == g_mg_dbg_res)) MG_STAMP(i); } while (0)
 #else
 #define MG_STAMP(i) do { } while (0)
+#define MG_STAMP_T(i) do { } while (0)
 #endif
 
 template <int TX_, int TY_, int NT_>
@@ -136,8 +139,8 @@
 
 #define MG_ROWPK(m) const int jj = BR ? (tid / PR)*GPAIRS + (m) : (tid + MG_NT*(m)) / PR, pk = BR ? (tid & (PR - 1)) : (tid + MG_NT*(m)) - jj*PR
 template <bool CC> __device__ __forceinline__ double restrict_at (const FView& fine, int i, int j, int n);
-template <class TS, bool CC, int SRC, bool DO_RES, bool FUSE_R, bool INTERIOR, int NSW, bool GATE_IN = (NSW == 4), bool RPULL = false>
-__device__ __forceinline__ void smooth_tile (double (&s_phi)[2][TS::AY*TS::AX], double* s_red, double* s_crs, const LevBox& b, const FView& phi_out,
+template <class TS, bool CC, int SRC, bool DO_RES, bool FUSE_R, bool INTERIOR, int NSW, bool GATE_IN = (NSW == 4), bool RPULL = false, bool SPLIT = false>
+__device__ __forceinline__ void smooth_tile (double (&s_phi)[SPLIT ? 1 : 2][TS::AY*TS::AX], double* s_red, double* s_crs, const LevBox& b, const FView& phi_out,
                                              const FView& phi_out2, const FView& rhs, const FView& acf, const FView& phi_in, const FView& crse,
                                              const FView& res_out, const FView& cres_out, double facx, double facy,
                                              int gi0, int gj0, unsigned long long* resnorm, unsigned long long* rhsnorm, const StopRule& sr)
@@ -146,9 +149,11 @@
     constexpr int GT_X = TS::TX, GT_Y = TS::TY, GA_X = TS::AX, GA_Y = TS::AY, MG_NT = TS::NT, GPAIRS = TS::GPAIRS, PR = TS::PR;
     constexpr int AXH = GA_X/2, CH = GA_Y*AXH;
     constexpr bool BR = GPAIRS <= 2 || INTERIOR;
+    constexpr bool C1 = !SPLIT;
+    constexpr int K1 = SPLIT ? 0 : 1;
     const int tid = threadIdx.x;
     const int cpar = (gi0 + gj0) & 1;
-    MG_STAMP(0);
+    MG_STAMP_T(0);
     double r0[GPAIRS][2], r1[GPAIRS][2], ac[GPAIRS][2], ci[GPAIRS][2];
     bool in[GPAIRS][2];
     int hx[GPAIRS];
@@ -168,8 +173,8 @@
             const bool ok = INTERIOR || (ic == i && jc == j);
             in[m][p] = ok;
             double a0, a1;
-            if constexpr (RPULL) { a0 = restrict_at<CC>(crse, ic, jc, 0); a1 = restrict_at<CC>(crse, ic, jc, 1); }
-            else { a0 = rhs(ic, jc, 0); a1 = rhs(ic, jc, 1); }
+            if constexpr (RPULL) { a0 = restrict_at<CC>(crse, ic, jc, 0); a1 = C1 ? restrict_at<CC>(crse, ic, jc, 1) : 0.0; }
+            else { a0 = rhs(ic, jc, 0); a1 = C1 ? rhs(ic, jc, 1) : 0.0; }
             const double a2 = acf(ic, jc, 0);
             r0[m][p] = ok ? a0 : 0.0;
             r1[m][p] = ok ? a1 : 0.0;
@@ -178,7 +183,7 @@
             if (rhsnorm) rmax = fmax(rmax, fmax(fabs(r0[m][p]), fabs(r1[m][p])));
         }
     }
-    MG_STAMP(1);
+    MG_STAMP_T(1);
     {
         constexpr int NF = (GA_X*GA_Y + MG_NT - 1)/MG_NT;
         double v0[NF], v1[NF];
@@ -194,12 +199,12 @@
                 const int q = min(tid + MG_NT*m, CXN*CYN - 1);
                 const int ly = q / CXN, lx = q - ly*CXN;
                 const int X = min(max(cx0 + lx, cxl), cxh), Y = min(max(cy0 + ly, cyl), cyh);
-                c0[m] = crse(X, Y, 0); c1[m] = crse(X, Y, 1);
+                c0[m] = crse(X, Y, 0); c1[m] = C1 ? crse(X, Y, 1) : 0.0;
             }
 #pragma unroll
             for (int m = 0; m < NC; ++m) {
                 const int q = tid + MG_NT*m;
-                if (q < CXN*CYN) { s_crs[q] = c0[m]; s_crs[CXN*CYN + q] = c1[m]; }
+                if (q < CXN*CYN) { s_crs[q] = c0[m]; if (C1) s_crs[CXN*CYN + q] = c1[m]; }
             }
         }
 #pragma unroll
@@ -210,8 +215,8 @@
             v0[m] = 0.0; v1[m] = 0.0;
             if (SRC != SRC_ZERO) {
                 const int ic = INTERIOR ? i : min(max(i, b.vlx), b.vhx), jc = INTERIOR ? j : min(max(j, b.vly), b.vhy);
-                double a0 = phi_in(ic, jc, 0), a1 = phi_in(ic, jc, 1);
-                if (SRC == SRC_PROLONG && !PLDS) { a0 += prolong_at<CC>(crse, ic, jc, 0); a1 += prolong_at<CC>(crse, ic, jc, 1); }
+                double a0 = phi_in(ic, jc, 0), a1 = C1 ? phi_in(ic, jc, 1) : 0.0;
+                if (SRC == SRC_PROLONG && !PLDS) { a0 += prolong_at<CC>(crse, ic, jc, 0); if (C1) a1 += prolong_at<CC>(crse, ic, jc, 1); }
                 const bool inside = INTERIOR || (ic == i && jc == j);
                 v0[m] = inside ? a0 : 0.0; v1[m] = inside ? a1 : 0.0;
             }
@@ -228,21 +233,21 @@
                 const int o = ((jc >> 1) - cy0)*CXN + (ic >> 1) - cx0;
                 const bool io = (ic & 1), jo = (jc & 1);
                 double p0, p1;
-                const double* q0 = s_crs + o; const double* q1 = s_crs + CXN*CYN + o;
+                const double* q0 = s_crs + o; const double* q1 = s_crs + K1*CXN*CYN + o;
                 if (io && jo)  { p0 = (q0[0] + q0[1] + q0[CXN] + q0[CXN + 1])*0.25; p1 = (q1[0] + q1[1] + q1[CXN] + q1[CXN + 1])*0.25; }
                 else if (io)   { p0 = (q0[0] + q0[1])*0.5; p1 = (q1[0] + q1[1])*0.5; }
                 else if (jo)   { p0 = (q0[0] + q0[CXN])*0.5; p1 = (q1[0] + q1[CXN])*0.5; }
                 else           { p0 = q0[0]; p1 = q1[0]; }
-                if (inside) { v0[m] += p0; v1[m] += p1; }
+                if (inside) { v0[m] += p0; if (C1) v1[m] += p1; }
             }
         }
         {
             if (GATE_IN) {
                 const bool active = vcycle_active(sr);
 #pragma unroll
-                for (int m = 0; m < GPAIRS; ++m) { HPS_KEEP(r0[m][0]); HPS_KEEP(r0[m][1]); HPS_KEEP(r1[m][0]); HPS_KEEP(r1[m][1]); HPS_KEEP(ac[m][0]); HPS_KEEP(ac[m][1]); }
-#pragma unroll
-                for (int m = 0; m < NF; ++m) { HPS_KEEP(v0[m]); HPS_KEEP(v1[m]); }
+                for (int m = 0; m < GPAIRS; ++m) { HPS_KEEP(r0[m][0]); HPS_KEEP(r0[m][1]); if (C1) { HPS_KEEP(r1[m][0]); HPS_KEEP(r1[m][1]); } HPS_KEEP(ac[m][0]); HPS_KEEP(ac[m][1]); }
+#pragma unroll
+                for (int m = 0; m < NF; ++m) { HPS_KEEP(v0[m]); if (C1) HPS_KEEP(v1[m]); }
                 if (!active) return;
             }
         }
@@ -252,12 +257,12 @@
             if (s < GA_X*GA_Y) {
                 const int lj = s / GA_X, li = s - lj*GA_X;
                 const int o = ((cpar + li + lj) & 1)*CH + lj*AXH + (li >> 1);
-                s_phi[0][o] = v0[m]; s_phi[1][o] = v1[m];
+                s_phi[0][o] = v0[m]; if (C1) s_phi[K1][o] = v1[m];
             }
         }
     }
     __syncthreads();
-    MG_STAMP(2);
+    MG_STAMP_T(2);
 
     double l0[GPAIRS][2], l1[GPAIRS][2];
     if constexpr (BR) {
@@ -266,7 +271,7 @@
             MG_ROWPK(m);
             const int row = (jj + 1)*AXH + pk;
 #pragma unroll
-            for (int p = 0; p < 2; ++p) { const int h = hx[m] ^ p; l0[m][p] = s_phi[0][p*CH + row + h]; l1[m][p] = s_phi[1][p*CH + row + h]; }
+            for (int p = 0; p < 2; ++p) { const int h = hx[m] ^ p; l0[m][p] = s_phi[0][p*CH + row + h]; l1[m][p] = C1 ? s_phi[K1][p*CH + row + h] : 0.0; }
         }
 #pragma unroll
         for (int icolor = 0; icolor < NSW; ++icolor) {
@@ -277,15 +282,16 @@
                 const int h = hx[m] ^ p;
                 const int row = (jj + 1)*AXH + pk;
                 const double* nb0 = &s_phi[0][(1 - p)*CH + row];
-                const double* nb1 = &s_phi[1][(1 - p)*CH + row];
+                const double* nb1 = &s_phi[K1][(1 - p)*CH + row];
                 const double we0 = nb0[h] + l0[m][1 - p], we1 = nb1[h] + l1[m][1 - p];
                 const double s0 = (m > 0) ? l0[m > 0 ? m - 1 : 0][1 - p] : nb0[h - AXH], s1 = (m > 0) ? l1[m > 0 ? m - 1 : 0][1 - p] : nb1[h - AXH];
                 const double t0 = (m + 1 < GPAIRS) ? l0[m + 1 < GPAIRS ? m + 1 : m][1 - p] : nb0[h + AXH], t1 = (m + 1 < GPAIRS) ? l1[m + 1 < GPAIRS ? m + 1 : m][1 - p] : nb1[h + AXH];
                 const double n0 = (r0[m][p] - (fxm[m][p]*we0 + fym[m]*(s0 + t0)))*ci[m][p];
-                const double n1 = (r1[m][p] - (fxm[m][p]*we1 + fym[m]*(s1 + t1)))*ci[m][p];
-                if (INTERIOR || in[m][p]) { s_phi[0][p*CH + row + h] = n0; s_phi[1][p*CH + row + h] = n1; l0[m][p] = n0; l1[m][p] = n1; }
+                const double n1 = C1 ? (r1[m][p] - (fxm[m][p]*we1 + fym[m]*(s1 + t1)))*ci[m][p] : 0.0;
+                if (INTERIOR || in[m][p]) { s_phi[0][p*CH + row + h] = n0; l0[m][p] = n0; if (C1) { s_phi[K1][p*CH + row + h] = n1; l1[m][p] = n1; } }
             }
             __syncthreads();
+            if (icolor < 4) MG_STAMP_T(44 + icolor);
         }
     } else {
 #pragma unroll
@@ -298,15 +304,16 @@
                 const int h = hx[m] ^ p;
                 const int row = (jj + 1)*AXH + pk;
                 const double* nb0 = &s_phi[0][(1 - p)*CH + row];
-                const double* nb1 = &s_phi[1][(1 - p)*CH + row];
+                const double* nb1 = &s_phi[K1][(1 - p)*CH + row];
                 const double n0 = (r0[m][p] - (fxm[m][p]*(nb0[0] + nb0[1]) + fym[m]*(nb0[h - AXH] + nb0[h + AXH])))*ci[m][p];
-                const double n1 = (r1[m][p] - (fxm[m][p]*(nb1[0] + nb1[1]) + fym[m]*(nb1[h - AXH] + nb1[h + AXH])))*ci[m][p];
-                if (INTERIOR || in[m][p]) { s_phi[0][p*CH + row + h] = n0; s_phi[1][p*CH + row + h] = n1; }
+                const double n1 = C1 ? (r1[m][p] - (fxm[m][p]*(nb1[0] + nb1[1]) + fym[m]*(nb1[h - AXH] + nb1[h + AXH])))*ci[m][p] : 0.0;
+                if (INTERIOR || in[m][p]) { s_phi[0][p*CH + row + h] = n0; if (C1) s_phi[K1][p*CH + row + h] = n1; }
             }
             __syncthreads();
-        }
-    }
-    MG_STAMP(3);
+            if (icolor < 4) MG_STAMP_T(44 + icolor);
+        }
+    }
+    MG_STAMP_T(3);
 
     double resmax = 0.0;
     if constexpr (BR) {
@@ -330,23 +337,23 @@
                 q0[p] = 0.0; q1[p] = 0.0;
                 if (DO_RES) {
                     const double* nb0 = &s_phi[0][(1 - p)*CH + row];
-                    const double* nb1 = &s_phi[1][(1 - p)*CH + row];
+                    const double* nb1 = &s_phi[K1][(1 - p)*CH + row];
                     const double o0 = nb0[h], o1 = nb1[h];
                     const double w0 = h ? l0[m][1 - p] : o0, e0 = h ? o0 : l0[m][1 - p];
                     const double w1 = h ? l1[m][1 - p] : o1, e1 = h ? o1 : l1[m][1 - p];
                     const double s0 = (m > 0) ? l0[m > 0 ? m - 1 : 0][1 - p] : nb0[h - AXH], s1 = (m > 0) ? l1[m > 0 ? m - 1 : 0][1 - p] : nb1[h - AXH];
                     const double n0 = (m + 1 < GPAIRS) ? l0[m + 1 < GPAIRS ? m + 1 : m][1 - p] : nb0[h + AXH], n1 = (m + 1 < GPAIRS) ? l1[m + 1 < GPAIRS ? m + 1 : m][1 - p] : nb1[h + AXH];
                     const double t0 = residual_v<INTERIOR>(f0, w0, e0, s0, n0, i, j, b, r0[m][p], ac[m][p], facx, facy);
-                    const double t1 = residual_v<INTERIOR>(f1, w1, e1, s1, n1, i, j, b, r1[m][p], ac[m][p], facx, facy);
+                    const double t1 = C1 ? residual_v<INTERIOR>(f1, w1, e1, s1, n1, i, j, b, r1[m][p], ac[m][p], facx, facy) : 0.0;
                     q0[p] = fin[p] ? t0 : 0.0; q1[p] = fin[p] ? t1 : 0.0;
                     resmax = fmax(resmax, fmax(fabs(q0[p]), fabs(q1[p])));
                 }
                 if (fin[p]) {
-                    if constexpr (RPULL) { rhs(i, j, 0) = r0[m][p]; rhs(i, j, 1) = r1[m][p]; }
-                    if (DO_RES && !FUSE_R) { res_out(i, j, 0) = q0[p]; res_out(i, j, 1) = q1[p]; }
+                    if constexpr (RPULL) { rhs(i, j, 0) = r0[m][p]; if (C1) rhs(i, j, 1) = r1[m][p]; }
+                    if (DO_RES && !FUSE_R) { res_out(i, j, 0) = q0[p]; if (C1) res_out(i, j, 1) = q1[p]; }
                     phi_out(i, j, 0) = f0;
-                    phi_out(i, j, 1) = f1;
-                    if (phi_out2.p) { phi_out2(i, j, 0) = f0; phi_out2(i, j, 1) = f1; }
+                    if (C1) phi_out(i, j, 1) = f1;
+                    if (phi_out2.p) { phi_out2(i, j, 0) = f0; if (C1) phi_out2(i, j, 1) = f1; }
                 }
             }
             const bool sw = (hx[m] != 0);
@@ -366,7 +373,7 @@
                     const double ua0 = own ? la0[mu] : c0, ub0 = own ? ra0[mu] : d0, ua1 = own ? la1[mu] : c1, ub1 = own ? ra1[mu] : d1;
                     const int ic = (gi0 + 2*pk) >> 1, jc = (gj0 + jj) >> 1;
                     cres_out(ic, jc, 0) = 0.25*(la0[m] + ra0[m] + ua0 + ub0);
-                    cres_out(ic, jc, 1) = 0.25*(la1[m] + ra1[m] + ua1 + ub1);
+                    if (C1) cres_out(ic, jc, 1) = 0.25*(la1[m] + ra1[m] + ua1 + ub1);
                 }
             }
         }
@@ -385,22 +392,22 @@
                 fin[p] = rowok && ii >= E && ii < GT_X - E && in[m][p];
                 const int i = gi0 + ii;
                 const int row = (jj + 1)*AXH + pk;
-                const double f0 = s_phi[0][p*CH + row + h], f1 = s_phi[1][p*CH + row + h];
+                const double f0 = s_phi[0][p*CH + row + h], f1 = C1 ? s_phi[K1][p*CH + row + h] : 0.0;
                 q0[p] = 0.0; q1[p] = 0.0;
                 if (DO_RES) {
                     const double* nb0 = &s_phi[0][(1 - p)*CH + row];
-                    const double* nb1 = &s_phi[1][(1 - p)*CH + row];
+                    const double* nb1 = &s_phi[K1][(1 - p)*CH + row];
                     const double t0 = residual_v<INTERIOR>(f0, nb0[0], nb0[1], nb0[h - AXH], nb0[h + AXH], i, j, b, r0[m][p], ac[m][p], facx, facy);
-                    const double t1 = residual_v<INTERIOR>(f1, nb1[0], nb1[1], nb1[h - AXH], nb1[h + AXH], i, j, b, r1[m][p], ac[m][p], facx, facy);
+                    const double t1 = C1 ? residual_v<INTERIOR>(f1, nb1[0], nb1[1], nb1[h - AXH], nb1[h + AXH], i, j, b, r1[m][p], ac[m][p], facx, facy) : 0.0;
                     q0[p] = fin[p] ? t0 : 0.0; q1[p] = fin[p] ? t1 : 0.0;
                     resmax = fmax(resmax, fmax(fabs(q0[p]), fabs(q1[p])));
                 }
                 if (fin[p]) {
-                    if constexpr (RPULL) { rhs(i, j, 0) = r0[m][p]; rhs(i, j, 1) = r1[m][p]; }
-                    if (DO_RES && !FUSE_R) { res_out(i, j, 0) = q0[p]; res_out(i, j, 1) = q1[p]; }
+                    if constexpr (RPULL) { rhs(i, j, 0) = r0[m][p]; if (C1) rhs(i, j, 1) = r1[m][p]; }
+                    if (DO_RES && !FUSE_R) { res_out(i, j, 0) = q0[p]; if (C1) res_out(i, j, 1) = q1[p]; }
                     phi_out(i, j, 0) = f0;
-                    phi_out(i, j, 1) = f1;
-                    if (phi_out2.p) { phi_out2(i, j, 0) = f0; phi_out2(i, j, 1) = f1; }
+                    if (C1) phi_out(i, j, 1) = f1;
+                    if (phi_out2.p) { phi_out2(i, j, 0) = f0; if (C1) phi_out2(i, j, 1) = f1; }
                 }
             }
             if (FUSE_R) {
@@ -412,30 +419,32 @@
                 if (fin[0] && ((tid & PR) == 0)) {
                     const int ic = (gi0 + 2*pk) >> 1, jc = j >> 1;
                     cres_out(ic, jc, 0) = 0.25*(la0 + ra0 + c0 + d0);
-                    cres_out(ic, jc, 1) = 0.25*(la1 + ra1 + c1 + d1);
+                    if (C1) cres_out(ic, jc, 1) = 0.25*(la1 + ra1 + c1 + d1);
                 }
             }
         }
     }
-    MG_STAMP(4);
+    MG_STAMP_T(4);
     if (DO_RES && resnorm) block_max_to<MG_NT>(resnorm, resmax, s_red);
     if (rhsnorm) block_max_to<MG_NT>(rhsnorm, rmax, s_red);
-    MG_STAMP(5);
-}
-
-template <class TS, bool CC, int SRC, bool DO_RES, bool FUSE_R, int NSW = 4, bool RPULL = false>
+    MG_STAMP_T(5);
+}
+
+template <class TS, bool CC, int SRC, bool DO_RES, bool FUSE_R, int NSW = 4, bool RPULL = false, bool SPLIT = false>
 __global__ __launch_bounds__(TS::NT, (RPULL && TS::GPAIRS > 1) ? 2 : 4)
 void k_smooth (LevBox b, FView phi_out, FView phi_out2, FView rhs, FView acf, FView phi_in, FView crse, FView res_out,
                FView cres_out, double facx, double facy, int ntx, unsigned long long* resnorm,
                unsigned long long* rhsnorm, StopRule sr)
 {
     static_assert(!FUSE_R || (CC && DO_RES), "fused restriction is cell-centred only");
+    static_assert(!SPLIT || NSW == 4, "one component per workgroup: the 4-sweep kernels of the mid levels only");
     if (NSW != 4 && !vcycle_active(sr)) return;
     constexpr int GT_X = TS::TX, GT_Y = TS::TY;
-    __shared__ double s_phi[2][TS::AY*TS::AX];
+    constexpr int NC = SPLIT ? 1 : 2;
+    __shared__ double s_phi[NC][TS::AY*TS::AX];
     __shared__ double s_red[TS::NT/64];
     constexpr bool PLDS = !CC && SRC == SRC_PROLONG;
-    __shared__ double s_crs[PLDS ? 2*(TS::AX/2 + 2)*(TS::AY/2 + 2) : 1];
+    __shared__ double s_crs[PLDS ? NC*(TS::AX/2 + 2)*(TS::AY/2 + 2) : 1];
     constexpr int E = DO_RES ? NSW : NSW - 1;
     constexpr int FX = GT_X - 2*E, FY = GT_Y - 2*E;
     const int nb = gridDim.x, q8 = nb >> 3, r8 = nb & 7, xcd = blockIdx.x & 7;
@@ -446,9 +455,19 @@
     const bool interior = (gi0 - 1 >= b.vlx) && (gi0 + GT_X <= b.vhx) && (gj0 - 1 >= b.vly) && (gj0 + GT_Y <= b.vhy)
                        && (gi0 > b.lox) && (gi0 + GT_X - 1 < b.hix) && (gj0 > b.loy) && (gj0 + GT_Y - 1 < b.hiy);
     constexpr bool GATE_IN = (NSW == 4);
-    if (interior) smooth_tile<TS, CC, SRC, DO_RES, FUSE_R, true, NSW, GATE_IN, RPULL>(s_phi, s_red, s_crs, b, phi_out, phi_out2, rhs, acf, phi_in, crse, res_out, cres_out,
+    if constexpr (SPLIT) {
+        const long n = blockIdx.y;
+        if (phi_out.p) phi_out.p += n*phi_out.ns;
+        if (phi_out2.p) phi_out2.p += n*phi_out2.ns;
+        if (rhs.p) rhs.p += n*rhs.ns;
+        if (phi_in.p) phi_in.p += n*phi_in.ns;
+        if (crse.p) crse.p += n*crse.ns;
+        if (res_out.p) res_out.p += n*res_out.ns;
+        if (cres_out.p) cres_out.p += n*cres_out.ns;
+    }
+    if (interior) smooth_tile<TS, CC, SRC, DO_RES, FUSE_R, true, NSW, GATE_IN, RPULL, SPLIT>(s_phi, s_red, s_crs, b, phi_out, phi_out2, rhs, acf, phi_in, crse, res_out, cres_out,
                                                              facx, facy, gi0, gj0, resnorm, rhsnorm, sr);
-    else          smooth_tile<TS, CC, SRC, DO_RES, FUSE_R, false, NSW, GATE_IN, RPULL>(s_phi, s_red, s_crs, b, phi_out, phi_out2, rhs, acf, phi_in, crse, res_out, cres_out,
+    else          smooth_tile<TS, CC, SRC, DO_RES, FUSE_R, false, NSW, GATE_IN, RPULL, SPLIT>(s_phi, s_red, s_crs, b, phi_out, phi_out2, rhs, acf, phi_in, crse, res_out, cres_out,
                                                               facx, facy, gi0, gj0, resnorm, rhsnorm, sr);
 }
 
@@ -1289,6 +1308,17 @@
         return FView{p, nxb, l.cells, -l.b.lox, -l.b.loy};
     }
     int nlev () const { return (int)L.size(); }
+    int num_cus = 0; bool split_comps = true;
+    bool small_tile (int il) const { return L[il].cells <= SMALL_TILE_CELLS; }
+    int down_leg_wgs (int il) const {
+        const LevBox& b = L[il].b;
+        const int tx = small_tile(il) ? 32 : (pulls(il) ? 32 : 64), ty = small_tile(il) ? 16 : 32;
+        return ceil_div(b.vhx - b.vlx + 1, tx - 8)*ceil_div(b.vhy - b.vly + 1, ty - 8);
+    }
+    bool split (int il) const {
+        if (pulls(il) && !small_tile(il)) return false;
+        return split_comps && il >= 1 && il < lowv_begin && 2*down_leg_wgs(il) <= num_cus;
+    }
     bool pulls (int il) const {
         return !cc && ((il >= 2 && ((il < lowv_begin && L[il].cells <= SMALL_TILE_CELLS) ||
                                     (il == lowv_begin && !use_low3 && !bottom))) ||
@@ -1404,13 +1434,20 @@
     HPS_HIP_CHECK(hipMemset(M->d_buf, 0, (3 + MG_MAX_VCYCLES)*MG_NSUB*sizeof(unsigned long long)));
     memset(M->h_buf, 0, (3 + MG_MAX_VCYCLES)*MG_NSUB*sizeof(unsigned long long));
     M->d_norms = M->d_buf + MG_NSUB; M->h_norms = M->h_buf + MG_NSUB;
+    {
+        int dev = 0;
+        HPS_HIP_CHECK(hipGetDevice(&dev));
+        HPS_HIP_CHECK(hipDeviceGetAttribute(&M->num_cus, hipDeviceAttributeMultiprocessorCount, dev));
+        const char* e = getenv("HPS_MG_SPLIT_COMPS");
+        if (e && *e) M->split_comps = atoi(e) != 0;
+    }
     HPS_HIP_CHECK(hipMalloc(&M->tmp0, 2*M->L[0].cells*sizeof(double)));
     HPS_HIP_CHECK(hipMemset(M->tmp0, 0, 2*M->L[0].cells*sizeof(double)));
     *out = M;
     return HPS_OK;
 }
 
-template <class TS, bool CC, int SRC, bool DO_RES, int NSW = 4, bool RPULL = false>
+template <class TS, bool CC, int SRC, bool DO_RES, int NSW = 4, bool RPULL = false, bool SPLIT = false>
 static void launch_smooth_ts (Multigrid* M, int il, FView phi_out, FView phi_out2, FView rhs, FView acf, FView phi_in, FView crse,
                               FView res_out, FView cres_out, unsigned long long* resnorm, unsigned long long* rhsnorm,
                               const StopRule& sr, hipStream_t st)
@@ -1423,7 +1460,7 @@
     const double ldx = M->dx*fac, ldy = M->dy*fac;
     const double facx = 1.0/(ldx*ldx), facy = 1.0/(ldy*ldy);
     constexpr bool FUSE = CC && DO_RES;
-    hipLaunchKernelGGL((k_smooth<TS, CC, SRC, DO_RES, FUSE, NSW, RPULL>), dim3(ntx*nty), dim3(TS::NT), 0, st, b, phi_out, phi_out2, rhs, acf,
+    hipLaunchKernelGGL((k_smooth<TS, CC, SRC, DO_RES, FUSE, NSW, RPULL, SPLIT>), dim3(ntx*nty, SPLIT ? 2 : 1), dim3(TS::NT), 0, st, b, phi_out, phi_out2, rhs, acf,
                        phi_in, crse, res_out, cres_out, facx, facy, ntx, resnorm, rhsnorm, sr);
 }
 
@@ -1432,7 +1469,16 @@
                            FView res_out, FView cres_out, unsigned long long* resnorm, unsigned long long* rhsnorm,
                            const StopRule& sr, hipStream_t st)
 {
-    if (M->L[il].cells <= SMALL_TILE_CELLS)
+    if constexpr (SRC != SRC_DIRECT) {
+        if (M->split(il)) {
+            if (M->small_tile(il))
+                launch_smooth_ts<TileSmall, CC, SRC, DO_RES, 4, false, true>(M, il, phi_out, phi_out2, rhs, acf, phi_in, crse, res_out, cres_out, resnorm, rhsnorm, sr, st);
+            else
+                launch_smooth_ts<TileBig, CC, SRC, DO_RES, 4, false, true>(M, il, phi_out, phi_out2, rhs, acf, phi_in, crse, res_out, cres_out, resnorm, rhsnorm, sr, st);
+            return;
+        }
+    }
+    if (M->small_tile(il))
         launch_smooth_ts<TileSmall, CC, SRC, DO_RES>(M, il, phi_out, phi_out2, rhs, acf, phi_in, crse, res_out, cres_out, resnorm, rhsnorm, sr, st);
     else
         launch_smooth_ts<TileBig, CC, SRC, DO_RES>(M, il, phi_out, phi_out2, rhs, acf, phi_in, crse, res_out, cres_out, resnorm, rhsnorm, sr, st);
@@ -1459,12 +1505,14 @@
             launch_smooth<CC, SRC_ZERO, true>(M, il, M->lv(il, M->L[il].cor), none, M->lv(il, M->L[il].res), M->lv(il, M->L[il].acf), none,
                                               none, M->lv(il, M->L[il].rescor), M->lv(il+1, M->L[il+1].res), nullptr, nullptr, sr, st);
         else if constexpr (!CC) {
-            if (M->L[il].cells > SMALL_TILE_CELLS)
-                launch_smooth_ts<TileMid, CC, SRC_ZERO, true, 4, true>(M, il, M->lv(il, M->L[il].cor), none, M->lv(il, M->L[il].res), M->lv(il, M->L[il].acf), none,
-                                                                       M->lv(il-1, M->L[il-1].rescor), M->lv(il, M->L[il].rescor), M->lv(il+1, M->L[il+1].res), nullptr, nullptr, sr, st);
-            else
-                launch_smooth_ts<TileSmall, CC, SRC_ZERO, true, 4, true>(M, il, M->lv(il, M->L[il].cor), none, M->lv(il, M->L[il].res), M->lv(il, M->L[il].acf), none,
-                                                                         M->lv(il-1, M->L[il-1].rescor), M->lv(il, M->L[il].rescor), M->lv(il+1, M->L[il+1].res), nullptr, nullptr, sr, st);
+            const FView cor = M->lv(il, M->L[il].cor), res = M->lv(il, M->L[il].res), acf = M->lv(il, M->L[il].acf);
+            const FView fres = M->lv(il-1, M->L[il-1].rescor), rescor = M->lv(il, M->L[il].rescor), cres = M->lv(il+1, M->L[il+1].res);
+            if (!M->small_tile(il))
+                launch_smooth_ts<TileMid, CC, SRC_ZERO, true, 4, true>(M, il, cor, none, res, acf, none, fres, rescor, cres, nullptr, nullptr, sr, st);
+            else {
+                if (M->split(il)) launch_smooth_ts<TileSmall, CC, SRC_ZERO, true, 4, true, true>(M, il, cor, none, res, acf, none, fres, rescor, cres, nullptr, nullptr, sr, st);
+                else              launch_smooth_ts<TileSmall, CC, SRC_ZERO, true, 4, true>(M, il, cor, none, res, acf, none, fres, rescor, cres, nullptr, nullptr, sr, st);
+            }
         }
         if (!M->pulls(il + 1)) restrict_residual_if_nodal<CC>(M, il, sr, st);
     }
@@ -1787,6 +1835,15 @@
     return HPS_OK;
 }
 
+extern "C" int hps_mg_split_info (void* handle, int* split, int* num_cus)
+{
+    HPS_REQUIRE(handle, "hps_mg_split_info: null handle");
+    const Multigrid* M = static_cast<const Multigrid*>(handle);
+    if (split) for (int il = 0; il < HPS_MG_MAXLEV; ++il) split[il] = il < M->lowv_begin ? (int)M->split(il) : -1;
+    if (num_cus) *num_cus = M->num_cus;
+    return HPS_OK;
+}
+
 extern "C" int hps_mg_solve1 (void* handle, hps_slab slab, int sol_comp, int rhs_comp, int acoef_comp, double tol_rel,
                               double tol_abs, int max_iters, int* iters_host, double* resnorm_host, hps_stream stream)
 {
@@ -1838,6 +1895,10 @@
         HPS_HIP_CHECK(hipMalloc(&d, 48*sizeof(long long)));
         HPS_HIP_CHECK(hipMemset(d, 0, 48*sizeof(long long)));
         HPS_HIP_CHECK(hipMemcpyToSymbol(HIP_SYMBOL(g_mg_dbg), &d, sizeof(d)));
+        const char* eh = getenv("HPS_MG_STAMP_HIX"); const char* er = getenv("HPS_MG_STAMP_RES");
+        const int hix = eh ? atoi(eh) : -1, res = er ? atoi(er) : -1;
+        HPS_HIP_CHECK(hipMemcpyToSymbol(HIP_SYMBOL(g_mg_dbg_hix), &hix, sizeof(hix)));
+        HPS_HIP_CHECK(hipMemcpyToSymbol(HIP_SYMBOL(g_mg_dbg_res), &res, sizeof(res)));
         return HPS_OK;
     }
     HPS_HIP_CHECK(hipDeviceSynchronize());
diff --git a/include/hpslice.h b/include/hpslice.h
--- a/include/hpslice.h
+++ b/include/hpslice.h
@@ -124,6 +124,7 @@
 enum { HPS_MG_MAXLEV = 31 };
 int hps_mg_info (void* handle, int* cc, int* nlev, int* lowv_begin, int* lowv_kind, long* lowv_lds, int* tiles,
                  int* nodal_pull1, int* pyr_levels, int* pyr_restricts);
+int hps_mg_split_info (void* handle, int* split, int* num_cus);
 int hps_mg_destroy (void* handle);
 
 int hps_mg2_create (int nx, int ny, double dx, double dy, void** handle);
```

Result: no change. 1654, median of 2 (+0.1%).
